# opensensor/thingino-accel

Measured on AMD Instinct MI355X. Metric: images/sec yolov5s_int8 640x640 batch256, higher is better.
Workload: dtype int8

## Files before the change

thingino-accel_amd/csrc/hip/conv_i8.hip:

```cpp
#include "conv_i8_common.hpp"

#ifndef I8M_ABL
#define I8M_ABL 0
#endif
template <int BPX, int BN, int STAGES, int KS = 1, int NW = 4>
__global__ __launch_bounds__(NW * 64) void conv_i8_mfma(const mhip_conv_i8_t p, const long total_pix, const int k64,
                                                         const int8_t *__restrict__ zeros, const unsigned noc,
                                                         const unsigned nblk, const int lg_inc, const unsigned kw_magic,
                                                         const fastdiv_t dhw, const fastdiv_t dow, const int bufmode,
                                                         const unsigned in_bytes) {
    ANAT_BEGIN();
    const bool POW2 = lg_inc >= 0;
    const bool masked = p.kh * p.kw <= 32;
    constexpr int SLICE = (BPX + BN) * BK;
    constexpr int STAGE = KS * SLICE;
    constexpr int NWN = BN == 128 ? 2 : 1;
    constexpr int NWM = NW / NWN;
    constexpr int WPX = BPX / NWM / 16;
    constexpr int WOC = BN / NWN / 16;
    constexpr int XROWS = BPX / NW;
    constexpr int XI = XROWS / 16;
    constexpr int LW = (BN / 16 + NW - 1) / NW;
    constexpr int L = XI + LW;
    static_assert(XI >= 1 && XROWS % 16 == 0, "every wave fetches whole 16-row pieces of the pixel tile");
// ... 1198 lines not shown
static bool chain_shape_ok(const mhip_conv_i8_t *a, const mhip_conv_i8_t *b, const mhip_conv_i8_t *d, int side) {
    if (!both_shape_ok(a, b) || a->out_c != 64 || !d || (side != 1 && side != 2)) return false;
    return d->kh == 1 && d->kw == 1 && d->stride_h == 1 && d->stride_w == 1 && !d->pad_top && !d->pad_left && d->in_c == 64 && d->out_c == 64 &&
           d->oc_pad == 64 && d->row_pad == 64 && d->frames == a->frames && d->in_h == a->out_h && d->in_w == a->out_w && d->out_h == a->out_h &&
           d->out_w == a->out_w && !d->out_pix_stride && !d->out_ch_off && d->lut && d->lut2 && !d->add && !d->out_nchw && d->nseg <= 1 &&
           persist_eligible(d) && d->out != a->out && d->out != b->out;
}
extern "C" int mhip_conv_i8_both_chain_ok(const mhip_conv_i8_t *a, const mhip_conv_i8_t *b, const mhip_conv_i8_t *d, int side) {
    return chain_shape_ok(a, b, d, side) ? 1 : 0;
}
static int both_launch(const mhip_conv_i8_t *a, const mhip_conv_i8_t *b, const conv_chain_t *ch);
extern "C" int mhip_conv_i8_both_chain(const mhip_conv_i8_t *a, const mhip_conv_i8_t *b, const mhip_conv_i8_t *d, int side, int elide) {
    if (!chain_shape_ok(a, b, d, side) || !d->w || !d->out) return -2;
    const mhip_conv_i8_t *src = side == 1 ? a : b;
    const mhip_conv_i8_t *other = side == 1 ? b : a;
    if (!other->out) return -2;
    if (!elide && (!src->out || d->in != src->out || d->in_stride != src->out_stride)) return -2;
    conv_chain_t ch;
    ch.w = d->w; ch.bias = d->bias; ch.lut2 = d->lut2; ch.out = d->out; ch.out_stride = d->out_stride;
    ch.out_bytes = (unsigned)persist_out_bytes(d); ch.cs = d->cs; ch.side = side; ch.elide = elide ? 1 : 0;
    return both_launch(a, b, &ch);
}
extern "C" int mhip_conv_i8_both(const mhip_conv_i8_t *a, const mhip_conv_i8_t *b) {
    if (!a || !b || !a->out || !b->out) return -2;
    return both_launch(a, b, nullptr);
}
static int both_launch(const mhip_conv_i8_t *a, const mhip_conv_i8_t *b, const conv_chain_t *ch) {
    if (!both_shape_ok(a, b) || (tune().variant && !ch) || !mhip_zero_page()) return -2;
    if (a->nseg > 1) {
        for (int i = 0; i < a->nseg; i++)
            if (a->seg_in[i] != b->seg_in[i]) return -2;
    } else if (a->in != b->in) {
        return -2;
    }
    const long total_pix = (long)a->frames * a->out_h * a->out_w;
    const int k64 = (a->kh * a->row_pad + BK - 1) / BK * BK, nks = k64 / BK;
    int lg = 0;
    while ((1 << lg) < a->in_c) lg++;
    int bpx, wres;
    both_form(2 * a->out_c, nks, ch != nullptr, &bpx, &wres);
    if (a->out_c == 128) {
        if (ch) return -2;
        return a->nseg > 1 ? launch_persist_t<128, 256, 2, true, true, false, true>(a, total_pix, k64, lg, 65536u, b, wres)
                           : launch_persist_t<128, 256, 2, true, false, false, true>(a, total_pix, k64, lg, 65536u, b, wres);
    }
    if (ch) {
        if (a->nseg > 1)
            return bpx == 256 ? launch_persist_t<256, 128, 2, true, true, false, true, true>(a, total_pix, k64, lg, 65536u, b, wres, ch)
                              : launch_persist_t<128, 128, 2, true, true, false, true, true>(a, total_pix, k64, lg, 65536u, b, wres, ch);
        return bpx == 256 ? launch_persist_t<256, 128, 2, true, false, false, true, true>(a, total_pix, k64, lg, 65536u, b, wres, ch)
                          : launch_persist_t<128, 128, 2, true, false, false, true, true>(a, total_pix, k64, lg, 65536u, b, wres, ch);
    }
    if (a->nseg > 1)
        return bpx == 256 ? launch_persist_t<256, 128, 2, true, true, false, true>(a, total_pix, k64, lg, 65536u, b, wres)
                          : launch_persist_t<128, 128, 2, true, true, false, true>(a, total_pix, k64, lg, 65536u, b, wres);
    return bpx == 256 ? launch_persist_t<256, 128, 2, true, false, false, true>(a, total_pix, k64, lg, 65536u, b, wres)
                      : launch_persist_t<128, 128, 2, true, false, false, true>(a, total_pix, k64, lg, 65536u, b, wres);
}

extern "C" int mhip_conv_i8_seg_ok(const mhip_conv_i8_t *p) {
    return p && (p->in_c % 16) == 0 && !mhip_conv_i8_small_c(p->in_c, p->kw, p->out_c) && seg_valid(p) && persist_eligible(p);
}

extern "C" int mhip_conv_i8_variants(const mhip_conv_i8_t *p, int *codes, int max) {
    if (!p || (p->in_c % 16) != 0 || mhip_conv_i8_small_c(p->in_c, p->kw, p->out_c)) return 0;
    const int k64 = (p->kh * p->row_pad + BK - 1) / BK * BK, nks = k64 / BK;
    int n = 0;
    if (p->pre_w) {
        const int first = conv_i8_pre_tile_rows(p);
        for (int th : {first, 16, 8, 4})
            if (th && n < max && conv_i8_patch_ok(p, th, nullptr)) {
                const int code = th == 16 ? 10 : (th == 8 ? 9 : 11);
                bool seen = false;
                for (int i = 0; i < n; i++) seen |= codes[i] == code;
                if (!seen) codes[n++] = code;
            }
        return n;
    }
    if (p->post_w) {
        for (int th : {16, 8, 4})
            if (n < max && conv_i8_patch_ok(p, th, nullptr)) codes[n++] = th == 16 ? 10 : (th == 8 ? 9 : 11);
        return n;
    }
    if (p->split_w) {
        for (int th : {16, 8, 4})
            if (n < max && conv_i8_patch_ok(p, th, nullptr)) codes[n++] = th == 16 ? 10 : (th == 8 ? 9 : 11);
        return n;
    }
    if (p->nseg > 1) {
        const int bn = p->oc_pad % 128 == 0 ? 128 : (p->oc_pad % 64 == 0 ? 64 : 32);
        const variant_t dv = default_variant(p, nks);
        const int dflt = dv.persist && dv.wres ? (dv.bpx == 256 ? 15 : 14) : (dv.bpx == 256 ? 4 : 2);
        if (n < max) codes[n++] = dflt;
        if (n < max && dflt != 2) codes[n++] = 2;
        if (n < max && dflt != 4) codes[n++] = 4;
        if (n < max && dflt != 14 && LUTB + 2 * (size_t)128 * BK + (size_t)nks * bn * BK <= 80 * 1024) codes[n++] = 14;
        if (n < max && dflt != 15 && LUTB + 2 * (size_t)256 * BK + (size_t)nks * bn * BK <= 80 * 1024) codes[n++] = 15;
        return n;
    }
    const int dflt = variant_code(default_variant(p, nks));
    if (n < max) codes[n++] = dflt;
    for (int code = 1; code <= NVARIANTS; code++) {
        const variant_t v = variant_of(code);
        if (code == dflt) continue;
        if (v.patch && !conv_i8_patch_ok(p, v.patch, nullptr)) continue;
        if (v.persist && !persist_eligible(p)) continue;
        if (v.ks2 && ((nks & 1) || nks < 4 || p->oc_pad % 64 != 0)) continue;
        if (v.w8 && (p->oc_pad % 128 != 0 || nks < 3)) continue;
        if (v.persist < 0) continue;
        if (v.r128 && !r128_ok(p)) continue;
        if (v.rows && !conv_i8_rows_ok(p)) continue;
        if (v.wres) {
            const int bn = p->oc_pad % 128 == 0 ? 128 : (p->oc_pad % 64 == 0 ? 64 : 32);
            if (LUTB + 2 * (size_t)v.bpx * BK + (size_t)nks * bn * BK > 80 * 1024) continue;
        }
        if (!v.persist && v.stages == 3 && nks <= 2) continue;
        if (n < max) codes[n++] = code;
    }
    return n;
}

template <int BN>
static int launch_generic(const mhip_conv_i8_t *p, long total_pix, int k64) {
    dim3 grid((unsigned)((total_pix + BP - 1) / BP), (unsigned)(p->oc_pad / BN));
    hipLaunchKernelGGL((conv_i8_generic<BN>), grid, dim3(NTHREADS), 0, mhip_stream_native(), *p, total_pix, k64,
                       make_fastdiv((unsigned)(p->out_h * p->out_w)));
    return mhip_check(hipGetLastError(), "conv_i8_generic launch");
}

extern "C" int mhip_conv_i8(const mhip_conv_i8_t *p) {
    if (!p || !p->in || (!p->out && !(p->post_w && p->post_out) && !(p->split_w && p->split_out[0] && p->split_out[1])) || !p->w) return -1;
    if (p->out_pix_stride < 0 || p->out_ch_off < 0 || (p->out_nchw && (p->out_pix_stride || p->out_ch_off)) ||
        (p->out_pix_stride && p->out_pix_stride < p->out_ch_off + p->out_c))
        return -1;
    if (p->frames <= 0 || p->in_h <= 0 || p->in_w <= 0 || p->in_c <= 0 || p->out_h <= 0 || p->out_w <= 0 ||
        p->out_c <= 0 || p->kh <= 0 || p->kw <= 0 || p->stride_h < 0 || p->stride_w < 0)
        return -1;
    int row_pad, oc_pad;
    mhip_conv_i8_pack_geom(p->in_c, p->kw, p->out_c, &row_pad, &oc_pad, nullptr);
    if (row_pad != p->row_pad || oc_pad != p->oc_pad) return -1;
    if (p->add && (!p->safe || p->out_nchw || ((p->out_c | p->out_pix_stride | p->out_ch_off) & 15) || (p->in_c % 16) != 0 ||
                   mhip_conv_i8_small_c(p->in_c, p->kw, p->out_c) || p->nseg > 1))
        return -1;
    const long total_pix = (long)p->frames * p->out_h * p->out_w;
    const int k64 = (p->kh * p->row_pad + BK - 1) / BK * BK;
    if (total_pix <= 0 || total_pix > 0x7fffffffL || (total_pix + BP - 1) / BP * (oc_pad / 32) > 0x7fffffffL) return -1;
    if (p->in_planar) {
        if (p->in_planar > 4 || p->in_c != 4 || p->in_w < 4 || p->stride_h < 1 || p->stride_w < 1 || p->add || p->nseg > 1 ||
            !mhip_conv_i8_small_c(p->in_c, p->kw, p->out_c))
            return -2;
        return conv_i8_try_smallc(p, k64);
    }
    if (mhip_conv_i8_small_c(p->in_c, p->kw, p->out_c)) {
        if (p->stride_h >= 1 && p->stride_w >= 1) {
            int rc = conv_i8_try_rgb(p, k64);
            if (rc == -2) rc = conv_i8_try_smallc(p, k64);
            if (rc != -2) return rc;
        }
        if (p->add || p->nseg > 1) return -1;
        if (oc_pad % 64 == 0) return launch_generic<64>(p, total_pix, k64);
        return launch_generic<32>(p, total_pix, k64);
    }
    if (p->pre_w) {
        if (!mhip_zero_page() || !mhip_conv_i8_pre_ok(p)) return -1;
        int th = conv_i8_pre_tile_rows(p);
        const int code = p->variant ? p->variant : tune().variant;
        if (code >= 9 && code <= 11) {
            const int want = code == 10 ? 16 : (code == 9 ? 8 : 4);
            if (conv_i8_patch_ok(p, want, nullptr)) th = want;
        } else if (tune().small_batch && conv_i8_patch_ok(p, 4, nullptr) &&
                   ((long)p->frames * p->out_h * p->out_w + 255) / 256 * ((p->oc_pad + 127) / 128) < 256) {
            th = 4;
        }
        return conv_i8_launch_patch(p, k64, th);
    }
    if (p->post_w) {
        if (!mhip_zero_page() || (p->in_c % 16) != 0 || !mhip_conv_i8_post_ok(p)) return -1;
        int th = conv_i8_post_tile_rows(p);
        const int code = p->variant ? p->variant : tune().variant;
        if (code >= 9 && code <= 11) {
            const int want = code == 10 ? 16 : (code == 9 ? 8 : 4);
            if (conv_i8_patch_ok(p, want, nullptr)) th = want;
        } else if (tune().small_batch && conv_i8_patch_ok(p, 4, nullptr) &&
                   ((long)p->frames * p->out_h * p->out_w + 255) / 256 * ((p->oc_pad + 127) / 128) < tune().few_wgs) {
            th = 4;
        }
        return conv_i8_launch_patch(p, k64, th);
    }
    if (p->split_w) {
        if (!mhip_zero_page() || (p->in_c % 16) != 0 || !mhip_conv_i8_split_ok(p)) return -1;
        int th = conv_i8_split_tile_rows(p);
        const int code = p->variant ? p->variant : tune().variant;
        if (code >= 9 && code <= 11) {
            const int want = code == 10 ? 16 : (code == 9 ? 8 : 4);
            if (conv_i8_patch_ok(p, want, nullptr)) th = want;
        } else if (tune().small_batch && conv_i8_patch_ok(p, 4, nullptr) &&
                   ((long)p->frames * p->out_h * p->out_w + 255) / 256 * ((p->oc_pad + 127) / 128) < tune().few_wgs) {
            th = 4;
        }
        return conv_i8_launch_patch(p, k64, th);
    }
    if ((p->in_c % 16) == 0) {
        if (!mhip_zero_page()) return -1;
        const int nks = k64 / BK;
        if (p->variant < 0 || p->variant > NVARIANTS) return -1;
        int code = p->variant;
        if (p->nseg > 1) {
            if (!seg_valid(p) || !persist_eligible(p)) return -1;
            if (!code && tune().variant) {
                int codes[NVARIANTS];
                const int n = mhip_conv_i8_variants(p, codes, NVARIANTS);
                for (int i = 0; i < n; i++)
                    if (codes[i] == tune().variant) code = codes[i];
            }
            variant_t v = variant_of(code == 4 || code == 14 || code == 15 ? code : 2);
            if (!code) {
                const variant_t dv = default_variant(p, nks);
                v.bpx = dv.bpx ? dv.bpx : 128;
                v.wres = dv.persist && dv.wres;
            }
            return launch_variant(p, total_pix, k64, v);
        }
        if (!code && tune().variant) {
            int codes[NVARIANTS];
            const int n = mhip_conv_i8_variants(p, codes, NVARIANTS);
            for (int i = 0; i < n; i++)
                if (codes[i] == tune().variant) code = codes[i];
        }
        return launch_variant(p, total_pix, k64, code ? variant_of(code) : default_variant(p, nks));
    }
    if (oc_pad % 64 == 0) return launch_generic<64>(p, total_pix, k64);
    return launch_generic<32>(p, total_pix, k64);
}
```

thingino-accel_amd/csrc/hip/conv_i8_common.hpp:

```cpp
#pragma once
#include <hip/hip_runtime.h>
#include <stdint.h>
#include <stdlib.h>
#include <string.h>
#include <type_traits>

#include "../mhip.h"

extern "C" hipStream_t mhip_stream_native(void);
extern "C" int mhip_check(hipError_t e, const char *what);
extern "C" const void *mhip_zero_page(void);

typedef int v4i __attribute__((ext_vector_type(4)));
typedef int v2i __attribute__((ext_vector_type(2)));

#ifdef ANATOMY
struct anat_rec_t {
    unsigned key, wg, hwid, xcc;
    unsigned long long t[4];
};
static __device__ anat_rec_t *g_anat_buf;
static __device__ unsigned g_anat_cap;
#define ANAT_SETTER(NAME)                                                                                                    \
    extern "C" int NAME(void *buf, unsigned cap) {                                                                          \
// ... 352 lines not shown
                if (rem & 8) { __builtin_memcpy(d, s, 8); o = 8; }
                if (rem & 4) { __builtin_memcpy(d + o, s + o, 4); o += 4; }
                if (rem & 2) { __builtin_memcpy(d + o, s + o, 2); o += 2; }
                if (rem & 1) d[o] = s[o];
            }
        }
    } else {
        for (int id = tid; id < BPX * BN; id += (int)blockDim.x) {
            const int c = id / BPX, row = id - c * BPX;
            const long off = rowoff[row];
            if (off < 0 || c >= ncols) continue;
            p.out[off + (size_t)(oc0 + c) * hw] = tile[row * ROW + c];
        }
    }
}

template <int BPX, int BN, int WPX, int WOC, bool LUT0 = false>
__device__ __forceinline__ void epilogue(const mhip_conv_i8_t &p, v4i (&acc)[WOC][WPX], int8_t *tile, const uint8_t *slut,
                                         const long *rowoff, int oc0, int pxw, int ocw, int hw) {
    const bool direct = !p.out_nchw && ((p.out_c | p.out_pix_stride | p.out_ch_off) & 15) == 0;
#define EPI(L, S, D) epilogue_t<BPX, BN, WPX, WOC, L, S, D, LUT0>(p, acc, tile, slut, rowoff, oc0, pxw, ocw, hw)
    if (direct) {
        if (p.lut) { if (p.safe) EPI(true, true, true); else EPI(true, false, true); }
        else { if (p.safe) EPI(false, true, true); else EPI(false, false, true); }
    } else {
        if (p.lut) { if (p.safe) EPI(true, true, false); else EPI(true, false, false); }
        else { if (p.safe) EPI(false, true, false); else EPI(false, false, false); }
    }
#undef EPI
}

template <int WPX, int WOC>
__device__ __forceinline__ void init_acc(const mhip_conv_i8_t &p, v4i (&acc)[WOC][WPX], int ocbase) {
    const int lane = threadIdx.x & 63;
#pragma unroll
    for (int s = 0; s < WOC; s++) {
        const v4i b = p.bias ? *(const v4i *)(p.bias + ocbase + s * 16 + (lane >> 4) * 4) : (v4i){0, 0, 0, 0};
#pragma unroll
        for (int t = 0; t < WPX; t++) acc[s][t] = b;
    }
}


struct tune_t {
    int init;
    int persist;
    int persist_stages;
    int persist_maxk;
    int persist_slots;
    int stages;
    int bpx;
    int variant;
    int bufmode;
    int small_batch;
    int rgb_direct;
    int wres;
    int few_wgs;
    int rows;
    int patch_ring;
    int patch_lds_kb;
    int both_bpx;
    int both_wide;
};
const tune_t &conv_i8_tune_state();

extern "C" int mhip_conv_i8_small_c(int in_c, int kw, int out_c);

static inline long in_extent_bytes(const mhip_conv_i8_t *p) {
    return (long)(p->frames - 1) * (long)p->in_stride + (long)p->in_h * p->in_w * p->in_c;
}
static inline long persist_out_bytes(const mhip_conv_i8_t *p) {
    const long pstride = p->out_pix_stride ? p->out_pix_stride : p->out_c;
    return (long)(p->frames - 1) * (long)p->out_stride + (long)p->out_h * p->out_w * pstride;
}
static inline bool conv_i8_direct_rows(const mhip_conv_i8_t *p) {
    return !p->out_nchw && ((p->out_c | p->out_pix_stride | p->out_ch_off) & 15) == 0;
}

bool conv_i8_patch_ok(const mhip_conv_i8_t *p, int th, int *ring);
int conv_i8_launch_patch(const mhip_conv_i8_t *p, int k64, int th);
int conv_i8_pre_tile_rows(const mhip_conv_i8_t *p);
int conv_i8_post_tile_rows(const mhip_conv_i8_t *p);
int conv_i8_split_tile_rows(const mhip_conv_i8_t *p);
bool conv_i8_rows_ok(const mhip_conv_i8_t *p);
int conv_i8_launch_rows(const mhip_conv_i8_t *p);
int conv_i8_try_rgb(const mhip_conv_i8_t *p, int k64);
int conv_i8_try_smallc(const mhip_conv_i8_t *p, int k64);
```

thingino-accel_amd/csrc/hip/conv_i8_patch.hip:

```cpp
#include "conv_i8_common.hpp"
#include <stdio.h>

#ifdef PATCH_STAMPS
__device__ unsigned long long patch_stamp_sums[8];
extern "C" int mhip_patch_stamps(unsigned long long *out, int reset) {
    if (out && hipMemcpyFromSymbol(out, HIP_SYMBOL(patch_stamp_sums), sizeof(patch_stamp_sums)) != hipSuccess) return -1;
    if (reset) {
        unsigned long long z[8] = {0};
        if (hipMemcpyToSymbol(HIP_SYMBOL(patch_stamp_sums), z, sizeof(z)) != hipSuccess) return -1;
    }
    return 0;
}
#define STAMP(t)                                                                          \
    do {                                                                                  \
        __builtin_amdgcn_sched_barrier(0);                                                \
        asm volatile("s_memtime %0\n\ts_waitcnt lgkmcnt(0)" : "=s"(t)::"memory");        \
        __builtin_amdgcn_sched_barrier(0);                                                \
    } while (0)
#else
#define STAMP(t) do { } while (0)
#endif
#define PT_TW 16
#define PT_NIMAX 10

template <int LO, int HI>
__device__ __forceinline__ void wait_vmcnt_tree(int n) {
    if constexpr (LO == HI) {
        wait_vmcnt<LO>();
    } else {
        constexpr int MID = (LO + HI + 1) / 2;
        if (n >= MID) wait_vmcnt_tree<MID, HI>(n);
        else wait_vmcnt_tree<LO, MID - 1>(n);
    }
}
template <int HI>
__device__ __forceinline__ void wait_vmcnt_upto(int n) {
    wait_vmcnt_tree<0, HI>(n > HI ? HI : n);
}
__device__ __forceinline__ void barrier_lds() {
    asm volatile("s_waitcnt lgkmcnt(0)\n\ts_barrier" ::: "memory");
}

template <int TH, int BN, bool HAS_LUT, bool PRE = false, bool POST = false, bool SPLIT = false, bool CHAIN = false>
__global__ __launch_bounds__(NTHREADS) void conv_i8_patch(const mhip_conv_i8_t p, const int k64, const int tiles_x,
                                                          const int tiles_y, const unsigned ntiles_all, const int PH,
                                                          const int PW, const int PWP, const int PWH, const int nblk,
                                                          const int8_t *__restrict__ zeros, const fastdiv_t dtx,
                                                          const fastdiv_t dty, const fastdiv_t dpwp, const unsigned out_bytes,
                                                          const int ring, const int xmap, const unsigned in_bytes) {
    ANAT_BEGIN();
    constexpr int WPX = TH / 4;
    constexpr int WOC = BN / 16;
    constexpr int NST = WPX;
    extern __shared__ __attribute__((aligned(16))) int8_t dynlds[];
    uint8_t *slut = (uint8_t *)dynlds;
    lds_base_must_be_zero(dynlds);
    const int nks = k64 / BK;
    constexpr int NPO = 2 * BN;
    static_assert(!SPLIT || (BN == 64 && HAS_LUT && !PRE && !POST), "SPLIT: one 64-channel tile, no other stage");
    static_assert(!CHAIN || SPLIT, "CHAIN: a stage of the SPLIT form");
    constexpr int LB = LUTB + ((PRE || POST) ? 512 : 0) + (SPLIT ? 1024 : 0) + (CHAIN ? 512 : 0);
    int *dutab = (int *)(dynlds + LB);
    int8_t *wl = dynlds + LB + ((nks * 16 + 255) & ~255);
    const int patch_bytes = nblk * 1024;
    int8_t *w1l = wl + nks * BN * BK;
    int8_t *pwl = w1l;
    const int *pbl = (const int *)(pwl + NPO * NPO);
    int8_t *swl = w1l;
    const int *sbl = (const int *)(swl + 64 * BK);
    int8_t *cwl = swl + 64 * BK + 64 * 4;
    const int *cbl = (const int *)(cwl + 32 * BK);
    int8_t *patch0 = w1l + (PRE ? p.in_c * BK : 0) + (POST ? NPO * NPO + NPO * 4 : 0) + (SPLIT ? 64 * BK + 64 * 4 : 0) + (CHAIN ? 32 * BK + 32 * 4 : 0);
    int8_t *tpatch = patch0 + ring * patch_bytes;

    const int tid = threadIdx.x, lane = tid & 63;
    const int wv = __builtin_amdgcn_readfirstlane(tid >> 6);
    const int oc0 = blockIdx.y * BN;
    const int C = p.in_c, lgc = 31 - __builtin_clz((unsigned)C), cpp = C >> 4, lgcpp = lgc - 4;
    const int s = p.stride_w;
    const unsigned M = C >= 128 ? 6u : (C >= 64 ? 2u : 0u);

    v4i bias[WOC];
#pragma unroll
    for (int q = 0; q < WOC; q++) bias[q] = p.bias ? *(const v4i *)(p.bias + oc0 + q * 16 + (lane >> 4) * 4) : (v4i){0, 0, 0, 0};
    constexpr int W1MAX = 4;
    v4i pbias[PRE ? W1MAX : 1];
    if (PRE) {
#pragma unroll
        for (int q = 0; q < W1MAX; q++) pbias[q] = q < (C >> 4) ? *(const v4i *)(p.pre_bias + q * 16 + (lane >> 4) * 4) : (v4i){0, 0, 0, 0};
    }
    if (HAS_LUT) {
        if (p.lut2) { if (tid < 128) ((uint32_t *)slut)[tid] = ((const uint32_t *)p.lut2)[tid]; }
        else if (tid < 64) ((uint32_t *)slut)[tid] = ((const uint32_t *)p.lut)[tid];
    }
    if (PRE && tid >= 128) ((uint32_t *)slut)[tid] = ((const uint32_t *)p.pre_lut2)[tid - 128];
    if (POST) {
        if (tid >= 128) ((uint32_t *)slut)[tid] = ((const uint32_t *)p.post_lut2)[tid - 128];
        if (tid < NPO) ((int *)(pwl + NPO * NPO))[tid] = ((const int *)(p.post_w + NPO * NPO))[tid];
    }
    if (SPLIT) {
        if (tid >= 128) {
            ((uint32_t *)slut)[tid] = ((const uint32_t *)p.split_lut2[0])[tid - 128];
            ((uint32_t *)slut)[tid + 128] = ((const uint32_t *)p.split_lut2[1])[tid - 128];
        }
        if (tid < 64) ((int *)(swl + 64 * BK))[tid] = ((const int *)(p.split_w + 64 * BK))[tid];
    }
    if (CHAIN) {
        if (tid >= 128) ((uint32_t *)slut)[tid + 256] = ((const uint32_t *)p.chain_lut2)[tid - 128];
        if (tid >= 64 && tid < 96) ((int *)(cwl + 32 * BK))[tid - 64] = ((const int *)(p.chain_w + 32 * BK))[tid - 64];
    }
    const int rowbytes = p.kw * C, kbytes = p.kh * rowbytes;
    for (int i = tid; i < nks * 4; i += NTHREADS) {
        const int kb = i * 16;
        int du = 0;
        if (kb < kbytes) {
            const int ky = kb / rowbytes, rem = kb - ky * rowbytes, kx = rem >> lgc, cc = (rem & (C - 1)) >> 4;
            const int dp = ky * PWP + (s == 2 ? (kx >> 1) + (kx & 1) * PWH : kx);
            du = dp * cpp + cc;
        }
        dutab[i] = du;
    }
    __syncthreads();
    {
        const int schunk = (lane & 3) ^ (((lane >> 4) & 1) << 1);
        for (int i = wv; i < nks * (BN / 16); i += 4) {
            const int ks = i / (BN / 16), g = i - ks * (BN / 16);
            glds16(p.w + (size_t)(oc0 + g * 16 + (lane >> 2)) * k64 + ks * BK + schunk * 16, wl + (ks * BN + g * 16) * BK);
        }
        if (PRE)
            for (int g = wv; g < C / 16; g += 4) glds16(p.pre_w + (size_t)(g * 16 + (lane >> 2)) * BK + schunk * 16, w1l + g * 16 * BK);
        if (POST)
            for (int i = wv; i < NPO * NPO / 1024; i += 4) glds16(p.post_w + i * 1024 + lane * 16, pwl + i * 1024);
        if (SPLIT)
            glds16(p.split_w + wv * 1024 + lane * 16, swl + wv * 1024);
        if (CHAIN && wv < 2)
            glds16(p.chain_w + wv * 1024 + lane * 16, cwl + wv * 1024);
    }
    int uoff[PT_NIMAX], upos[PT_NIMAX];
#pragma unroll
    for (int n = 0; n < PT_NIMAX; n++) {
        uoff[n] = 0;
        upos[n] = -1;
        if (n * 4 + wv < nblk) {
            const unsigned phys = (unsigned)((n * 4 + wv) * 64 + lane);
            const unsigned U = phys ^ ((phys >> 3) & M);
            const unsigned pp = U >> lgcpp, cc = U & (unsigned)(cpp - 1);
            const unsigned py = fdiv(pp, dpwp), col = pp - py * (unsigned)PWP;
            const int px = s == 2 ? ((int)col < PWH ? 2 * (int)col : 2 * ((int)col - PWH) + 1) : (int)col;
            if ((int)py < PH && px < PW) {
                uoff[n] = ((int)py * p.in_w + px) * C + (int)cc * 16;
                upos[n] = ((int)py << 16) | px;
            }
        }
    }
    const int npw = nblk > wv ? (nblk - wv + 3) >> 2 : 0;
    const unsigned xcd = blockIdx.x & 7u;
    const unsigned xstart = xmap ? (unsigned)(((unsigned long long)ntiles_all * xcd) >> 3) : 0u;
    const unsigned xend = xmap ? (unsigned)(((unsigned long long)ntiles_all * (xcd + 1u)) >> 3) : 0u;
    const unsigned ntiles = xmap ? (xend - xstart) * 8u + xcd : ntiles_all;
    auto tile_xy = [&](unsigned t, int &tx, int &ty, unsigned &f) {
        const unsigned j = xmap ? xstart + (t >> 3) : t, q = fdiv(j, dtx);
        tx = (int)(j - q * (unsigned)tiles_x);
        f = fdiv(q, dty);
        ty = (int)(q - f * (unsigned)tiles_y);
    };
    const __amdgpu_buffer_rsrc_t xrs = __builtin_amdgcn_make_buffer_rsrc((void *)p.in, 0, (int)in_bytes, 0x00020000);
    auto issue_patch = [&](unsigned t, int8_t *dst) {
#ifdef PATCH_ABL
        return;
#endif
        int tx, ty;
        unsigned f;
        tile_xy(t, tx, ty, f);
        const int iy0 = ty * TH * s - p.pad_top, ix0 = tx * PT_TW * s - p.pad_left;
        if (in_bytes != 0u && iy0 >= 0 && ix0 >= 0 && iy0 + PH <= p.in_h && ix0 + PW <= p.in_w) {
            const int sbase = (int)(f * (unsigned)p.in_stride) + (iy0 * p.in_w + ix0) * C;
#pragma unroll
            for (int n = 0; n < PT_NIMAX; n++)
                if (n * 4 + wv < nblk) blds16(xrs, uoff[n], sbase, dst + (n * 4 + wv) * 1024);
            return;
        }
        const int8_t *base = p.in + (size_t)f * p.in_stride + ((long)iy0 * p.in_w + ix0) * C;
#pragma unroll
        for (int n = 0; n < PT_NIMAX; n++)
            if (n * 4 + wv < nblk) {
                const int py = upos[n] >> 16, px = upos[n] & 0xffff;
                const bool ok = upos[n] >= 0 && (unsigned)(iy0 + py) < (unsigned)p.in_h && (unsigned)(ix0 + px) < (unsigned)p.in_w;
                glds16(ok ? base + uoff[n] : zeros, dst + (n * 4 + wv) * 1024);
            }
    };

    const __amdgpu_buffer_rsrc_t orsrc = __builtin_amdgcn_make_buffer_rsrc(SPLIT ? p.split_out[0] : (POST ? p.post_out : p.out), 0, (int)out_bytes, 0x00020000);
    const unsigned out_bytes1 = SPLIT ? (unsigned)(p.frames - 1) * (unsigned)p.split_out_stride[1] + (unsigned)(p.out_h * p.out_w) * 32u : 0u;
    const __amdgpu_buffer_rsrc_t orsrc1 = __builtin_amdgcn_make_buffer_rsrc(SPLIT ? p.split_out[1] : p.out, 0, (int)out_bytes1, 0x00020000);
    const unsigned out_bytes2 = CHAIN ? (unsigned)(p.frames - 1) * (unsigned)p.chain_out_stride + (unsigned)(p.out_h * p.out_w) * 32u : 0u;
    const __amdgpu_buffer_rsrc_t orsrc2 = __builtin_amdgcn_make_buffer_rsrc(CHAIN ? p.chain_out : p.out, 0, (int)out_bytes2, 0x00020000);
    const bool cside1 = CHAIN && p.chain_side == 2;
    const bool has_add = !SPLIT && p.add != nullptr;
    constexpr int RROW = WOC == 4 ? 1024 : 512;
    constexpr int NRI = WOC == 4 ? WPX : 2 * WPX;
    int8_t *rstage = patch0 + (ring + (PRE ? 1 : 0)) * patch_bytes + wv * (WPX * RROW);
    const int frow = lane & 15, fchunk = lane >> 4;
    const int chan = (lane >> 4) * (4 * WOC);
    const int NR = has_add || POST ? NRI : 0;
    const int ntail = POST ? (has_add ? NRI : 0) + WPX * (NPO / 64) : (SPLIT ? (CHAIN ? 3 : 2) * WPX : NST);
    const int ppstride = p.post_out_pix_stride ? p.post_out_pix_stride : NPO;
    auto issue_rows = [&](const int8_t *base, size_t fstride, int tx, int ty, unsigned f) {
#pragma unroll
        for (int u = 0; u < WPX; u++) {
            const int oy = ty * TH + wv * WPX + u, ox = tx * PT_TW + frow;
            const int8_t *src = oy < p.out_h && ox < p.out_w ? base + (size_t)f * fstride + ((size_t)(oy * p.out_w + ox) * BN + (size_t)chan) : zeros;
            if (WOC == 4) {
                glds16(src, rstage + u * RROW);
            } else {
                __builtin_amdgcn_global_load_lds((const __attribute__((address_space(1))) void *)src,
                                                 (__attribute__((address_space(3))) void *)(rstage + u * RROW), 4, 0, 0);
                __builtin_amdgcn_global_load_lds((const __attribute__((address_space(1))) void *)(src + 4),
                                                 (__attribute__((address_space(3))) void *)(rstage + u * RROW + 256), 4, 0, 0);
            }
        }
    };
    const int pstride = p.out_pix_stride ? p.out_pix_stride : p.out_c;
    const int lo = p.relu ? 0 : -128;
    const uint8_t *lut128 = slut + 128;
    int ubase[WPX];
#pragma unroll
    for (int u = 0; u < WPX; u++) ubase[u] = ((wv * WPX + u) * s * PWP + frow) * cpp;

    const unsigned G = gridDim.x;
    const int D = ring - 1;
    unsigned t = blockIdx.x;
    int yg0 = 0, yg1 = 0, yg2 = 0;
    {
        int issued = 0;
        for (int d = 0; d < D; d++)
            if (t + (unsigned)d * G < ntiles) {
                issue_patch(t + (unsigned)d * G, patch0 + d * patch_bytes);
                issued++;
            }
        yg0 = issued > 1 ? (issued - 1) * npw : 0;
        yg1 = issued > 2 ? (issued - 2) * npw : 0;
        yg2 = 0;
    }
#ifdef PATCH_STAMPS
    unsigned long long st0 = 0, st1 = 0, st2 = 0, st3 = 0, st4 = 0, sum_wait = 0, sum_issue = 0, sum_k = 0, sum_epi = 0, sum_tiles = 0;
#endif
    int cur = 0;
    int pn_last = 0;
    bool first = true;
    ANAT_NOW(1);
    for (; t < ntiles; t += G) {
        STAMP(st0);
        int tx, ty;
        unsigned f;
        tile_xy(t, tx, ty, f);
        int voffs[WPX];
        uint32_t xw[WPX][WOC];
#pragma unroll
        for (int u = 0; u < WPX; u++) {
            const int oy = ty * TH + wv * WPX + u, ox = tx * PT_TW + frow;
            const unsigned off = f * (unsigned)p.out_stride + (unsigned)(oy * p.out_w + ox) * (unsigned)pstride +
                                 (unsigned)(p.out_ch_off + oc0 + chan);
            const bool ok = oy < p.out_h && ox < p.out_w && oc0 + chan < p.out_c;
            voffs[u] = ok ? (int)off : -1;
#pragma unroll
            for (int q = 0; q < WOC; q++) xw[u][q] = 0;
        }
        if (POST) {
#pragma unroll
            for (int u = 0; u < WPX; u++) {
                const int oy = ty * TH + wv * WPX + u, ox = tx * PT_TW + frow;
                const unsigned off = f * (unsigned)p.post_out_stride + (unsigned)(oy * p.out_w + ox) * (unsigned)ppstride +
                                     (unsigned)(p.post_out_ch_off + (lane >> 4) * (NPO / 4));
                voffs[u] = oy < p.out_h && ox < p.out_w ? (int)off : -1;
            }
            if (has_add) issue_rows(p.add, p.out_stride, tx, ty, f);
            else issue_rows(p.post_in, p.post_in_stride, tx, ty, f);
        } else if (SPLIT) {
#pragma unroll
            for (int u = 0; u < WPX; u++) {
                const int oy = ty * TH + wv * WPX + u, ox = tx * PT_TW + frow;
                voffs[u] = oy < p.out_h && ox < p.out_w ? (oy * p.out_w + ox) * 32 + (lane >> 4) * 8 : -1;
            }
        } else if (has_add) {
#pragma unroll
            for (int u = 0; u < WPX; u++) {
                const int8_t *src = voffs[u] >= 0 ? p.add + (unsigned)voffs[u] : zeros;
                if (WOC == 4) {
// ... 59 lines not shown
                    }
                    uint32_t pk4[4];
                    requant_pack_pre<16>(a1, p.pre_cs, pk4);
#pragma unroll
                    for (int e = 0; e < 4; e++) pk1[e] = inimg ? pk4[e] : 0u;
                    const unsigned Uw = (unsigned)(pp * cpp + (lane >> 4));
                    if (live) *(v4i *)(tpatch + ((Uw ^ ((Uw >> 3) & M)) << 4)) = (v4i){(int)pk1[0], (int)pk1[1], (int)pk1[2], (int)pk1[3]};
                } else {
                    int a1[8];
#pragma unroll
                    for (int q = 0; q < 2; q++) {
                        const v4i wa = *(const v4i *)(w1l + lds_off(q * 16 + frow, fchunk));
                        const v4i r = __builtin_amdgcn_mfma_i32_16x16x64_i8(wa, xb1, pbias[PRE ? q : 0], 0, 0, 0);
#pragma unroll
                        for (int e = 0; e < 4; e++) a1[q * 4 + e] = r[e];
                    }
                    uint32_t pk2[2];
                    requant_pack_pre<8>(a1, p.pre_cs, pk2);
                    const int g4 = lane >> 4;
                    const unsigned Uw = (unsigned)(pp * cpp + (g4 >> 1));
                    if (live)
                        *(uint2 *)(tpatch + ((Uw ^ ((Uw >> 3) & M)) << 4) + (g4 & 1) * 8) = make_uint2(inimg ? pk2[0] : 0u, inimg ? pk2[1] : 0u);
                }
            }
            barrier_lds();
            patch = tpatch;
        }
        v4i acc[WOC][WPX];
        v4i xa[WPX], wa[WOC], xb[WPX], wb[WOC];
        auto load_frags = [&](int ks, int du, v4i (&xf)[WPX], v4i (&wf)[WOC]) {
#pragma unroll
            for (int u = 0; u < WPX; u++) {
                const unsigned U = (unsigned)(ubase[u] + du);
                xf[u] = *(const v4i *)(patch + ((U ^ ((U >> 3) & M)) << 4));
            }
            const int8_t *ws = wl + ks * BN * BK;
#pragma unroll
            for (int q = 0; q < WOC; q++) wf[q] = *(const v4i *)(ws + lds_off(q * 16 + frow, fchunk));
        };
        auto mfma_step = [&](const v4i (&xf)[WPX], const v4i (&wf)[WOC]) {
#pragma unroll
            for (int q = 0; q < WOC; q++)
#pragma unroll
                for (int u = 0; u < WPX; u++) acc[q][u] = __builtin_amdgcn_mfma_i32_16x16x64_i8(wf[q], xf[u], acc[q][u], 0, 0, 0);
        };
        const int last = nks - 1;
        auto clampk = [&](int k) { return k < last ? k : last; };
        load_frags(0, dutab[fchunk], xa, wa);
        load_frags(clampk(1), dutab[clampk(1) * 4 + fchunk], xb, wb);
        int du_n = dutab[clampk(2) * 4 + fchunk];
#pragma unroll
        for (int q = 0; q < WOC; q++)
#pragma unroll
            for (int u = 0; u < WPX; u++) acc[q][u] = __builtin_amdgcn_mfma_i32_16x16x64_i8(wa[q], xa[u], bias[q], 0, 0, 0);
        int ks = 1;
        for (; ks + 1 < nks; ks += 2) {
            load_frags(ks + 1, du_n, xa, wa);
            du_n = dutab[clampk(ks + 2) * 4 + fchunk];
            __builtin_amdgcn_sched_barrier(0);
            mfma_step(xb, wb);
            __builtin_amdgcn_sched_barrier(0);
            load_frags(clampk(ks + 2), du_n, xb, wb);
            du_n = dutab[clampk(ks + 3) * 4 + fchunk];
            __builtin_amdgcn_sched_barrier(0);
            mfma_step(xa, wa);
            __builtin_amdgcn_sched_barrier(0);
        }
        if (ks < nks) mfma_step(xb, wb);
        STAMP(st3);
        if (D > 0) cur = cur + 1 == ring ? 0 : cur + 1;
        if (has_add) {
            if (D > 0) wait_vmcnt_upto<15>(pn_last);
#pragma unroll
            for (int u = 0; u < WPX; u++) {
                if (WOC == 4) {
                    const v4i r = *(const v4i *)(rstage + u * RROW + lane * 16);
                    xw[u][0] = (uint32_t)r[0]; xw[u][1] = (uint32_t)r[1]; xw[u][WOC > 2 ? 2 : 0] = (uint32_t)r[2]; xw[u][WOC > 3 ? 3 : 0] = (uint32_t)r[3];
                } else {
                    xw[u][0] = *(const uint32_t *)(rstage + u * RROW + lane * 4);
                    xw[u][WOC > 1 ? 1 : 0] = *(const uint32_t *)(rstage + u * RROW + 256 + lane * 4);
                }
            }
        }
        uint32_t pku[POST || SPLIT ? WPX : 1][WOC];
        if (POST && has_add) {
#pragma unroll
            for (int u = 0; u < WPX; u++) {
                if constexpr (WOC == 4) asm volatile("s_waitcnt lgkmcnt(0)" : "+v"(xw[u][0]), "+v"(xw[u][1]), "+v"(xw[u][2]), "+v"(xw[u][3])::"memory");
                else asm volatile("s_waitcnt lgkmcnt(0)" : "+v"(xw[u][0]), "+v"(xw[u][1])::"memory");
            }
            issue_rows(p.post_in, p.post_in_stride, tx, ty, f);
        }
#pragma unroll
        for (int u = 0; u < WPX; u++) {
            uint32_t pk[WOC];
            int a[WOC * 4];
#pragma unroll
            for (int q = 0; q < WOC; q++)
#pragma unroll
                for (int r = 0; r < 4; r++) a[q * 4 + r] = acc[q][u][r];
            const bool fast = HAS_LUT && p.lut2 != nullptr;
            if (has_add) {
                const add_args_t ga = {p.add_s_conv, p.add_s_other, p.add_inv};
                if (fast) requant_pack<WOC * 4, HAS_LUT, true, true, true, true>(a, p.cs, lo, lut128, pk, xw[u], &ga);
                else requant_pack<WOC * 4, HAS_LUT, true, true, true>(a, p.cs, lo, lut128, pk, xw[u], &ga);
            } else {
                if (fast) requant_pack<WOC * 4, HAS_LUT, true, true, false, true>(a, p.cs, lo, lut128, pk);
                else requant_pack<WOC * 4, HAS_LUT, true, true>(a, p.cs, lo, lut128, pk);
            }
            if (POST) {
#pragma unroll
                for (int q = 0; q < WOC; q++) pku[POST ? u : 0][q] = pk[q];
                continue;
            }
            if (SPLIT) {
#pragma unroll
                for (int q = 0; q < WOC; q++) pku[SPLIT ? u : 0][q] = pk[q];
                continue;
            }
            const int voff = voffs[u];
            if (WOC == 4)
                __builtin_amdgcn_raw_buffer_store_b128((v4i){(int)pk[0], (int)pk[1], (int)pk[2], (int)pk[3]}, orsrc, voff, 0, 0);
            else if (WOC == 2)
                __builtin_amdgcn_raw_buffer_store_b64((v2i){(int)pk[0], (int)pk[WOC > 1 ? 1 : 0]}, orsrc, voff, 0, 0);
        }
        if (SPLIT) {
            v4i sw4[4], sb4[4];
#pragma unroll
            for (int r = 0; r < 4; r++) {
                sw4[r] = *(const v4i *)(swl + lds_off(r * 16 + frow, fchunk));
                sb4[r] = *(const v4i *)(sbl + r * 16 + fchunk * 4);
            }
            v4i sc[WPX][4];
#pragma unroll
            for (int u = 0; u < WPX; u++) {
                const v4i b0 = {(int)pku[SPLIT ? u : 0][0], (int)pku[SPLIT ? u : 0][1], (int)pku[SPLIT ? u : 0][WOC > 2 ? 2 : 0], (int)pku[SPLIT ? u : 0][WOC > 3 ? 3 : 0]};
#pragma unroll
                for (int r = 0; r < 4; r++) sc[u][r] = __builtin_amdgcn_mfma_i32_16x16x64_i8(sw4[r], b0, sb4[r], 0, 0, 0);
            }
            const unsigned fo0 = f * (unsigned)p.split_out_stride[0], fo1 = f * (unsigned)p.split_out_stride[1];
            uint32_t ck[CHAIN ? WPX : 1][2];
#pragma unroll
            for (int u = 0; u < WPX; u++) {
                int a2[16];
#pragma unroll
                for (int r = 0; r < 4; r++)
#pragma unroll
                    for (int e = 0; e < 4; e++) a2[r * 4 + e] = sc[u][r][e];
                uint32_t pk4[4];
                requant_pack_two(a2, p.split_cs[0], p.split_cs[1], pk4);
                const int voff0 = voffs[u] >= 0 ? voffs[u] + (int)fo0 : -1, voff1 = voffs[u] >= 0 ? voffs[u] + (int)fo1 : -1;
                __builtin_amdgcn_raw_buffer_store_b64((v2i){(int)pk4[0], (int)pk4[1]}, orsrc, voff0, 0, 0);
                __builtin_amdgcn_raw_buffer_store_b64((v2i){(int)pk4[2], (int)pk4[3]}, orsrc1, voff1, 0, 0);
                if (CHAIN) {
                    ck[CHAIN ? u : 0][0] = cside1 ? pk4[2] : pk4[0];
                    ck[CHAIN ? u : 0][1] = cside1 ? pk4[3] : pk4[1];
                }
            }
            if (CHAIN) {
                v4i cw4[2], cb4[2];
#pragma unroll
                for (int r = 0; r < 2; r++) {
                    cw4[r] = *(const v4i *)(cwl + lds_off(r * 16 + frow, fchunk));
                    cb4[r] = *(const v4i *)(cbl + r * 16 + fchunk * 4);
                }
                v4i cc[WPX][2];
#pragma unroll
                for (int u = 0; u < WPX; u++) {
                    const v4i b0 = {(int)ck[CHAIN ? u : 0][0], (int)ck[CHAIN ? u : 0][1], 0, 0};
#pragma unroll
                    for (int r = 0; r < 2; r++) cc[u][r] = __builtin_amdgcn_mfma_i32_16x16x64_i8(cw4[r], b0, cb4[r], 0, 0, 0);
                }
                const unsigned fo2 = f * (unsigned)p.chain_out_stride;
#pragma unroll
                for (int u = 0; u < WPX; u++) {
                    int a1[8];
#pragma unroll
                    for (int r = 0; r < 2; r++)
#pragma unroll
                        for (int e = 0; e < 4; e++) a1[r * 4 + e] = cc[u][r][e];
                    uint32_t pk2[2];
                    requant_pack_chain(a1, p.chain_cs, pk2);
                    const int voff2 = voffs[u] >= 0 ? voffs[u] + (int)fo2 : -1;
                    __builtin_amdgcn_raw_buffer_store_b64((v2i){(int)pk2[0], (int)pk2[1]}, orsrc2, voff2, 0, 0);
                }
            }
        }
        if (POST) {
            if (has_add) wait_vmcnt<0>();
            else if (D > 0) wait_vmcnt_upto<15>(pn_last);
#pragma unroll
            for (int u = 0; u < WPX; u++) {
                v4i b0, b1 = {0, 0, 0, 0};
                if (WOC == 4) {
                    b0 = (v4i){(int)pku[POST ? u : 0][0], (int)pku[POST ? u : 0][1], (int)pku[POST ? u : 0][WOC > 2 ? 2 : 0], (int)pku[POST ? u : 0][WOC > 3 ? 3 : 0]};
                    b1 = *(const v4i *)(rstage + u * RROW + lane * 16);
                } else {
                    b0 = (v4i){(int)pku[POST ? u : 0][0], (int)pku[POST ? u : 0][WOC > 1 ? 1 : 0], *(const int *)(rstage + u * RROW + lane * 4),
                               *(const int *)(rstage + u * RROW + 256 + lane * 4)};
                }
#pragma unroll
                for (int h = 0; h < NPO / 64; h++) {
                    int a[16];
#pragma unroll
                    for (int s4 = 0; s4 < 4; s4++) {
                        const int row = (h * 4 + s4) * 16;
                        v4i c = *(const v4i *)(pbl + row + fchunk * 4);
// ... 1 lines not shown
                        if (WOC == 4) c = __builtin_amdgcn_mfma_i32_16x16x64_i8(*(const v4i *)(pwl + NPO * BK + lds_off(row + frow, fchunk)), b1, c, 0, 0, 0);
#pragma unroll
                        for (int e = 0; e < 4; e++) a[s4 * 4 + e] = c[e];
                    }
                    uint32_t pk4[4];
                    requant_pack_pre<16>(a, p.post_cs, pk4);
                    const int voff = voffs[u] >= 0 ? voffs[u] + h * 16 : -1;
                    __builtin_amdgcn_raw_buffer_store_b128((v4i){(int)pk4[0], (int)pk4[1], (int)pk4[2], (int)pk4[3]}, orsrc, voff, 0, 0);
                }
            }
        }
#ifdef PATCH_STAMPS
        STAMP(st4);
        if (D == 0) st1 = st2;
        sum_wait += st1 - st0; sum_issue += st2 - st1; sum_k += st3 - st2; sum_epi += st4 - st3; sum_tiles += 1;
#endif
    }
    ANAT_NOW(2);
    ANAT_END(p);
#ifdef PATCH_STAMPS
    if (lane == 0) {
        atomicAdd(&patch_stamp_sums[0], sum_wait); atomicAdd(&patch_stamp_sums[1], sum_issue); atomicAdd(&patch_stamp_sums[2], sum_k);
        atomicAdd(&patch_stamp_sums[3], sum_epi); atomicAdd(&patch_stamp_sums[4], sum_tiles);
    }
#endif
}

ANAT_SETTER(mhip_anatomy_set_patch)
struct patch_geom_t {
    int bn, tiles_x, tiles_y, PH, PW, PWP, PWH, nblk, nks, ring;
    size_t lds;
};
static inline const tune_t &tune() { return conv_i8_tune_state(); }
static size_t patch_lds_budget(int bn) {
    const int kb = tune().patch_lds_kb;
    if (kb >= 16 && kb <= 160 && kb != 80) return (size_t)kb * 1024;
    return (size_t)(bn == 32 ? 53 : 80) * 1024;
}
static bool patch_geom(const mhip_conv_i8_t *p, int th, patch_geom_t *g) {
    const bool direct = conv_i8_direct_rows(p);
    const int C = p->in_c, s = p->stride_w;
    static const bool no_c16 = getenv("MARS_HIP_PATCH_NO_C16") != nullptr;
    if (!direct || !p->safe || (C != 16 && C != 32 && C != 64 && C != 128) || (C == 16 && (no_c16 || p->pre_w)) || (s != 1 && s != 2) || p->stride_h != s ||
        p->kh > 7 || p->kw > 7 || p->kh * p->kw < 2 || p->row_pad != p->kw * C || persist_out_bytes(p) > 0x7fffffffL)
        return false;
    const int k64 = (p->kh * p->row_pad + BK - 1) / BK * BK;
    g->nks = k64 / BK;
    g->bn = p->oc_pad % 64 == 0 ? 64 : 32;
    g->tiles_x = (p->out_w + PT_TW - 1) / PT_TW;
    g->tiles_y = (p->out_h + th - 1) / th;
    if ((double)p->out_h * p->out_w < (C == 128 ? 0.80 : 0.85) * (double)g->tiles_x * PT_TW * g->tiles_y * th) return false;
    g->PH = (th - 1) * s + p->kh;
    g->PW = (PT_TW - 1) * s + p->kw;
    g->PWH = s == 2 ? (g->PW + 1) / 2 : 0;
    g->PWP = s == 2 ? 2 * g->PWH : g->PW;
    const long units = (long)g->PH * g->PWP * (C / 16);
    g->nblk = (int)((units + 63) / 64);
    if (g->nblk > 4 * PT_NIMAX) return false;
    const bool pre = p->pre_w != nullptr;
    if (pre && (s != 1 || (C != 32 && C != 64) || !p->pre_bias || !p->pre_lut2 || !p->lut2)) return false;
    const bool post = p->post_w != nullptr;
    if (post) {
        const long ppstride = p->post_out_pix_stride ? p->post_out_pix_stride : 2 * g->bn;
        if (pre || s != 1 || p->out_c != g->bn || p->oc_pad != g->bn || p->out_pix_stride || p->out_ch_off || !p->lut2 || !p->post_lut2 || !p->post_in ||
            !p->post_out || ((p->post_out_pix_stride | p->post_out_ch_off) & 15) || p->post_out_pix_stride < 0 || p->post_out_ch_off < 0 ||
            ppstride < p->post_out_ch_off + 2 * g->bn ||
            (long)(p->frames - 1) * (long)p->post_out_stride + (long)p->out_h * p->out_w * ppstride > 0x7fffffffL)
            return false;
    }
    const bool split = p->split_w != nullptr;
    if (split) {
        if (pre || post || p->add || g->bn != 64 || p->out_c != 64 || p->oc_pad != 64 || p->out_pix_stride || p->out_ch_off || !p->lut2 || !p->split_lut2[0] ||
            !p->split_lut2[1] || !p->split_out[0] || !p->split_out[1])
            return false;
        for (int i = 0; i < 2; i++)
            if ((long)(p->frames - 1) * (long)p->split_out_stride[i] + (long)p->out_h * p->out_w * 32 > 0x7fffffffL) return false;
    }
    const bool chain = p->chain_side != 0;
    if (chain) {
        if (!split || (p->chain_side != 1 && p->chain_side != 2) || !p->chain_w || !p->chain_lut2 || !p->chain_out || p->chain_out == p->split_out[0] ||
            p->chain_out == p->split_out[1] || (long)(p->frames - 1) * (long)p->chain_out_stride + (long)p->out_h * p->out_w * 32 > 0x7fffffffL)
            return false;
    }
    const size_t pb = (size_t)g->nblk * 1024;
    const size_t radd = p->add || post ? (size_t)4 * (th / 4) * (g->bn == 64 ? 1024 : 512) : 0;
    const size_t fixed = LUTB + (pre ? 512 + (size_t)C * BK + pb : 0) + (post ? 512 + (size_t)4 * g->bn * g->bn + (size_t)8 * g->bn : 0) +
                         (split ? 1024 + (size_t)64 * BK + 64 * 4 : 0) + (chain ? 512 + (size_t)32 * BK + 32 * 4 : 0) +
                         (((size_t)g->nks * 16 + 255) & ~(size_t)255) + (size_t)g->nks * g->bn * BK + radd;
    const size_t budget = patch_lds_budget(g->bn);
    if (fixed + pb > budget) return false;
    const int fit = (int)((budget - fixed) / pb);
    const int cap = tune().patch_ring > 0 ? (tune().patch_ring > 4 ? 4 : tune().patch_ring) : 2;
    int ring = fit < cap ? fit : cap;
    g->ring = ring;
    g->lds = fixed + (size_t)ring * pb;
    if ((long)g->tiles_x * g->tiles_y * p->frames > 0x7fffffffL) return false;
    return true;
}

static inline long post_out_bytes(const mhip_conv_i8_t *p) {
    const long ppstride = p->post_out_pix_stride ? p->post_out_pix_stride : 2 * p->out_c;
    return (long)(p->frames - 1) * (long)p->post_out_stride + (long)p->out_h * p->out_w * ppstride;
}
static inline long split_out_bytes(const mhip_conv_i8_t *p, int side) {
    return (long)(p->frames - 1) * (long)p->split_out_stride[side] + (long)p->out_h * p->out_w * 32;
}
template <int TH, int BN, bool HAS_LUT, bool PRE = false, bool POST = false, bool SPLIT = false, bool CHAIN = false>
static int launch_patch_t(const mhip_conv_i8_t *p, int k64, const patch_geom_t &g) {
    auto kern = conv_i8_patch<TH, BN, HAS_LUT, PRE, POST, SPLIT, CHAIN>;
    static int cus = 0;
    static size_t slots_lds[8];
    static int slots_n[8], nslots = 0;
    if (!cus) {
        int dev = 0;
        hipDeviceProp_t prop;
        if (hipFuncSetAttribute((const void *)kern, hipFuncAttributeMaxDynamicSharedMemorySize, 160 * 1024) != hipSuccess ||
            hipGetDevice(&dev) != hipSuccess || hipGetDeviceProperties(&prop, dev) != hipSuccess)
            return mhip_check(hipErrorUnknown, "conv_i8_patch occupancy query");
        cus = prop.multiProcessorCount;
    }
    int slots = 0;
    for (int i = 0; i < nslots; i++)
        if (slots_lds[i] == g.lds) slots = slots_n[i];
    if (!slots) {
        int occ = 0;
        if (hipOccupancyMaxActiveBlocksPerMultiprocessor(&occ, kern, NTHREADS, g.lds) != hipSuccess)
            return mhip_check(hipErrorUnknown, "conv_i8_patch occupancy query");
        slots = (occ > 0 ? occ : 1) * cus;
        if (nslots < 8) { slots_lds[nslots] = g.lds; slots_n[nslots++] = slots; }
    }
    const unsigned ntiles = (unsigned)((long)g.tiles_x * g.tiles_y * p->frames);
    const unsigned noc = (unsigned)(p->oc_pad / BN);
    unsigned gx = (unsigned)(tune().persist_slots > 0 ? tune().persist_slots : slots) / noc;
    if (gx < 1) gx = 1;
    if (gx > ntiles) gx = ntiles;
    const int xmap = gx >= 8 && ntiles < 0x0fffffffu;
    if (xmap) gx &= ~7u;
    {
        static const char *dbg = getenv("MARS_HIP_PATCH_DEBUG");
        static size_t last_lds = 0;
        static int last_ring = 0;
        if (dbg && (last_lds != g.lds || last_ring != g.ring)) {
            fprintf(stderr, "Mars: conv_i8_patch<%d,%d> ring %d, patch %d KB, LDS %zu B, %d workgroups per CU, grid %u x %u\n", TH, BN, g.ring,
                    g.nblk, g.lds, slots / cus, gx, noc);
            last_lds = g.lds;
            last_ring = g.ring;
        }
    }
    hipLaunchKernelGGL(kern, dim3(gx, noc), dim3(NTHREADS), g.lds, mhip_stream_native(), *p, k64,
                       g.tiles_x, g.tiles_y, ntiles, g.PH, g.PW, g.PWP, g.PWH, g.nblk, (const int8_t *)mhip_zero_page(),
                       make_fastdiv((unsigned)g.tiles_x), make_fastdiv((unsigned)g.tiles_y), make_fastdiv((unsigned)g.PWP),
                       (unsigned)(SPLIT ? split_out_bytes(p, 0) : (POST ? post_out_bytes(p) : persist_out_bytes(p))), g.ring, xmap,
                       in_extent_bytes(p) <= 0x7fffffffL ? (unsigned)in_extent_bytes(p) : 0u);
    return mhip_check(hipGetLastError(), "conv_i8_patch launch");
}

bool conv_i8_patch_ok(const mhip_conv_i8_t *p, int th, int *ring) {
    patch_geom_t g;
    if (!patch_geom(p, th, &g)) return false;
    if (ring) *ring = g.ring;
    return true;
}

int conv_i8_launch_patch(const mhip_conv_i8_t *p, int k64, int th) {
    patch_geom_t g;
    if (!patch_geom(p, th, &g)) return -1;
#define PATCH(T, B)                                                                       \
    (p->post_w ? launch_patch_t<T, B, true, false, true>(p, k64, g)                       \
     : p->pre_w ? launch_patch_t<T, B, true, true>(p, k64, g)                             \
                : (p->lut ? launch_patch_t<T, B, true>(p, k64, g) : launch_patch_t<T, B, false>(p, k64, g)))
    if (p->split_w && p->chain_side) {
        if (th == 16) return launch_patch_t<16, 64, true, false, false, true, true>(p, k64, g);
        if (th == 8) return launch_patch_t<8, 64, true, false, false, true, true>(p, k64, g);
        return launch_patch_t<4, 64, true, false, false, true, true>(p, k64, g);
    }
    if (p->split_w) {
        if (th == 16) return launch_patch_t<16, 64, true, false, false, true>(p, k64, g);
        if (th == 8) return launch_patch_t<8, 64, true, false, false, true>(p, k64, g);
        return launch_patch_t<4, 64, true, false, false, true>(p, k64, g);
    }
    if (th == 16) return g.bn == 64 ? PATCH(16, 64) : PATCH(16, 32);
    if (th == 8) return g.bn == 64 ? PATCH(8, 64) : PATCH(8, 32);
    return g.bn == 64 ? PATCH(4, 64) : PATCH(4, 32);
#undef PATCH
}

int conv_i8_pre_tile_rows(const mhip_conv_i8_t *p) {
    patch_geom_t g;
    for (int th : {16, 8, 4})
        if (patch_geom(p, th, &g) && (th == 4 || g.ring >= 2)) return th;
    return 0;
}
extern "C" int mhip_conv_i8_pre_ok(const mhip_conv_i8_t *p) {
    if (!p || !p->pre_w || p->nseg > 1 || p->out_nchw) return 0;
    return conv_i8_pre_tile_rows(p) != 0;
}

int conv_i8_post_tile_rows(const mhip_conv_i8_t *p) {
    patch_geom_t g;
    for (int th : {16, 8, 4})
        if (patch_geom(p, th, &g)) return th;
    return 0;
}
extern "C" int mhip_conv_i8_post_ok(const mhip_conv_i8_t *p) {
    if (!p || !p->post_w || p->pre_w || p->nseg > 1 || p->out_nchw) return 0;
    return conv_i8_post_tile_rows(p) != 0;
}
extern "C" int mhip_conv_i8_post_k(int c, int k) {
    if (c == 64) return k;
    return k < 32 ? (k >> 3) * 16 + (k & 7) : ((k - 32) >> 3) * 16 + 8 + (k & 7);
}
extern "C" int mhip_conv_i8_post_row(int c, int oc) {
    const int per = c / 2, g = oc / per, rem = oc - g * per;
    return (rem >> 2) * 16 + g * 4 + (rem & 3);
}
extern "C" size_t mhip_conv_i8_post_pack(int c, const int8_t *packed, const int32_t *bias, int8_t *out) {
    if (c != 32 && c != 64) return 0;
    const int n = 2 * c;
    const size_t bytes = (size_t)n * n + (size_t)n * 4;
    if (!packed || !out) return bytes;
    memset(out, 0, bytes);
    for (int oc = 0; oc < n; oc++) {
        const int R = mhip_conv_i8_post_row(c, oc), src = mhip_conv_i8_oc_row(oc, n);
        for (int k = 0; k < n; k++) {
            const int pos = mhip_conv_i8_post_k(c, k), ks = pos >> 6, chunk = (pos & 63) >> 4;
            out[(size_t)(ks * n + R) * BK + (((chunk ^ ((R >> 1) & 2))) << 4) + (pos & 15)] = packed[(size_t)src * n + k];
        }
        ((int32_t *)(out + (size_t)n * n))[R] = bias ? bias[src] : 0;
    }
    return bytes;
}

int conv_i8_split_tile_rows(const mhip_conv_i8_t *p) {
    patch_geom_t g;
    for (int th : {16, 8, 4})
        if (patch_geom(p, th, &g)) return th;
    return 0;
}
extern "C" int mhip_conv_i8_split_ok(const mhip_conv_i8_t *p) {
    if (!p || !p->split_w || p->pre_w || p->post_w || p->add || p->nseg > 1 || p->out_nchw) return 0;
    return conv_i8_split_tile_rows(p) != 0;
}
extern "C" int mhip_conv_i8_split_row(int side, int oc) {
    const int g = oc >> 3, rem = oc & 7;
    return side * 32 + (rem >> 2) * 16 + g * 4 + (rem & 3);
}
extern "C" size_t mhip_conv_i8_split_pack(const int8_t *packed0, const int32_t *bias0, const int8_t *packed1, const int32_t *bias1, int8_t *out) {
    const size_t bytes = (size_t)64 * BK + (size_t)64 * 4;
    if (!packed0 || !packed1 || !out) return bytes;
    memset(out, 0, bytes);
    for (int side = 0; side < 2; side++) {
        const int8_t *packed = side ? packed1 : packed0;
        const int32_t *bias = side ? bias1 : bias0;
        for (int oc = 0; oc < 32; oc++) {
            const int R = mhip_conv_i8_split_row(side, oc), src = mhip_conv_i8_oc_row(oc, 32);
            for (int k = 0; k < 64; k++) out[(size_t)R * BK + ((((k >> 4) ^ ((R >> 1) & 2))) << 4) + (k & 15)] = packed[(size_t)src * 64 + k];
            ((int32_t *)(out + (size_t)64 * BK))[R] = bias ? bias[src] : 0;
        }
    }
    return bytes;
}

extern "C" int mhip_conv_i8_chain_k(int c) { return (c >> 3) * 16 + (c & 7); }
extern "C" size_t mhip_conv_i8_chain_pack(const int8_t *packed, const int32_t *bias, int8_t *out) {
    const size_t bytes = (size_t)32 * BK + (size_t)32 * 4;
    if (!packed || !out) return bytes;
    memset(out, 0, bytes);
    for (int oc = 0; oc < 32; oc++) {
        const int R = mhip_conv_i8_split_row(0, oc), src = mhip_conv_i8_oc_row(oc, 32);
        for (int c = 0; c < 32; c++) {
            const int k = mhip_conv_i8_chain_k(c);
            out[(size_t)R * BK + ((((k >> 4) ^ ((R >> 1) & 2))) << 4) + (k & 15)] = packed[(size_t)src * 64 + c];
        }
        ((int32_t *)(out + (size_t)32 * BK))[R] = bias ? bias[src] : 0;
    }
    return bytes;
}
```

thingino-accel_amd/csrc/host/mars_internal.h:

```cpp
#ifndef MARS_INTERNAL_H
#define MARS_INTERNAL_H

#include <math.h>
#include <stddef.h>
#include <stdint.h>

#include "../mhip.h"
#include "mars_hip.h"
#include "mars_runtime.h"

enum {
    OP_CONV_I8 = 0,
    OP_CONV_F32,
    OP_RELU_BYTES,
    OP_LUT_I8,
    OP_BINARY_I8,
    OP_SIGMOID_F32,
    OP_BINARY_F32,
    OP_RELU_F32,
    OP_BN,
    OP_MAXPOOL,
    OP_CONCAT_SLICE,
    OP_UPSAMPLE,
    OP_UPSAMPLE_Q, OP_MAXPOOL_Q,
    OP_CONCAT_Q,
    OP_CONV_F32_VHEAD,
    OP_FAIL,
};

#define NO_OFF ((size_t)-1)
#define MARS_MAX_IO 4
#define MARS_MAX_MODEL_TUNE 16

typedef struct {
    size_t bytes;
    size_t extent;
    size_t stride;
    uint8_t *dev;
    int is_weight;
    int needed;
    int io_in, io_out;
    uint8_t *host;
    uint8_t *dense_dev;
    int pix_c, pix_stride;
    int rec_c, rec_hw;
    int nhwc_c, nhwc_hw;
    size_t zero_from;
    int partial;
    int nhwc_pitch;
    int tail_read;
} mtensor_t;

typedef struct {
    int kind, layer, err;
    int t_in[4], n_in, t_out;
    int in_h, in_w, in_c, out_h, out_w, out_c, kh, kw, sh, sw, pt, pl;
    int nchw, relu, is_mul, is_f32, leaky, safe;
    size_t in_byte_off, out_byte_off;
    int k_limit;
    int vc_n, vc_t[3], vc_run, vc_shift;
    int rows_only;
    int out_nchw;
    int silu_f32;
    int f32_exact;
    int variant;
    int add_t; float add_s_conv, add_s_other, add_inv;
    int nseg, seg_t[4], seg_c[4], seg_up;
    int chain_n, chain_out[3];
    int pair_next;
    int pair_both;
    int both_chain;
    int both_elide;
    int row_pad, oc_pad, c_pad;
    int ch_off, scale_h, scale_w, bn_n;
    int out_pix_stride, out_ch_off;
    int store_c;
    float cs, f0, f1, f2;
    size_t n;
    size_t w_off, b_off, lut_off, s_off;
    int pre;
    size_t pre_w_off, pre_b_off, pre_lut2_off;
    float pre_cs;
    int post_next;
    size_t post_w_off;
    int split_next;
    size_t split_w_off;
    int split_chain;
    size_t chain_w_off;
    size_t w2_off;
    int w2_rows;
    int w2_planes;
    size_t w3_off;
    int w3_stem;
    int in_rec, out_rec;
    size_t lut2_off;
    size_t w_blob_off[2];
    double macs, bytes;
    int prof_kind;
    float last_ms;
    void *ev0, *ev1;
    int prof_rec;
    void *ev_start;
} mars_op_t;

typedef struct { void *dev; size_t bytes; int frames; void *ev[2]; } mars_block_t;
typedef struct { void *dst; size_t off, bytes; } mars_block_part_t;
typedef struct { void *dev; int cap, frames; } mars_det_side_t;
typedef struct { int buf; const int8_t *base; size_t stride; int c, h, w, pix_step, ch_step; } mars_side_tensor_t;
typedef struct { float key[4][2]; int n; } mars_lut_cache_t;

typedef struct {
    int fusion;
    unsigned no_fuse_lut : 1, no_nhwc_internal : 1, no_vconcat_q : 1, no_pair_f32 : 1, no_rec : 1, no_zero_tail : 1, no_vconcat_f32 : 1,
        no_rowpad : 1, no_post : 1, no_split : 1, no_chain : 1, no_both : 1, no_both_chain : 1;
    size_t rec_limit;
    size_t vconcat_limit;
    size_t bottleneck_limit;
} plan_switches_t;

typedef struct mars_model_ext {
    mars_model_t pub;
    plan_switches_t sw;
    int batch, profiling, deferred;
    int plan_err;
    int no_vconcat;
    int no_download;
    int no_bottleneck;
    int no_post;
    int no_split;
    int no_chain;
    int no_both;
    int no_both_chain;
    int rec_frames;
    int rec_skipped;
    size_t rec_max_frames;
    mtensor_t *mt;
    mars_op_t *ops;
    int n_ops, cap_ops;
    uint8_t *arena_host;
    size_t arena_size, arena_cap;
    uint8_t *arena_dev;
    size_t blob_mirror_bytes;
    uint8_t *act_dev;
    size_t act_bytes;
    uint8_t *scratch_dev;
    size_t scratch_per_frame;
    int scratch_t, scratch_cpad, scratch_f0, scratch_n;
    void *det_dev;
    int *det_counts_dev;
    float *det_lut_dev;
    int det_cap;
    mars_lut_cache_t det_lut;
    int det_lut_mono[4];
    float *heads_lut_dev;
    mars_lut_cache_t heads_lut;
    float *dfl_lut_dev;
    mars_lut_cache_t dfl_lut;
    void *ev_graph_done, *ev_tail_done;
    int tail_pending;
    int frame0, run_frames;
    void *ev_fork, *ev_join[3];
    void *ev_chunk[2][8];
    void *graph_exec;
    unsigned graph_gen;
    int ran_plain;
    void *pipe;
    struct { char key[28]; int value, saved; } tune[MARS_MAX_MODEL_TUNE];
    int n_tune, tune_depth;
    int plan_f32_mode;
    unsigned char *layer_noop;
    void *roi_dev;
    int roi_cap_slots, roi_cap_frames;
    int roi_slots;
    struct mars_model_ext *roi_from;
    void *roi_fit_dev;
    int roi_fit_slots;
    mars_block_t cls;
    size_t cls_sums_off, cls_top_off;
    int cls_c, cls_top_k;
    void *ev_label_done;
    int label_pending;
    mars_det_side_t label;
    mars_block_t match;
    size_t match_top_off, match_row_off;
    int match_top_k;
    mars_det_side_t ident;
    mars_det_side_t track;
    mars_block_t track_app;
    mars_block_t seg;
    size_t seg_rec_off, seg_word_off;
    int seg_max, seg_ph, seg_pw;
    mars_block_t segn;
    size_t segn_rec_off, segn_word_off;
    int segn_max, segn_oh, segn_ow;
    int segn_key[10];
    mars_block_t pose;
    size_t pose_rec_off, pose_kpt_off;
    int pose_max, pose_k;
    mars_lut_cache_t pose_lut;
    mars_block_t obb;
    size_t obb_cnt_off, obb_out_off, obb_csn_off;
    mars_lut_cache_t obb_lut;
    int det_mapped;
    mars_block_t tile_roi;
    mars_block_t tile;
    size_t tile_off[4];
    mars_block_t redact;
    size_t redact_stats_off;
    void *ev_redact_done;
    mars_block_t overlay;
    size_t overlay_stats_off;
    void *overlay_img;
    size_t overlay_img_bytes;
    mars_det_side_t motion;
    struct mars_model_ext *live_next;
} mars_model_ext_t;

enum {
    FORM_PLAIN = 0,
    FORM_PAIR,
    FORM_BOTH,
    FORM_BOTH_CHAIN,
    FORM_POST,
    FORM_SPLIT,
    FORM_SPLIT_CHAIN,
    FORM_PAIR_F32,
    FORM_BAD,
    FORM_COUNT
};
static inline int form_span(int form) {
    static const int span[FORM_COUNT] = {[FORM_PLAIN] = 1, [FORM_PAIR] = 2, [FORM_BOTH] = 2, [FORM_BOTH_CHAIN] = 3, [FORM_POST] = 2, [FORM_SPLIT] = 3,
                                         [FORM_SPLIT_CHAIN] = 4, [FORM_PAIR_F32] = 2, [FORM_BAD] = 1};
    return form >= 0 && form < FORM_COUNT ? span[form] : 0;
}
static inline int op_form(const mars_model_ext_t *m, int i, int g[4]) {
    const mars_op_t *o = &m->ops[i];
    int form = FORM_PLAIN;
    if (o->split_next) form = o->split_chain ? FORM_SPLIT_CHAIN : FORM_SPLIT;
    else if (o->post_next) form = FORM_POST;
    else if (o->pair_next) form = o->kind == OP_CONV_F32 ? FORM_PAIR_F32 : !o->pair_both ? FORM_PAIR : o->both_chain ? FORM_BOTH_CHAIN : FORM_BOTH;
    int span = form_span(form);
    if (i + span > m->n_ops) { form = FORM_BAD; span = m->n_ops - i; }
    for (int k = 0; k < 4; k++) g[k] = k < span ? i + k : -1;
    return form;
}
static inline int op_span(const mars_model_ext_t *m, int i) {
    int g[4], n = 0;
    op_form(m, i, g);
    while (n < 4 && g[n] >= 0) n++;
    return n;
}
static inline int op_head(const mars_model_ext_t *m, int i) {
    int h = 0;
    for (int s; h + (s = op_span(m, h)) <= i; h += s) {}
    return h;
}
static inline int op_is_mate(const mars_model_ext_t *m, int i) { return op_head(m, i) != i; }
static inline int op_plain(const mars_model_ext_t *m, int i) {
    int g[4];
    return op_form(m, i, g) == FORM_PLAIN;
}
static inline uint8_t *tdev(const mars_model_ext_t *m, int ti) {
    if (ti < 0 || !m->mt[ti].dev) return NULL;
    return m->mt[ti].dev + (m->mt[ti].is_weight ? 0 : (size_t)m->frame0 * m->mt[ti].stride);
}
static inline size_t tstride(const mars_model_ext_t *m, int ti) { return ti >= 0 ? m->mt[ti].stride : 0; }


#define MARS_INTERNAL __attribute__((visibility("hidden")))
#define ALIGN_UP(x, a) (((x) + (size_t)(a) - 1) & ~((size_t)(a) - 1))
#define NO_TENSOR 0xFFFFFFFFu
#define MAX_DIM_PRODUCT ((size_t)1 << 40)
#define ARENA_MAX ((size_t)1 << 40)
#define MAX_CHANNELS 65536
MARS_INTERNAL int mars_verbose(void);
#define VLOG(...) do { if (mars_verbose()) fprintf(stderr, "Mars: " __VA_ARGS__); } while (0)
MARS_INTERNAL void drop_graph(mars_model_ext_t *m);
MARS_INTERNAL mars_model_ext_t *mars_live_models(void);
MARS_INTERNAL void plan_switches_read(plan_switches_t *sw, int at_load);
MARS_INTERNAL mars_error_t build_plan(mars_model_ext_t *m);
MARS_INTERNAL mars_error_t upload_params(mars_model_ext_t *m);
MARS_INTERNAL mars_error_t alloc_batch(mars_model_ext_t *m, int n);
MARS_INTERNAL size_t elem_size(uint32_t dtype);
MARS_INTERNAL size_t shape_numel(const mars_tensor_t *d);
MARS_INTERNAL size_t reference_buffer_size(const mars_model_ext_t *m);
MARS_INTERNAL size_t arena_reserve(mars_model_ext_t *m, size_t bytes);
MARS_INTERNAL void blob_read(const mars_model_ext_t *m, size_t off, size_t n, void *dst);
MARS_INTERNAL int op_reads(const mars_op_t *o, int t);
MARS_INTERNAL int op_writes(const mars_op_t *o, int t);
MARS_INTERNAL size_t planned_stride(const mtensor_t *t);
MARS_INTERNAL int conv_i8_pre_fits(const mars_op_t *op, int frames, size_t in_stride, size_t out_stride);
MARS_INTERNAL void conv_i8_group_records(const mars_model_ext_t *m, int form, const mars_op_t *g[4], int side, int frames, int live, mhip_conv_i8_t *p);
MARS_INTERNAL int conv_i8_group_fits(const mars_model_ext_t *m, int form, const mars_op_t *g[4], int side, int frames);
MARS_INTERNAL void fuse_both_chain(mars_model_ext_t *m);
MARS_INTERNAL void plan_layer(mars_model_ext_t *m, int li);
MARS_INTERNAL void fold_silu(mars_model_ext_t *m, int f32);
MARS_INTERNAL void fuse_lut(mars_model_ext_t *m);
MARS_INTERNAL void nhwc_internal(mars_model_ext_t *m);
MARS_INTERNAL void fold_add(mars_model_ext_t *m, int f32);
MARS_INTERNAL void virtual_concat(mars_model_ext_t *m);
MARS_INTERNAL void elide_concat(mars_model_ext_t *m);
MARS_INTERNAL void trim_concat(mars_model_ext_t *m);
MARS_INTERNAL void fuse_pool_chains(mars_model_ext_t *m);
MARS_INTERNAL void pair_convs(mars_model_ext_t *m);
MARS_INTERNAL void fuse_bottleneck(mars_model_ext_t *m);
MARS_INTERNAL void fuse_post(mars_model_ext_t *m);
MARS_INTERNAL void fuse_split(mars_model_ext_t *m);
MARS_INTERNAL void fuse_split_chain(mars_model_ext_t *m);
MARS_INTERNAL void pad_output_rows(mars_model_ext_t *m);
MARS_INTERNAL void virtual_concat_q(mars_model_ext_t *m);
MARS_INTERNAL void f32_policy(mars_model_ext_t *m);
MARS_INTERNAL void zero_tail_f32(mars_model_ext_t *m);
MARS_INTERNAL void pair_convs_f32(mars_model_ext_t *m);
MARS_INTERNAL void rec_pairs(mars_model_ext_t *m);
MARS_INTERNAL void virtual_concat_f32(mars_model_ext_t *m);
MARS_INTERNAL void plan_check(mars_model_ext_t *m);
MARS_INTERNAL int mars_preproc_prepare(int w, int h, int tw, int th);
MARS_INTERNAL int mars_preproc_prepare_nv12(int w, int h, int tw, int th, int frames);

MARS_INTERNAL void mars_roi_release(mars_model_ext_t *m);

static inline int mars_scale_ok(float s) { return s > 0 && isfinite(s); }
static inline mars_error_t mars_stage_guard(const mars_model_ext_t *m) {
    if (!m->act_dev || !mhip_ready()) return MARS_ERR_NNA_INIT_FAILED;
    return m->pipe ? MARS_ERR_INVALID_TENSOR : MARS_OK;
}
static inline int mars_has_dets(const mars_model_ext_t *m) { return m->det_dev && m->det_counts_dev && m->det_cap >= m->batch; }
typedef struct { int tid, nhwc, tw, th; int8_t *dev; size_t stride; } mars_pixel_input_t;
MARS_INTERNAL mars_error_t mars_pixel_input(const mars_model_ext_t *m, int input_index, int geometry_only, mars_pixel_input_t *out);
MARS_INTERNAL mars_error_t mars_aux_behind_current(void **ev);
MARS_INTERNAL size_t mars_block_layout(const size_t *sz, int n, size_t *off);
MARS_INTERNAL mars_error_t mars_block_reserve(mars_block_t *b, size_t total, int with_events, int *fresh);
MARS_INTERNAL void mars_block_release(mars_block_t *b);
MARS_INTERNAL float mars_block_ms(const mars_block_t *b);
MARS_INTERNAL mars_error_t mars_block_fetch(const mars_block_t *b, const mars_block_part_t *parts, int n, int *tail_pending);
MARS_INTERNAL mars_error_t mars_side_reserve(mars_det_side_t *s, int frames, size_t rec);
MARS_INTERNAL void mars_side_release(mars_det_side_t *s);
MARS_INTERNAL mars_error_t mars_side_fetch(const mars_det_side_t *s, void *dst, size_t rec);
MARS_INTERNAL mars_error_t mars_scatter_on_aux(mars_model_ext_t *det, mars_model_ext_t *m, const mars_block_t *src, size_t top_off, int top_k,
                                               mars_det_side_t *side);
MARS_INTERNAL mars_error_t mars_side_tensor(const mars_model_ext_t *m, int T, int want_c, int want_h, int want_w, mars_side_tensor_t *out);
MARS_INTERNAL int mars_lut_stale(const mars_lut_cache_t *c, int n, const float key[4][2]);
MARS_INTERNAL mars_error_t mars_lut_refresh(mars_lut_cache_t *c, void *dst, int n, const float key[4][2], const float *tab, size_t floats_per_head);
MARS_INTERNAL void mars_stages_release(mars_model_ext_t *m);

MARS_INTERNAL int mars_tensor_chw(const mars_tensor_t *d, int *c, int *h, int *w);
MARS_INTERNAL int mars_locate_i8(const mars_model_ext_t *m, int T, int ch, int hh, int ww, int any_writer, int *buf, int *off, int *pix_step, int *ch_step);
MARS_INTERNAL mars_error_t mars_own_det_buffers(mars_model_ext_t *m);
MARS_INTERNAL mars_error_t mars_tail_on_aux(mars_model_ext_t *m, int (*launch)(struct mars_model_ext *, const void *, void *, int *), const void *cfg);

mars_error_t mars_detect_prepare(mars_model_ext_t *m, const int *output_indices, int n_outputs);
int mars_detect_launch(mars_model_ext_t *m, const int *output_indices, int n_outputs, float nms_thresh, void *dets_dev,
                       int *counts_dev);

typedef struct {
    int n, ti[4], stride[4], nc[4], h[4], w[4], pix_step[4], ch_step[4];
    float anchors[4][3][2];
    float conf, nms;
    int map, px, py;
    float rx, ry;
    int internal;
} mars_heads_cfg_t;
MARS_INTERNAL int mars_find_heads(const mars_model_ext_t *m, int *tensor_ids, int *strides, int *num_classes, int cap);
MARS_INTERNAL mars_error_t mars_heads_resolve(mars_model_ext_t *m, const mars_yolo_heads_t *h, mars_heads_cfg_t *c);
MARS_INTERNAL mars_error_t mars_heads_prepare(mars_model_ext_t *m, const mars_heads_cfg_t *c);
MARS_INTERNAL int mars_heads_launch(mars_model_ext_t *m, const mars_heads_cfg_t *c, void *dets_dev, int *counts_dev);

typedef struct {
    int n, reg_max, stride[4], nc[4], h[4], w[4];
    int box_t[4], cls_t[4], box_buf[4], cls_buf[4], box_off[4], cls_off[4];
    int box_pix_step[4], box_ch_step[4], cls_pix_step[4], cls_ch_step[4];
    float box_scale[4], cls_scale[4];
    float conf, nms;
    int map, px, py;
    float rx, ry;
    int nw, nh;
    int internal;
    int *cand_pred, *kept_pred;
    void *premap;
} mars_dfl_cfg_t;
MARS_INTERNAL int mars_find_dfl_heads(const mars_model_ext_t *m, int *box_ids, int *cls_ids, int *strides, int *num_classes, int *reg_max, int cap);
MARS_INTERNAL mars_error_t mars_dfl_resolve(mars_model_ext_t *m, const mars_yolo_dfl_heads_t *h, mars_dfl_cfg_t *c);
MARS_INTERNAL mars_error_t mars_dfl_prepare(mars_model_ext_t *m, const mars_dfl_cfg_t *c);
MARS_INTERNAL int mars_dfl_launch(mars_model_ext_t *m, const mars_dfl_cfg_t *c, void *dets_dev, int *counts_dev);

int32_t mars_trunc_x86(float x);
void mars_pack_conv_i8(const int8_t *w, size_t avail, int nchw, int out_c, int in_c, int kh, int kw,
                       int c_pad, int row_pad, int oc_pad, int8_t *dst);

#endif
```

thingino-accel_amd/csrc/host/mars_model.c:

```c
#include <math.h>
#include <stdio.h>
#include <stdlib.h>
#include <string.h>
#include <sys/types.h>
#include <time.h>

#include "mars_internal.h"
#include "nna.h"


int mars_verbose(void) {
    static int v = -1;
    if (v < 0) v = getenv("MARS_VERBOSE") ? 1 : 0;
    return v;
}

void plan_switches_read(plan_switches_t *sw, int at_load) {
    const char *e;
    if (at_load) sw->fusion = (e = getenv("MARS_HIP_FUSION")) ? atoi(e) : 1;
    sw->no_fuse_lut = getenv("MARS_HIP_NO_FUSE_LUT") != NULL;
    sw->no_nhwc_internal = getenv("MARS_HIP_NO_NHWC_INTERNAL") != NULL;
    sw->no_vconcat_q = getenv("MARS_HIP_NO_VCONCAT_Q") != NULL;
    sw->no_pair_f32 = getenv("MARS_HIP_NO_PAIR_F32") != NULL;
    sw->no_rec = getenv("MARS_HIP_NO_REC") != NULL;
    sw->no_zero_tail = getenv("MARS_HIP_NO_ZERO_TAIL") != NULL;
    sw->no_vconcat_f32 = getenv("MARS_HIP_NO_VCONCAT_F32") != NULL;
    sw->no_rowpad = getenv("MARS_HIP_NO_ROWPAD") != NULL;
    sw->no_post = getenv("MARS_HIP_NO_POST") != NULL;
    sw->no_split = getenv("MARS_HIP_NO_SPLIT") != NULL;
    sw->no_chain = getenv("MARS_HIP_NO_CHAIN") != NULL;
    sw->no_both = getenv("MARS_HIP_NO_BOTH") != NULL;
    sw->no_both_chain = getenv("MARS_HIP_NO_BOTH_CHAIN") != NULL;
    sw->rec_limit = (e = getenv("MARS_HIP_REC_LIMIT")) ? (size_t)strtoull(e, NULL, 0) : (size_t)0xfffffff0u;
    sw->vconcat_limit = (e = getenv("MARS_HIP_VCONCAT_LIMIT")) ? (size_t)strtoull(e, NULL, 0) : (size_t)0x7fffffffu;
    sw->bottleneck_limit = (e = getenv("MARS_HIP_BOTTLENECK_LIMIT")) ? (size_t)strtoull(e, NULL, 0) : 0;
}

void drop_graph(mars_model_ext_t *m) {
    if (m->graph_exec) {
        mhip_sync();
        mhip_graph_destroy(m->graph_exec);
    }
    m->graph_exec = NULL;
    m->ran_plain = 0;
}

static const char *const k_err[] = {
    "OK", "Invalid magic number", "Version mismatch", "Memory allocation failed",
    "Invalid file format", "NNA initialization failed", "Layer execution failed",
    "Invalid tensor", "Invalid layer",
};

const char *mars_get_error_string(mars_error_t err) {
    int i = -(int)err;
    if (i >= 0 && i < (int)(sizeof(k_err) / sizeof(k_err[0]))) return k_err[i];
    return "Unknown error";
}

static void free_device_state(mars_model_ext_t *m) {
    drop_graph(m);
    if (m->act_dev) mhip_free(m->act_dev);
    if (m->scratch_dev) mhip_free(m->scratch_dev);
    m->act_dev = m->scratch_dev = NULL;
    for (uint32_t i = 0; m->mt && i < m->pub.header.num_tensors; i++) {
        if (m->mt[i].host) mhip_host_free(m->mt[i].host);
        m->mt[i].host = NULL;
        if (m->mt[i].dense_dev) mhip_free(m->mt[i].dense_dev);
        m->mt[i].dense_dev = NULL;
        if (!m->mt[i].is_weight) m->mt[i].dev = NULL;
    }
    if (m->det_dev) mhip_free(m->det_dev);
    if (m->det_counts_dev) mhip_free(m->det_counts_dev);
    m->det_dev = NULL;
    m->det_counts_dev = NULL;
    m->det_cap = 0;
    m->tail_pending = 0;
    mars_stages_release(m);
}

static void free_ops(mars_model_ext_t *m) {
    drop_graph(m);
    for (int i = 0; i < m->n_ops; i++) {
        if (m->ops[i].ev0) mhip_event_destroy(m->ops[i].ev0);
        if (m->ops[i].ev1) mhip_event_destroy(m->ops[i].ev1);
    }
    free(m->ops);
    m->ops = NULL;
    m->n_ops = m->cap_ops = 0;
}

static mars_model_ext_t *g_live_models = NULL;
mars_model_ext_t *mars_live_models(void) { return g_live_models; }

void mars_free(mars_model_t *model) {
    if (!model) return;
    mars_model_ext_t *m = (mars_model_ext_t *)model;
    for (mars_model_ext_t **pp = &g_live_models; *pp; pp = &(*pp)->live_next)
        if (*pp == m) { *pp = m->live_next; break; }
    for (mars_model_ext_t *x = g_live_models; x; x = x->live_next)
        if (x->roi_from == m) x->roi_from = NULL;
    if (m->pipe) mars_hip_pipe_close(model);
    if (mhip_ready()) mhip_sync();
    free_device_state(m);
    free_ops(m);
    if (m->arena_dev) mhip_free(m->arena_dev);
    if (m->det_lut_dev) mhip_free(m->det_lut_dev);
    if (m->heads_lut_dev) mhip_free(m->heads_lut_dev);
    if (m->dfl_lut_dev) mhip_free(m->dfl_lut_dev);
    if (m->ev_graph_done) mhip_event_destroy(m->ev_graph_done);
    if (m->ev_tail_done) mhip_event_destroy(m->ev_tail_done);
    if (m->ev_label_done) mhip_event_destroy(m->ev_label_done);
    if (m->ev_fork) mhip_event_destroy(m->ev_fork);
    for (int k = 0; k < 3; k++)
        if (m->ev_join[k]) mhip_event_destroy(m->ev_join[k]);
    for (int k = 0; k < 2; k++)
        for (int c = 0; c < 8; c++)
            if (m->ev_chunk[k][c]) mhip_event_destroy(m->ev_chunk[k][c]);
    free(m->arena_host);
    free(m->layer_noop);
    free(m->mt);
    free(m->pub.weights);
    free(m->pub.layers);
    free(m->pub.tensors);
    free(m);
}

mars_error_t build_plan(mars_model_ext_t *m) {
    const uint32_t nt = m->pub.header.num_tensors, nl = m->pub.header.num_layers;
    plan_switches_read(&m->sw, 0);
    free_ops(m);
    m->arena_size = 0;
    if (m->arena_host) memset(m->arena_host, 0, m->arena_cap);
    m->scratch_per_frame = 0;
    m->plan_err = MARS_OK;
    m->plan_f32_mode = mhip_conv_f32_mode(-1);
    m->blob_mirror_bytes = m->pub.weights_size;
    for (uint32_t i = 0; i < nt; i++) {
        m->mt[i].extent = m->mt[i].bytes;
        m->mt[i].pix_c = m->mt[i].pix_stride = 0;
        m->mt[i].needed = (m->mt[i].io_in || m->mt[i].io_out) ? 1 : 0;
    }
    for (uint32_t i = 0; i < nl && m->plan_err == MARS_OK; i++) {
        const int n0 = m->n_ops;
        plan_layer(m, (int)i);
        m->layer_noop[i] = m->n_ops == n0;
    }
    if (m->plan_err != MARS_OK) return (mars_error_t)m->plan_err;
    if (m->sw.fusion >= 1) {
        fold_silu(m, 0);
        fuse_lut(m);
        fold_silu(m, 1);
        nhwc_internal(m);
        fold_add(m, 0);
        fold_add(m, 1);
        if (!m->no_vconcat) virtual_concat(m);
        elide_concat(m);
        trim_concat(m);
        fuse_pool_chains(m);
        pair_convs(m);
        if (m->sw.fusion >= 2 && !m->no_bottleneck) fuse_bottleneck(m);
        fuse_post(m);
        fuse_split(m);
        fuse_split_chain(m);
        pad_output_rows(m);
        virtual_concat_q(m);
        fuse_both_chain(m);
    } else {
        nhwc_internal(m);
    }
    f32_policy(m);
    zero_tail_f32(m);
    if (m->sw.fusion >= 1) pair_convs_f32(m);
    rec_pairs(m);
    virtual_concat_f32(m);
    if (m->plan_err == MARS_OK) plan_check(m);
    return (mars_error_t)m->plan_err;
}

mars_error_t upload_params(mars_model_ext_t *m) {
    size_t mirror_off = arena_reserve(m, m->blob_mirror_bytes + 64);
    if (mirror_off == NO_OFF) return MARS_ERR_ALLOC_FAILED;
    if (!m->deferred) blob_read(m, 0, m->blob_mirror_bytes, m->arena_host + mirror_off);
    if (m->arena_dev) mhip_free(m->arena_dev);
    m->arena_dev = (uint8_t *)mhip_malloc(m->arena_size);
    if (!m->arena_dev) return MARS_ERR_ALLOC_FAILED;
    if (mhip_h2d_async(m->arena_dev, m->arena_host, m->arena_size) || mhip_sync()) return MARS_ERR_NNA_INIT_FAILED;
    for (uint32_t i = 0; i < m->pub.header.num_tensors; i++) {
        if (!m->mt[i].is_weight) continue;
        m->mt[i].dev = m->arena_dev + mirror_off + (size_t)m->pub.tensors[i].desc.data_offset;
        m->mt[i].stride = 0;
        m->pub.tensors[i].paddr = m->mt[i].dev;
    }
    m->pub.ddr_paddr = m->arena_dev;
    m->pub.ddr_size = m->arena_size;
    return MARS_OK;
}

static mars_error_t replan(mars_model_ext_t *m) {
    const mars_error_t e = build_plan(m);
    return e == MARS_OK ? upload_params(m) : e;
}

enum { ASK_VCONCAT, ASK_PRE, ASK_GROUP };
typedef struct { size_t flag; int ask, form, chained; } take_back_t;
#define FLAG(f) offsetof(mars_model_ext_t, f)
static const take_back_t TAKE_BACK[] = {
    {FLAG(no_vconcat), ASK_VCONCAT, 0, 0},
    {FLAG(no_bottleneck), ASK_PRE, 0, 0},
    {FLAG(no_post), ASK_GROUP, FORM_POST, FORM_POST},
    {FLAG(no_chain), ASK_GROUP, FORM_SPLIT_CHAIN, FORM_SPLIT_CHAIN},
    {FLAG(no_split), ASK_GROUP, FORM_SPLIT, FORM_SPLIT_CHAIN},
    {FLAG(no_both_chain), ASK_GROUP, FORM_BOTH_CHAIN, FORM_BOTH_CHAIN},
    {FLAG(no_both), ASK_GROUP, FORM_BOTH, FORM_BOTH_CHAIN},
};
#undef FLAG

mars_error_t alloc_batch(mars_model_ext_t *m, int n) {
    const uint32_t nt = m->pub.header.num_tensors;
    if (m->pipe) mars_hip_pipe_close(&m->pub);
    if (mhip_sync()) return MARS_ERR_LAYER_FAILED;
    plan_switches_read(&m->sw, 0);
    const size_t vlim = m->sw.vconcat_limit, blim = m->sw.bottleneck_limit;
    const int rec_replan = (size_t)n > m->rec_max_frames || (m->rec_skipped && n < m->rec_frames);
    m->rec_frames = n;
    if (m->no_vconcat || m->no_bottleneck || m->no_post || m->no_split || m->no_chain || m->no_both || m->no_both_chain || rec_replan) {
        m->no_vconcat = m->no_bottleneck = m->no_post = m->no_split = m->no_chain = m->no_both = m->no_both_chain = 0;
        const mars_error_t e = replan(m);
        if (e != MARS_OK) return e;
    }
    for (size_t r = 0; r < sizeof TAKE_BACK / sizeof *TAKE_BACK; r++) {
        const take_back_t *tb = &TAKE_BACK[r];
        int *off = (int *)((char *)m + tb->flag);
        if (*off || (tb->ask == ASK_PRE && m->sw.fusion < 2)) continue;
        for (int i = 0; i < m->n_ops; i++) {
            const mars_op_t *op = &m->ops[i], *mem[4] = {op, NULL, NULL, NULL};
            int g[4], fits = 1;
            if (op->kind != OP_CONV_I8) continue;
            if (tb->ask == ASK_VCONCAT) {
                fits = op->nseg < 2 || op->t_out < 0 || planned_stride(&m->mt[op->t_out]) * (size_t)n <= vlim;
            } else if (tb->ask == ASK_PRE) {
                const size_t in_stride = op->t_in[0] >= 0 ? planned_stride(&m->mt[op->t_in[0]]) : 0;
                fits = !op->pre || op->t_out < 0 || (conv_i8_pre_fits(op, n, in_stride, planned_stride(&m->mt[op->t_out])) && !(blim && (size_t)n > blim));
            } else {
                const int form = op_form(m, i, g);
                if (form != tb->form && form != tb->chained) continue;
                for (int q = 1; q < form_span(tb->form); q++) mem[q] = &m->ops[g[q]];
                fits = conv_i8_group_fits(m, tb->form, mem, tb->form == FORM_SPLIT_CHAIN ? op->split_chain : op->both_chain, n);
            }
            if (fits) continue;
            *off = 1;
            const mars_error_t e = replan(m);
            if (e != MARS_OK) return e;
            break;
        }
    }
    free_device_state(m);
    size_t per_frame = 0;
    for (uint32_t i = 0; i < nt; i++) {
        mtensor_t *t = &m->mt[i];
        if (t->is_weight || !t->needed) continue;
        t->stride = planned_stride(t);
        per_frame += t->stride;
    }
    m->act_bytes = per_frame * (size_t)n;
    m->act_dev = (uint8_t *)mhip_malloc(m->act_bytes + 512);
    if (!m->act_dev) return MARS_ERR_ALLOC_FAILED;
    if (mhip_memset_async(m->act_dev, 0, m->act_bytes + 256)) return MARS_ERR_ALLOC_FAILED;
    size_t off = 256;
    for (uint32_t i = 0; i < nt; i++) {
        mtensor_t *t = &m->mt[i];
        mars_runtime_tensor_t *rt = &m->pub.tensors[i];
        if (t->is_weight) continue;
        rt->vaddr = NULL; rt->paddr = NULL; rt->alloc_size = 0;
        if (!t->needed) continue;
        t->dev = m->act_dev + off;
        off += t->stride * (size_t)n;
        rt->paddr = t->dev;
        rt->alloc_size = t->stride * (size_t)n;
        if (t->io_in || t->io_out) {
            const size_t hb = t->bytes * (size_t)n, ref = reference_buffer_size(m);
            size_t cap = hb > ref ? hb : ref;
            if (ref > ((size_t)8 << 20)) cap = hb;
            t->host = (uint8_t *)mhip_host_alloc(cap ? cap : 64);
            if (!t->host) return MARS_ERR_ALLOC_FAILED;
            memset(t->host, 0, cap);
            rt->vaddr = t->host;
            rt->alloc_size = n == 1 && cap >= ref ? ref : hb;
        }
        if (t->pix_stride) {
            t->dense_dev = (uint8_t *)mhip_malloc(t->bytes * (size_t)n);
            if (!t->dense_dev) return MARS_ERR_ALLOC_FAILED;
        }
    }
    if (m->scratch_per_frame) {
        m->scratch_dev = (uint8_t *)mhip_malloc(ALIGN_UP(m->scratch_per_frame, 256) * (size_t)n + 256);
        if (!m->scratch_dev) return MARS_ERR_ALLOC_FAILED;
    }
    m->batch = n;
    m->frame0 = 0;
    m->run_frames = n;
    return mhip_sync() ? MARS_ERR_ALLOC_FAILED : MARS_OK;
}

static mars_error_t load_host(const void *data, size_t size, unsigned flags, mars_model_ext_t **out_m) {
    if (!data || !out_m || size < sizeof(mars_header_t)) return MARS_ERR_INVALID_FILE;
    const uint8_t *p = (const uint8_t *)data;
    mars_header_t h;
    memcpy(&h, p, sizeof(h));
    if (h.magic != MARS_MAGIC) {
// ... 20 lines not shown
    m->layer_noop = (unsigned char *)calloc(h.num_layers ? h.num_layers : 1, 1);
    if (!m->pub.tensors || !m->pub.layers || !m->mt || !m->layer_noop) { mars_free(&m->pub); return MARS_ERR_ALLOC_FAILED; }
    const uint8_t *q = p + sizeof(h);
    for (uint32_t i = 0; i < h.num_tensors; i++, q += sizeof(mars_tensor_t)) memcpy(&m->pub.tensors[i].desc, q, sizeof(mars_tensor_t));
    for (uint32_t i = 0; i < h.num_layers; i++, q += sizeof(mars_layer_t)) memcpy(&m->pub.layers[i].desc, q, sizeof(mars_layer_t));

    m->pub.weights_size = (size_t)h.weights_size;
    if (h.weights_size) {
        m->pub.weights = calloc(1, (size_t)h.weights_size);
        if (!m->pub.weights) { mars_free(&m->pub); return MARS_ERR_ALLOC_FAILED; }
        if (!deferred) memcpy(m->pub.weights, p + h.weights_offset, (size_t)h.weights_size);
    }
    m->pub.ddr_base = m->pub.weights;
    for (uint32_t i = 0; i < h.num_tensors; i++) {
        mars_runtime_tensor_t *rt = &m->pub.tensors[i];
        if (rt->desc.ndims > MARS_MAX_DIMS) { mars_free(&m->pub); return MARS_ERR_INVALID_FILE; }
        m->mt[i].bytes = shape_numel(&rt->desc) * elem_size(rt->desc.dtype);
        if (rt->desc.data_size > 0) {
            if (rt->desc.data_offset > h.weights_size) { mars_free(&m->pub); return MARS_ERR_INVALID_FILE; }
            m->mt[i].is_weight = 1;
            rt->vaddr = (uint8_t *)m->pub.weights + rt->desc.data_offset;
            rt->alloc_size = (size_t)rt->desc.data_size;
        }
    }
    for (uint32_t i = 0; i < h.num_inputs; i++) {
        uint32_t id = h.input_tensor_ids[i];
        if (id < h.num_tensors && !m->mt[id].is_weight) m->mt[id].io_in = (int)i + 1;
    }
    for (uint32_t i = 0; i < h.num_outputs; i++) {
        uint32_t id = h.output_tensor_ids[i];
        if (id < h.num_tensors && !m->mt[id].is_weight) m->mt[id].io_out = (int)i + 1;
    }

    mars_error_t err = build_plan(m);
    if (err != MARS_OK) { mars_free(&m->pub); return err; }
    VLOG("%u layers -> %d launches, parameter arena %zu bytes\n", h.num_layers, m->n_ops, m->arena_size);
    *out_m = m;
    return MARS_OK;
}

mars_error_t mars_hip_load_memory_ex(const void *data, size_t size, unsigned flags, mars_model_t **out_model) {
    if (!out_model) return MARS_ERR_INVALID_FILE;
    mars_model_ext_t *m = NULL;
    mars_error_t err = load_host(data, size, flags, &m);
    if (err != MARS_OK) return err;
    if (!nna_is_ready() || !mhip_ready()) {
        fprintf(stderr, "Mars: no initialised MI355X device (call nna_init first); refusing to load\n");
        mars_free(&m->pub);
        return MARS_ERR_NNA_INIT_FAILED;
    }
    err = upload_params(m);
    if (err == MARS_OK) err = alloc_batch(m, 1);
    if (err != MARS_OK) { mars_free(&m->pub); return err; }
    m->live_next = g_live_models;
    g_live_models = m;
    *out_model = &m->pub;
    return MARS_OK;
}

static int describe_op_full(const mars_op_t *o, char *line, size_t cap, int k) {
#define ADD(...) k += snprintf(line + k, cap - (size_t)k, __VA_ARGS__)
    ADD(" | err %d in %dx%dx%d out %dx%dx%d k %dx%d s %dx%d p %d,%d", o->err, o->in_h, o->in_w, o->in_c, o->out_h, o->out_w, o->out_c, o->kh, o->kw, o->sh, o->sw, o->pt, o->pl);
    ADD(" nchw %d out_nchw %d relu %d is_mul %d is_f32 %d leaky %d safe %d silu %d f32_exact %d variant %d", o->nchw, o->out_nchw, o->relu, o->is_mul, o->is_f32, o->leaky,
        o->safe, o->silu_f32, o->f32_exact, o->variant);
    ADD(" row_pad %d oc_pad %d c_pad %d store_c %d ch_off %d out_ch_off %d out_pix_stride %d in_byte_off %zu out_byte_off %zu scale %dx%d bn_n %d n %zu", o->row_pad,
        o->oc_pad, o->c_pad, o->store_c, o->ch_off, o->out_ch_off, o->out_pix_stride, o->in_byte_off, o->out_byte_off, o->scale_h, o->scale_w, o->bn_n, o->n);
    ADD(" k_limit %d rows_only %d pair_next %d in_rec %d out_rec %d vc %d,%d,%d:", o->k_limit, o->rows_only, o->pair_next, o->in_rec, o->out_rec, o->vc_n, o->vc_run, o->vc_shift);
    for (int q = 0; q < o->vc_n && q < 3; q++) ADD(" %d", o->vc_t[q]);
    ADD(" add %d %a %a %a seg %d up %d:", o->add_t, (double)o->add_s_conv, (double)o->add_s_other, (double)o->add_inv, o->nseg, o->seg_up);
    for (int q = 0; q < o->nseg && q < 4; q++) ADD(" %d/%d", o->seg_t[q], o->seg_c[q]);
    ADD(" chain %d:", o->chain_n);
    for (int q = 0; q < o->chain_n && q < 3; q++) ADD(" %d", o->chain_out[q]);
    ADD(" cs %a f %a %a %a", (double)o->cs, (double)o->f0, (double)o->f1, (double)o->f2);
    ADD(" w_off %zd b_off %zd lut_off %zd lut2_off %zd s_off %zd w2_off %zd rows %d planes %d w3_off %zd stem %d blob %zd %zd", (ssize_t)o->w_off, (ssize_t)o->b_off,
        (ssize_t)o->lut_off, (ssize_t)o->lut2_off, (ssize_t)o->s_off, (ssize_t)o->w2_off, o->w2_rows, o->w2_planes, (ssize_t)o->w3_off, o->w3_stem, (ssize_t)o->w_blob_off[0],
        (ssize_t)o->w_blob_off[1]);
    ADD(" post_next %d", o->post_next);
    if (o->post_next) ADD(" %zd", (ssize_t)o->post_w_off);
    ADD(" split_next %d", o->split_next);
    if (o->split_next) ADD(" %zd", (ssize_t)o->split_w_off);
    ADD(" split_chain %d", o->split_chain);
    if (o->split_chain) ADD(" %zd", (ssize_t)o->chain_w_off);
    ADD(" pair_both %d both_chain %d both_elide %d", o->pair_both, o->both_chain, o->both_elide);
    ADD(" pre %d", o->pre);
    if (o->pre) ADD(" %zd %zd %zd %a", (ssize_t)o->pre_w_off, (ssize_t)o->pre_b_off, (ssize_t)o->pre_lut2_off, (double)o->pre_cs);
    ADD(" macs %a bytes %a prof_kind %d", o->macs, o->bytes, o->prof_kind);
#undef ADD
    return k;
}

size_t mars_hip_describe_plan(const void *data, size_t size, unsigned flags, char *out, size_t cap) {
    static const char *const kinds[] = {"conv_i8", "conv_f32", "relu_bytes", "lut_i8", "binary_i8", "sigmoid_f32", "binary_f32", "relu_f32", "bn",
                                        "maxpool", "concat_slice", "upsample", "upsample_q", "maxpool_q", "concat_q", "conv_f32_vhead", "fail"};
    mars_model_ext_t *m = NULL;
    const int full = (flags & MARS_HIP_DESCRIBE_FULL) != 0;
    if (load_host(data, size, flags & ~MARS_HIP_DESCRIBE_FULL, &m) != MARS_OK) return 0;
    size_t n = 0;
    char line[4096];
#define EMIT() do { const size_t l = strlen(line); if (out && n < cap) memcpy(out + n, line, n + l <= cap ? l : cap - n); n += l; } while (0)
    for (int i = 0; i < m->n_ops; i++) {
        const mars_op_t *o = &m->ops[i];
        int k = snprintf(line, sizeof line, "op %d layer %d %s in", i, o->layer, o->kind >= 0 && o->kind <= OP_FAIL ? kinds[o->kind] : "?");
        for (int q = 0; q < o->n_in && q < 4; q++) k += snprintf(line + k, sizeof line - (size_t)k, " %d", o->t_in[q]);
        k += snprintf(line + k, sizeof line - (size_t)k, " out %d", o->t_out);
#define FLAG(cond, ...) if (cond) k += snprintf(line + k, sizeof line - (size_t)k, __VA_ARGS__)
        FLAG(o->kind == OP_CONV_I8 || o->kind == OP_CONV_F32 || o->kind == OP_CONV_F32_VHEAD, " k%dx%d s%d c%d->%d", o->kh, o->kw, o->sw, o->in_c, o->out_c);
        FLAG(o->nchw, " relayout"); FLAG(o->out_nchw, " planar_store"); FLAG(o->lut_off != NO_OFF, " lut"); FLAG(o->add_t, " add=%d", o->add_t - 1);
        FLAG(o->nseg, " seg=%d", o->nseg); FLAG(o->pair_next && !(o->pair_both && o->nseg), " pair_next");  FLAG(o->pair_both, " pair_both"); FLAG(o->both_chain, " both_chain=%d", o->both_chain); FLAG(o->both_elide, " both_elide"); FLAG(o->post_next, " post_next"); FLAG(o->split_next, " split_next"); FLAG(o->pre, " pre"); FLAG(o->silu_f32, " silu");
        FLAG(o->k_limit, " k_limit=%d", o->k_limit); FLAG(o->in_rec, " in_rec=%d", o->in_rec); FLAG(o->out_rec, " out_rec");
        FLAG(o->vc_shift, " view=-%d", o->vc_shift); FLAG(o->vc_n, " vcat=%dx%d", o->vc_n, o->vc_run);
        FLAG(o->rows_only, " rows_only=%d", o->rows_only); FLAG(o->out_byte_off, " out_off=%zu", o->out_byte_off); FLAG(o->chain_n, " chain=%d", o->chain_n);
        FLAG(o->out_pix_stride, " pix_stride=%d", o->out_pix_stride); FLAG(o->kind == OP_FAIL, " err=%d", o->err);
#undef FLAG
        if (full) k = describe_op_full(o, line, sizeof line, k);
        snprintf(line + k, sizeof line - (size_t)k, "\n");
        EMIT();
    }
    for (uint32_t t = 0; t < m->pub.header.num_tensors; t++) {
        const mtensor_t *mt = &m->mt[t];
        const int listed = mt->nhwc_c || mt->partial || mt->zero_from || mt->rec_c || mt->pix_stride;
        if (!listed && !(full && mt->needed)) continue;
        int k = listed ? snprintf(line, sizeof line, "tensor %u nhwc_c %d pitch %d partial %d zero_from %zu rec_c %d pix_stride %d", t, mt->nhwc_c, mt->nhwc_pitch,
                                  mt->partial, mt->zero_from, mt->rec_c, mt->pix_stride)
                       : snprintf(line, sizeof line, "+tensor %u", t);
        if (full)
            k += snprintf(line + k, sizeof line - (size_t)k, " | bytes %zu extent %zu needed %d tail_read %d weight %d io %d,%d pix_c %d rec_hw %d nhwc_hw %d", mt->bytes,
                          mt->extent, mt->needed, mt->tail_read, mt->is_weight, mt->io_in, mt->io_out, mt->pix_c, mt->rec_hw, mt->nhwc_hw);
        snprintf(line + k, sizeof line - (size_t)k, "\n");
        EMIT();
    }
    if (full) {
        const plan_switches_t *w = &m->sw;
        snprintf(line, sizeof line, "+plan n_ops %d arena_size %zu scratch_per_frame %zu blob_mirror_bytes %zu rec_max_frames %zu rec_skipped %d f32_mode %d | fusion %d"
                 " no_fuse_lut %d no_nhwc_internal %d no_vconcat_q %d no_pair_f32 %d no_rec %d no_zero_tail %d no_vconcat_f32 %d no_rowpad %d no_post %d no_split %d no_chain %d no_both %d no_both_chain %d rec_limit %zu"
                 " vconcat_limit %zu bottleneck_limit %zu\n", m->n_ops, m->arena_size, m->scratch_per_frame, m->blob_mirror_bytes, m->rec_max_frames, m->rec_skipped,
                 m->plan_f32_mode, w->fusion, w->no_fuse_lut, w->no_nhwc_internal, w->no_vconcat_q, w->no_pair_f32, w->no_rec, w->no_zero_tail, w->no_vconcat_f32,
                 w->no_rowpad, w->no_post, w->no_split, w->no_chain, w->no_both, w->no_both_chain, w->rec_limit, w->vconcat_limit, w->bottleneck_limit);
        EMIT();
    }
#undef EMIT
    if (out && cap) out[n < cap ? n : cap - 1] = 0;
    mars_free(&m->pub);
    return n;
}

int mars_yolo_find_heads(const void *data, size_t size, int *tensor_ids, int *strides, int *num_classes, int cap) {
    mars_model_ext_t *m = NULL;
    if (load_host(data, size, 0, &m) != MARS_OK) return -1;
    const int n = mars_find_heads(m, tensor_ids, strides, num_classes, cap);
    mars_free(&m->pub);
    return n;
}

int mars_yolo_find_dfl_heads(const void *data, size_t size, int *box_ids, int *cls_ids, int *strides, int *num_classes, int *reg_max, int cap) {
    mars_model_ext_t *m = NULL;
    if (load_host(data, size, 0, &m) != MARS_OK) return -1;
    const int n = mars_find_dfl_heads(m, box_ids, cls_ids, strides, num_classes, reg_max, cap);
    mars_free(&m->pub);
    return n;
}

mars_error_t mars_load_memory(const void *data, size_t size, mars_model_t **model) {
    return mars_hip_load_memory_ex(data, size, 0, model);
}

mars_error_t mars_load_file(const char *path, mars_model_t **model) {
    if (!path || !model) return MARS_ERR_INVALID_FILE;
    FILE *fp = fopen(path, "rb");
    if (!fp) {
        fprintf(stderr, "Mars: Cannot open %s\n", path);
        return MARS_ERR_INVALID_FILE;
    }
    fseek(fp, 0, SEEK_END);
    long size = ftell(fp);
    fseek(fp, 0, SEEK_SET);
    if (size <= 0) { fclose(fp); return MARS_ERR_INVALID_FILE; }
    void *buf = malloc((size_t)size);
    if (!buf) { fclose(fp); return MARS_ERR_ALLOC_FAILED; }
    if (fread(buf, 1, (size_t)size, fp) != (size_t)size) { free(buf); fclose(fp); return MARS_ERR_INVALID_FILE; }
    fclose(fp);
    mars_error_t err = mars_load_memory(buf, (size_t)size, model);
    free(buf);
    return err;
}

mars_runtime_tensor_t *mars_get_input(mars_model_t *model, int index) {
    if (!model || index < 0 || (uint32_t)index >= model->header.num_inputs) return NULL;
    uint32_t tid = model->header.input_tensor_ids[index];
    if (tid >= model->header.num_tensors) return NULL;
    return &model->tensors[tid];
}

mars_runtime_tensor_t *mars_get_output(mars_model_t *model, int index) {
    if (!model || index < 0 || (uint32_t)index >= model->header.num_outputs) return NULL;
    uint32_t tid = model->header.output_tensor_ids[index];
    if (tid >= model->header.num_tensors) return NULL;
    return &model->tensors[tid];
}

int mars_get_num_inputs(mars_model_t *model) { return model ? (int)model->header.num_inputs : 0; }
int mars_get_num_outputs(mars_model_t *model) { return model ? (int)model->header.num_outputs : 0; }

void mars_print_summary(mars_model_t *model) {
    if (!model) return;
    mars_model_ext_t *m = (mars_model_ext_t *)model;
    printf("\nMars model summary (MI355X)\n");
    printf("Layers: %u\n", model->header.num_layers);
    printf("Tensors: %u\n", model->header.num_tensors);
    printf("Inputs: %u\n", model->header.num_inputs);
    printf("Outputs: %u\n", model->header.num_outputs);
    printf("Weights: %zu bytes\n", model->weights_size);
    printf("Launches per run: %d, batch %d, activations %zu bytes, parameters %zu bytes\n\n", m->n_ops, m->batch,
           m->act_bytes, m->arena_size);
}
```

thingino-accel_amd/csrc/host/mars_plan.c:

```c
#include <math.h>
#include <stdio.h>
#include <stdlib.h>
#include <string.h>
#include <time.h>

#include "mars_internal.h"
#include "nna.h"

int32_t mars_trunc_x86(float x) {
    if (x >= -2147483648.0f && x < 2147483648.0f) return (int32_t)x;
    return INT32_MIN;
}
static int sat8(int32_t v) { return v > 127 ? 127 : (v < -128 ? -128 : v); }
static int q_half_up(float v) { return sat8(mars_trunc_x86(v + 0.5f)); }

size_t elem_size(uint32_t dtype) {
    switch (dtype) {
        case MARS_DTYPE_FLOAT32: case MARS_DTYPE_INT32: return 4;
        case MARS_DTYPE_INT16: return 2;
        default: return 1;
    }
}

size_t shape_numel(const mars_tensor_t *d) {
// ... 565 lines not shown
static void lut2_from_lut(mars_model_ext_t *m, mars_op_t *c, const int8_t *tab) {
    if (!mhip_conv_i8_lut2_ok(c->cs)) return;
    int8_t tab2[512];
    for (int k = -256; k < 256; k++) {
        int r = k >= 0 ? (k + 1) >> 1 : -((1 - k) >> 1);
        const int lo = c->relu ? 0 : -128;
        r = r < lo ? lo : (r > 127 ? 127 : r);
        tab2[k + 256] = tab[r + 128];
    }
    c->lut2_off = arena_reserve(m, 512);
    if (c->lut2_off != NO_OFF) memcpy(m->arena_host + c->lut2_off, tab2, 512);
}

static void conv_i8_geometry(const mars_op_t *op, int frames, mhip_conv_i8_t *p) {
    memset(p, 0, sizeof(*p));
    p->frames = frames;
    p->in_c = op->in_c; p->in_h = op->in_h; p->in_w = op->in_w;
    p->out_h = op->out_h; p->out_w = op->out_w; p->out_c = op->store_c ? op->store_c : op->out_c;
    p->kh = op->kh; p->kw = op->kw; p->stride_h = op->sh; p->stride_w = op->sw; p->pad_top = op->pt; p->pad_left = op->pl;
    p->row_pad = op->row_pad; p->oc_pad = op->oc_pad; p->safe = op->safe;
    p->out_pix_stride = op->out_pix_stride; p->out_ch_off = op->out_ch_off;
}
int conv_i8_pre_fits(const mars_op_t *op, int frames, size_t in_stride, size_t out_stride) {
    mhip_conv_i8_t p;
    conv_i8_geometry(op, frames, &p);
    p.in_stride = in_stride; p.out_stride = out_stride;
    p.pre_w = (const int8_t *)op; p.pre_bias = (const int32_t *)op; p.pre_lut2 = (const uint8_t *)op; p.lut2 = (const uint8_t *)op;
    p.lut = (const uint8_t *)op;
    return mhip_conv_i8_pre_ok(&p);
}

typedef struct { const mars_model_ext_t *m; int frames, live; } rec_ctx_t;
static uint8_t *rec_addr(const rec_ctx_t *c, int ti) {
    if (c->live) return tdev(c->m, ti);
    return ti >= 0 ? (uint8_t *)c->m->mt + ti : NULL;
}
static size_t rec_stride(const rec_ctx_t *c, int ti) { return c->live ? tstride(c->m, ti) : ti >= 0 ? planned_stride(&c->m->mt[ti]) : 0; }
static const uint8_t *rec_param(const rec_ctx_t *c, size_t off, int image) {
    if (!c->live) return image || off != NO_OFF ? (const uint8_t *)c->m->mt : NULL;
    return off != NO_OFF ? c->m->arena_dev + off : NULL;
}
static void conv_i8_record(const rec_ctx_t *c, const mars_op_t *op, int unwritten, mhip_conv_i8_t *p) {
    conv_i8_geometry(op, c->frames, p);
    p->in = (const int8_t *)rec_addr(c, op->t_in[0]); p->in_stride = rec_stride(c, op->t_in[0]);
    p->out = (int8_t *)rec_addr(c, op->t_out); p->out_stride = rec_stride(c, op->t_out);
    if (c->live && p->in) p->in += op->in_byte_off;
    if (c->live && p->out) p->out += op->out_byte_off;
    p->w = (const int8_t *)rec_param(c, op->w_off, 0);
    p->bias = (const int32_t *)rec_param(c, op->b_off, 0);
    p->lut = rec_param(c, op->lut_off, 0);
    p->lut2 = op->lut_off != NO_OFF ? rec_param(c, op->lut2_off, 0) : NULL;
    p->w_rgb = !op->w2_rows ? (const int8_t *)rec_param(c, op->w2_off, 0) : NULL;
    p->w_rows = op->w2_rows ? (const int8_t *)rec_param(c, op->w2_off, 0) : NULL;
    if (op->pre) {
        p->pre_w = (const int8_t *)rec_param(c, op->pre_w_off, 0);
        p->pre_bias = (const int32_t *)rec_param(c, op->pre_b_off, 0);
        p->pre_lut2 = rec_param(c, op->pre_lut2_off, 0);
        p->pre_cs = op->pre_cs;
    }
    p->cs = op->cs; p->relu = op->relu; p->out_nchw = op->out_nchw;
    p->variant = op->variant;
    if (unwritten && op->t_out >= 0) p->out_stride = planned_stride(&c->m->mt[op->t_out]);
    if (op->add_t && (!c->live || rec_stride(c, op->add_t - 1) == p->out_stride)) {
        p->add = (const int8_t *)rec_addr(c, op->add_t - 1);
        p->add_s_conv = op->add_s_conv; p->add_s_other = op->add_s_other; p->add_inv = op->add_inv;
    }
    p->nseg = op->nseg;
    p->seg_up = op->seg_up;
    int c0 = 0;
    for (int k = 0; k < 4; k++) {
        p->seg_c0[k] = 0x7fffffff;
        if (k < op->nseg) {
            p->seg_in[k] = (const int8_t *)rec_addr(c, op->seg_t[k]);
            p->seg_stride[k] = rec_stride(c, op->seg_t[k]);
            p->seg_c[k] = op->seg_c[k];
            p->seg_c0[k] = c0;
            c0 += op->seg_c[k];
        }
    }
    if (op->nseg > 1) p->in = p->seg_in[0];
}
void conv_i8_group_records(const mars_model_ext_t *m, int form, const mars_op_t *g[4], int side, int frames, int live, mhip_conv_i8_t *p) {
    const rec_ctx_t c = {m, frames, live};
    const int patch = form == FORM_POST || form == FORM_SPLIT || form == FORM_SPLIT_CHAIN;
    conv_i8_record(&c, g[0], patch, &p[0]);
    if (!patch) {
        for (int k = 1; k < form_span(form); k++) conv_i8_record(&c, g[k], 0, &p[k]);
        return;
    }
    if (form == FORM_POST) {
        const mars_op_t *cv3 = g[1];
        p->post_w = (const int8_t *)rec_param(&c, g[0]->post_w_off, 1);
        p->post_lut2 = rec_param(&c, cv3->lut2_off, 0);
        p->post_cs = cv3->cs;
        p->post_in = (const int8_t *)rec_addr(&c, cv3->seg_t[1]); p->post_in_stride = rec_stride(&c, cv3->seg_t[1]);
        p->post_out = (int8_t *)rec_addr(&c, cv3->t_out); p->post_out_stride = rec_stride(&c, cv3->t_out);
        if (live && p->post_out) p->post_out += cv3->out_byte_off;
        p->post_out_pix_stride = cv3->out_pix_stride; p->post_out_ch_off = cv3->out_ch_off;
        return;
    }
    p->split_w = (const int8_t *)rec_param(&c, g[0]->split_w_off, 1);
    for (int k = 0; k < 2; k++) {
        p->split_lut2[k] = rec_param(&c, g[1 + k]->lut2_off, 0);
        p->split_cs[k] = g[1 + k]->cs;
        p->split_out[k] = (int8_t *)rec_addr(&c, g[1 + k]->t_out); p->split_out_stride[k] = rec_stride(&c, g[1 + k]->t_out);
    }
    if (form == FORM_SPLIT_CHAIN) {
        p->chain_side = side;
        p->chain_w = (const int8_t *)rec_param(&c, g[0]->chain_w_off, 1);
        p->chain_lut2 = rec_param(&c, g[3]->lut2_off, 0);
        p->chain_cs = g[3]->cs;
        p->chain_out = (int8_t *)rec_addr(&c, g[3]->t_out); p->chain_out_stride = rec_stride(&c, g[3]->t_out);
    }
}
int conv_i8_group_fits(const mars_model_ext_t *m, int form, const mars_op_t *g[4], int side, int frames) {
    mhip_conv_i8_t p[3];
    const int tile = form == FORM_BOTH || form == FORM_BOTH_CHAIN;
    for (int k = 0; k < form_span(form); k++)
        if (g[k]->t_out < 0 || (tile && g[k]->nchw)) return 0;
    if ((!tile && g[0]->t_in[0] < 0) || ((form == FORM_BOTH_CHAIN || form == FORM_SPLIT_CHAIN) && side != 1 && side != 2)) return 0;
    conv_i8_group_records(m, form, g, side, frames, 0, p);
    switch (form) {
        case FORM_POST: return mhip_conv_i8_post_ok(&p[0]);
        case FORM_SPLIT: case FORM_SPLIT_CHAIN: return mhip_conv_i8_split_ok(&p[0]);
        case FORM_BOTH: return mhip_conv_i8_both_ok(&p[0], &p[1]);
        case FORM_BOTH_CHAIN: return mhip_conv_i8_both_chain_ok(&p[0], &p[1], &p[2], side);
        default: return 0;
    }
}

static int match_silu(const mars_model_ext_t *m, int i, int f32, const int *readers, const int *writers, int q[3], int *fwd) {
    const mars_op_t *c = &m->ops[i], *s = c + 1, *mu = c + 2;
    if (c->kind != (f32 ? OP_CONV_F32 : OP_CONV_I8) || s->kind != (f32 ? OP_SIGMOID_F32 : OP_LUT_I8) || mu->kind != (f32 ? OP_BINARY_F32 : OP_BINARY_I8) || !mu->is_mul)
        return 0;
    if (!f32 && m->pub.layers[s->layer].desc.type != MARS_LAYER_SIGMOID) return 0;
    const int q1 = q[0] = c->t_out, q2 = q[1] = s->t_out, q3 = q[2] = mu->t_out;
    if (s->t_in[0] != q1 || q1 == q2 || q2 == q3 || q1 == q3) return 0;
    *fwd = mu->t_in[0] == q1 && mu->t_in[1] == q2;
    if (!*fwd && !(mu->t_in[0] == q2 && mu->t_in[1] == q1)) return 0;
    if (f32 ? q3 == c->t_in[0] || m->mt[q3].is_weight : op_reads(c, q3)) return 0;
    if (readers[q1] != 2 || readers[q2] != 1 || writers[q1] != 1 || writers[q2] != 1 || writers[q3] != 1) return 0;
    if (m->mt[q1].io_out || m->mt[q2].io_out || m->mt[q1].io_in || m->mt[q2].io_in) return 0;
    const size_t n1 = (size_t)c->out_h * c->out_w * c->out_c;
    return s->n == n1 && mu->n == n1;
}

void fold_silu(mars_model_ext_t *m, int f32) {
    int *readers, *writers;
    if (!use_counts(m, &readers, &writers)) return;
    for (int i = 0; i + 2 < m->n_ops; i++) {
        mars_op_t *c = &m->ops[i];
        int q[3], fwd;
        if (!match_silu(m, i, f32, readers, writers, q, &fwd)) continue;
        const size_t n1 = (size_t)c->out_h * c->out_w * c->out_c;
        if (f32) {
            c->silu_f32 = 1;
        } else {
            const mars_tensor_t *d1 = &m->pub.tensors[q[0]].desc, *d2 = &m->pub.tensors[q[1]].desc, *d3 = &m->pub.tensors[q[2]].desc;
            int8_t tab[256];
            for (int v = -128; v < 128; v++) {
                int sg = sigmoid_q(v, d1->scale, d2->scale);
                tab[v + 128] = (int8_t)(fwd ? binary_q(1, v, sg, d1->scale, d2->scale, d3->scale)
                                            : binary_q(1, sg, v, d2->scale, d1->scale, d3->scale));
            }
            c->lut_off = lut_i8(m, tab);
            lut2_from_lut(m, c, tab);
        }
        c->t_out = q[2];
        touch(m, q[2], n1 * (f32 ? 4 : 1));
        m->mt[q[0]].needed = 0;
        m->mt[q[1]].needed = 0;
        memmove(&m->ops[i + 1], &m->ops[i + 3], (size_t)(m->n_ops - i - 3) * sizeof(mars_op_t));
        m->n_ops -= 2;
    }
    free(readers);
}

void fuse_lut(mars_model_ext_t *m) {
    if (m->sw.no_fuse_lut) return;
    int *readers, *writers;
    if (!use_counts(m, &readers, &writers)) return;
    for (int i = 0; i + 1 < m->n_ops; i++) {
        mars_op_t *c = &m->ops[i], *s = &m->ops[i + 1];
        if (c->kind != OP_CONV_I8 || s->kind != OP_LUT_I8 || c->lut_off != NO_OFF || s->lut_off == NO_OFF) continue;
        const int q1 = c->t_out, q2 = s->t_out;
        if (q1 < 0 || q2 < 0 || s->t_in[0] != q1 || q1 == q2) continue;
        if (op_reads(c, q2)) continue;
        if (readers[q1] != 1 || writers[q1] != 1 || writers[q2] != 1 || m->mt[q1].io_out || m->mt[q1].io_in || m->mt[q1].is_weight || m->mt[q2].is_weight) continue;
        const size_t n1 = (size_t)c->out_h * c->out_w * c->out_c;
        if (s->n != n1 || m->mt[q2].bytes < n1) continue;
        if (m->pub.tensors[q1].desc.dtype != MARS_DTYPE_INT8 || m->pub.tensors[q2].desc.dtype != MARS_DTYPE_INT8) continue;
        c->lut_off = s->lut_off;
        lut2_from_lut(m, c, (const int8_t *)(m->arena_host + s->lut_off));
        c->t_out = q2;
        touch(m, q2, n1);
        m->mt[q1].needed = 0;
        memmove(&m->ops[i + 1], &m->ops[i + 2], (size_t)(m->n_ops - i - 2) * sizeof(mars_op_t));
        m->n_ops -= 1;
    }
    free(readers);
}

void elide_concat(mars_model_ext_t *m) {
    int *readers, *writers;
    if (!use_counts(m, &readers, &writers)) return;
    for (int i = 0; i < m->n_ops; i++) {
// ... 359 lines not shown
    for (int i = 0; i + 1 < m->n_ops; i++) {
        mars_op_t *a = &m->ops[i], *b = &m->ops[i + 1];
        if (a->kind != OP_CONV_I8 || b->kind != OP_CONV_I8 || a->pre || b->pre || !op_plain(m, i) || !op_plain(m, i + 1) || op_is_mate(m, i)) continue;
        const int c = a->out_c, T = a->t_out, O = b->t_out;
        if ((c != 32 && c != 64) || a->oc_pad != c || a->kh * a->kw < 2 || a->sh != 1 || a->sw != 1 || !a->safe || a->nchw || a->out_nchw || a->nseg ||
            a->out_pix_stride || a->out_ch_off || a->store_c || a->chain_n || a->in_byte_off || a->out_byte_off || a->lut_off == NO_OFF ||
            a->lut2_off == NO_OFF || a->n_in >= 4)
            continue;
        if (b->kh != 1 || b->kw != 1 || b->sh != 1 || b->sw != 1 || b->pt || b->pl || !b->safe || b->nchw || b->out_nchw || b->add_t || b->chain_n ||
            b->store_c || b->in_byte_off || b->lut_off == NO_OFF || b->lut2_off == NO_OFF || b->nseg != 2 || b->seg_up || b->seg_t[0] != T ||
            b->seg_c[0] != c || b->seg_c[1] != c || b->in_c != 2 * c || b->out_c != 2 * c || b->oc_pad != 2 * c || b->row_pad != 2 * c ||
            b->in_h != a->out_h || b->in_w != a->out_w || b->out_h != a->out_h || b->out_w != a->out_w)
            continue;
        const int Y = b->seg_t[1];
        if (T < 0 || O < 0 || Y < 0 || Y == T || O == T || O == Y || readers[T] != 1 || writers[T] != 1 || m->mt[T].io_in || m->mt[T].io_out ||
            m->mt[T].is_weight || m->mt[T].tail_read || m->mt[Y].is_weight || m->mt[Y].pix_stride ||
            m->mt[Y].bytes != (size_t)a->out_h * a->out_w * c || op_reads(a, O) || op_reads(a, Y))
            continue;
        const mars_op_t *g[4] = {a, b};
        if (!conv_i8_group_fits(m, FORM_POST, g, 0, 1)) continue;
        const size_t bytes = mhip_conv_i8_post_pack(c, NULL, NULL, NULL);
        const size_t off = arena_reserve(m, bytes);
        if (off == NO_OFF) break;
        mhip_conv_i8_post_pack(c, (const int8_t *)(m->arena_host + b->w_off), b->b_off != NO_OFF ? (const int32_t *)(m->arena_host + b->b_off) : NULL,
                               (int8_t *)(m->arena_host + off));
        a->post_next = 1;
        a->post_w_off = off;
        a->t_in[a->n_in++] = Y;
        m->mt[T].needed = 0;
        readers[T] = 0;
        readers[Y]++;
        i++;
    }
    free(readers);
}

static int free_1x1_ok(const mars_op_t *d, const mars_op_t *a, int in_c, int out_c) {
    return d->kind == OP_CONV_I8 && d->kh == 1 && d->kw == 1 && d->sh == 1 && d->sw == 1 && !d->pt && !d->pl && d->safe && !d->nchw && !d->out_nchw && !d->add_t &&
           !d->chain_n && !d->store_c && !d->in_byte_off && !d->out_byte_off && !d->out_pix_stride && !d->out_ch_off && d->lut_off != NO_OFF &&
           d->lut2_off != NO_OFF && !d->nseg && !d->pre && d->n_in == 1 && d->in_c == in_c && d->out_c == out_c && d->oc_pad == out_c && d->row_pad == in_c &&
           d->in_h == a->out_h && d->in_w == a->out_w && d->out_h == a->out_h && d->out_w == a->out_w;
}
void fuse_split(mars_model_ext_t *m) {
    if (m->sw.no_split || m->no_split) return;
    int *readers, *writers;
    if (!use_counts(m, &readers, &writers)) return;
    for (int i = 0; i + 2 < m->n_ops; i++) {
        mars_op_t *a = &m->ops[i], *b = &m->ops[i + 1], *c = &m->ops[i + 2];
        int gi[4];
        if (a->kind != OP_CONV_I8 || a->pre || !op_plain(m, i) || op_form(m, i + 1, gi) != FORM_PAIR || !op_plain(m, i + 2) || op_is_mate(m, i)) continue;
        const int T = a->t_out;
        if (a->out_c != 64 || a->oc_pad != 64 || a->kh * a->kw < 2 || (a->sh != 1 && a->sh != 2) || a->sw != a->sh || !a->safe || a->nchw || a->out_nchw ||
            a->nseg || a->out_pix_stride || a->out_ch_off || a->store_c || a->chain_n || a->in_byte_off || a->out_byte_off || a->add_t ||
            a->lut_off == NO_OFF || a->lut2_off == NO_OFF || a->n_in != 1)
            continue;
        if (T < 0 || !free_1x1_ok(b, a, 64, 32) || !free_1x1_ok(c, a, 64, 32) || b->t_in[0] != T || c->t_in[0] != T) continue;
        const int O0 = b->t_out, O1 = c->t_out;
        if (O0 < 0 || O1 < 0 || O0 == O1 || O0 == T || O1 == T || readers[T] != 2 || writers[T] != 1 || m->mt[T].io_in || m->mt[T].io_out ||
            m->mt[T].is_weight || m->mt[T].tail_read || m->mt[O0].pix_stride || m->mt[O1].pix_stride || op_reads(a, O0) || op_reads(a, O1))
            continue;
        const mars_op_t *g[4] = {a, b, c};
        if (!conv_i8_group_fits(m, FORM_SPLIT, g, 0, 1)) continue;
        const size_t bytes = mhip_conv_i8_split_pack(NULL, NULL, NULL, NULL, NULL);
        const size_t off = arena_reserve(m, bytes);
        if (off == NO_OFF) break;
        mhip_conv_i8_split_pack((const int8_t *)(m->arena_host + b->w_off), b->b_off != NO_OFF ? (const int32_t *)(m->arena_host + b->b_off) : NULL,
                                (const int8_t *)(m->arena_host + c->w_off), c->b_off != NO_OFF ? (const int32_t *)(m->arena_host + c->b_off) : NULL,
                                (int8_t *)(m->arena_host + off));
        a->split_next = 1;
        a->split_w_off = off;
        m->mt[T].needed = 0;
        i += 2;
    }
    free(readers);
}

static void move_up(mars_model_ext_t *m, int to, int from) {
    const mars_op_t moved = m->ops[from];
    memmove(&m->ops[to + 1], &m->ops[to], sizeof(mars_op_t) * (size_t)(from - to));
    m->ops[to] = moved;
}

static int find_chained_1x1(const mars_model_ext_t *m, int i, int form, int c, const int *writers, int *side_out) {
    const int n = form_span(form) - 1, O0 = m->ops[i + n - 2].t_out, O1 = m->ops[i + n - 1].t_out;
    const mars_op_t *a = &m->ops[i], *g[4] = {a, a + 1, a + 2, NULL};
    for (int j = i + n; j < m->n_ops && j <= i + 48; j++) {
        const mars_op_t *d = &m->ops[j];
        if (!free_1x1_ok(d, a, c, c) || !op_plain(m, j) || op_is_mate(m, j)) continue;
        const int side = d->t_in[0] == O0 ? 1 : (d->t_in[0] == O1 ? 2 : 0), O = d->t_out;
        if (!side || O < 0 || O == O0 || O == O1 || O == a->t_out || writers[O] != 1 || m->mt[O].io_in || m->mt[O].is_weight || m->mt[O].pix_stride || op_reads(d, O))
            continue;
        int reads = 0;
        for (int k = 0; k < n; k++) reads |= op_reads(&a[k], O);
        if (reads || touched_between(m, i + n, j, O, USE_READ | USE_WRITE) || touched_between(m, i + n, j, d->t_in[0], USE_WRITE)) continue;
        g[n] = d;
        if (!conv_i8_group_fits(m, form, g, side, 1)) continue;
        *side_out = side;
        return j;
    }
    return -1;
}

void fuse_split_chain(mars_model_ext_t *m) {
    if (m->sw.no_chain || m->no_chain || m->sw.no_split || m->no_split) return;
    int *readers, *writers, g[4];
    if (!use_counts(m, &readers, &writers)) return;
    for (int i = 0; i + 3 < m->n_ops; i += op_span(m, i)) {
        mars_op_t *a = &m->ops[i];
        if (a->kind != OP_CONV_I8 || op_form(m, i, g) != FORM_SPLIT) continue;
        int side;
        const int j = find_chained_1x1(m, i, FORM_SPLIT_CHAIN, 32, writers, &side);
        if (j < 0) continue;
        const size_t bytes = mhip_conv_i8_chain_pack(NULL, NULL, NULL);
        const size_t off = arena_reserve(m, bytes);
        if (off == NO_OFF) break;
        move_up(m, i + 3, j);
        const mars_op_t *d = &m->ops[i + 3];
        mhip_conv_i8_chain_pack((const int8_t *)(m->arena_host + d->w_off), d->b_off != NO_OFF ? (const int32_t *)(m->arena_host + d->b_off) : NULL,
                                (int8_t *)(m->arena_host + off));
        a->split_chain = side;
        a->chain_w_off = off;
    }
    free(readers);
}

void fuse_both_chain(mars_model_ext_t *m) {
    if (m->sw.no_both_chain || m->no_both_chain || m->sw.no_both || m->no_both) return;
    int *readers, *writers, g[4];
    if (!use_counts(m, &readers, &writers)) return;
    for (int i = 0; i + 2 < m->n_ops; i += op_span(m, i)) {
        mars_op_t *a = &m->ops[i];
        if (a->kind != OP_CONV_I8 || op_form(m, i, g) != FORM_BOTH || a->in_byte_off || a[1].in_byte_off || a->out_byte_off || a[1].out_byte_off) continue;
        int side;
        const int j = find_chained_1x1(m, i, FORM_BOTH_CHAIN, 64, writers, &side);
        if (j < 0) continue;
        move_up(m, i + 2, j);
        a->both_chain = side;
        const int S = a[side - 1].t_out;
        if (readers[S] == 1 && writers[S] == 1 && !m->mt[S].io_in && !m->mt[S].io_out && !m->mt[S].is_weight && !m->mt[S].tail_read) {
            a->both_elide = 1;
            m->mt[S].needed = 0;
        }
    }
    free(readers);
}

void pad_output_rows(mars_model_ext_t *m) {
    for (uint32_t i = 0; i < m->pub.header.num_tensors; i++) m->mt[i].pix_c = m->mt[i].pix_stride = 0;
    if (m->sw.no_rowpad) return;
    for (int i = 0; i < m->n_ops; i++) {
        mars_op_t *o = &m->ops[i];
        if (o->kind != OP_CONV_I8 || o->out_nchw || o->out_pix_stride || o->out_ch_off || o->add_t || o->t_out < 0 ||
            (o->out_c & 15) == 0 || (o->in_c & 15) != 0)
            continue;
        mtensor_t *t = &m->mt[o->t_out];
        const int P = (o->out_c + 15) & ~15;
        const size_t px = (size_t)o->out_h * o->out_w;
        if (!t->io_out || t->io_in || P > o->oc_pad || t->bytes != px * (size_t)o->out_c || (px * P) % 256 != 0) continue;
        if (touched_by_other(m, o->t_out, i, i)) continue;
        o->out_pix_stride = P;
        o->store_c = P;
        t->pix_c = o->out_c;
        t->pix_stride = P;
        if (px * P > t->extent) t->extent = px * P;
    }
}

void virtual_concat(mars_model_ext_t *m) {
    const int nt = (int)m->pub.header.num_tensors;
    for (int T = 0; T < nt; T++) {
        const mtensor_t *mt = &m->mt[T];
        if (mt->is_weight || mt->io_in || mt->io_out) continue;
        int sl[4], ns = 0, bad = 0, first_reader = -1, last_reader = -1, last_slice = -1;
        for (int i = 0; i < m->n_ops && !bad; i++) {
            const mars_op_t *o = &m->ops[i];
            if (o->t_out == T) {
                if (o->kind != OP_CONCAT_SLICE || ns >= 4) bad = 1;
                else { sl[ns++] = i; last_slice = i; }
            }
            for (int k = 0; k < o->n_in; k++)
                if (o->t_in[k] == T) {
                    if (o->kind != OP_CONV_I8 || k != 0 || o->n_in != 1 || o->nchw || o->kh != 1 || o->kw != 1 || o->sh != 1 ||
                        o->sw != 1 || o->pt || o->pl || !o->safe || o->nseg || (o->out_c & 15) || o->in_h != o->out_h ||
                        o->in_w != o->out_w || (o->in_c & (o->in_c - 1)) != 0 || o->add_t)
                        bad = 1;
                    if (first_reader < 0) first_reader = i;
                    last_reader = i;
                }
        }
        if (bad || ns < 2 || first_reader < 0 || last_slice > first_reader) continue;
        for (int a = 0; a < ns; a++)
            for (int b = a + 1; b < ns; b++)
                if (m->ops[sl[b]].ch_off < m->ops[sl[a]].ch_off) { int t = sl[a]; sl[a] = sl[b]; sl[b] = t; }
        int c = 0;
        const mars_op_t *s0 = &m->ops[sl[0]];
        for (int a = 0; a < ns && !bad; a++) {
            const mars_op_t *o = &m->ops[sl[a]];
            if (o->ch_off != c || (o->in_c & 31) || o->out_h != s0->out_h || o->out_w != s0->out_w || o->out_c != s0->out_c ||
                o->t_in[0] == T || o->t_in[0] < 0)
                bad = 1;
            c += o->in_c;
            if (!bad && touched_between(m, sl[a] + 1, last_reader + 1, o->t_in[0], USE_WRITE)) bad = 1;
        }
        if (bad || c != s0->out_c) continue;
// ... 347 lines not shown
        }
        memmove(&m->ops[rl + 1 + heads], &m->ops[rl + 1], sizeof(mars_op_t) * (size_t)(m->n_ops - rl - 1));
        m->n_ops += heads;
        for (int q = 0; q < heads; q++) {
            mars_op_t *x = &m->ops[r1 + q], *h = &m->ops[rl + 1 + q];
            const double hw = (double)x->in_h * x->in_w;
            x->t_in[0] = TL;
            x->vc_shift = (int)sB;
            x->k_limit = (int)km;
            x->macs = hw * x->out_c * (double)km;
            x->bytes = (hw * (double)km + hw * x->out_c) * 4.0;
            *h = *x;
            h->kind = OP_CONV_F32_VHEAD;
            h->pair_next = 0; h->vc_shift = 0;
            h->k_limit = (int)km + 1;
            h->vc_n = N - 1; h->vc_run = Wb / 4;
            h->n_in = N;
            for (int k = 0; k < N - 1; k++) { h->vc_t[k] = firsts[k]; h->t_in[1 + k] = firsts[k]; }
            h->macs = (double)(sB / 4) * x->out_c * (double)(km + 1);
            h->bytes = ((double)(sB / 4) * (double)(km + 1) + (double)(sB / 4) * x->out_c) * 4.0;
            h->variant = 0;
            h->w3_off = wt_off[q]; h->w3_stem = 0;
            h->w2_off = NO_OFF; h->w2_planes = 0;
        }
        memmove(&m->ops[first_op], &m->ops[e + 1], sizeof(mars_op_t) * (size_t)(m->n_ops - e - 1));
        m->n_ops -= N;
        m->mt[T].needed = 0;
        m->mt[T].partial = 1;
        m->mt[T].zero_from = 0;
        i = first_op - 1;
    }
}

void f32_policy(mars_model_ext_t *m) {
    const int nt = (int)m->pub.header.num_tensors;
    unsigned char *hot = (unsigned char *)calloc((size_t)nt + 1, 1);
    if (!hot) {
        for (int i = 0; i < m->n_ops; i++) m->ops[i].f32_exact = 1;
        return;
    }
    for (int i = m->n_ops - 1; i >= 0; i--) {
        mars_op_t *o = &m->ops[i];
        int reach = 0;
        if (o->kind == OP_MAXPOOL && o->t_in[0] >= 0 && m->pub.tensors[o->t_in[0]].desc.dtype == MARS_DTYPE_FLOAT32) reach = 1;
        if (o->kind == OP_RELU_BYTES && o->t_out >= 0) {
            hot[o->t_out] = 1;
            continue;
        }
        if (o->t_out >= 0 && hot[o->t_out]) reach = 1;
        for (int k = 0; k < o->chain_n; k++)
            if (o->chain_out[k] >= 0 && hot[o->chain_out[k]]) reach = 1;
        if (!reach) continue;
        for (int k = 0; k < o->n_in; k++)
            if (o->t_in[k] >= 0) hot[o->t_in[k]] = 1;
        if (o->kind == OP_CONV_F32) o->f32_exact = 1;
    }
    free(hot);
}

void plan_check(mars_model_ext_t *m) {
    for (int i = 0; i < m->n_ops; i++) {
        const mars_op_t *o = &m->ops[i];
        const char *why = NULL;
        const mars_op_t *M[4];
        int g[4], gg[4];
        op_form(m, i, g);
        for (int k = 0; k < 4; k++) M[k] = g[k] >= 0 ? &m->ops[g[k]] : NULL;
        if (o->kind == -1) why = "a dead op is left";
        else if (o->n_in < 0 || o->n_in > 4 || o->nseg < 0 || o->nseg > 4 || o->chain_n < 0 || o->chain_n > 3 || o->vc_n < 0 || o->vc_n > 3) why = "an operand count is out of range";
        else if (o->add_t && !op_reads(o, o->add_t - 1)) why = "add_t is not among t_in";
        else if (o->chain_n && o->t_out != o->chain_out[o->chain_n - 1]) why = "t_out is not the chain's last stage";
        else if (o->pair_next && (!M[1] || M[1]->kind != o->kind)) why = "pair_next without a mate of its kind";
        else if (o->pair_both && (!o->pair_next || o->kind != OP_CONV_I8 || (o->out_c != 64 && o->out_c != 128) || M[1]->out_c != o->out_c)) why = "pair_both without a pair of 64- or 128-channel sides";
        else if (o->kind == OP_CONV_I8 && o->pair_next && o->nseg && !o->pair_both) why = "a side-by-side pair over a virtual concat";
        else if (o->post_next && (o->kind != OP_CONV_I8 || !M[1] || M[1]->kind != OP_CONV_I8 || M[1]->nseg != 2 || M[1]->seg_t[0] != o->t_out || !op_reads(o, M[1]->seg_t[1])))
            why = "post_next without its 1x1 behind it, or y2 is not among t_in";
        else if (o->split_next && (o->kind != OP_CONV_I8 || !M[2] || M[1]->kind != OP_CONV_I8 || M[2]->kind != OP_CONV_I8 || op_form(m, g[1], gg) != FORM_PAIR || !op_plain(m, g[2]) ||
                                   M[1]->n_in != 1 || M[2]->n_in != 1 || M[1]->t_in[0] != o->t_out || M[2]->t_in[0] != o->t_out || o->post_next || o->pair_next || o->pre || o->add_t))
            why = "split_next without its pair of 1x1s behind it";
        else if (o->split_chain && (!o->split_next || !M[3] || !free_1x1_ok(M[3], o, 32, 32) || !op_plain(m, g[3]) || (o->split_chain != 1 && o->split_chain != 2) ||
                                    M[3]->t_in[0] != M[o->split_chain]->t_out || M[3]->t_out < 0 || M[3]->t_out == M[1]->t_out || M[3]->t_out == M[2]->t_out ||
                                    M[3]->t_out == o->t_out || m->mt[M[3]->t_out].pix_stride || o->chain_w_off == NO_OFF))
            why = "split_chain without its 1x1 behind the pair";
        else if (o->both_chain && (!o->pair_both || !M[2] || !free_1x1_ok(M[2], o, 64, 64) || !op_plain(m, g[2]) || (o->both_chain != 1 && o->both_chain != 2) ||
                                   M[2]->t_in[0] != M[o->both_chain - 1]->t_out || M[2]->t_out < 0 || M[2]->t_out == o->t_out || M[2]->t_out == M[1]->t_out))
            why = "both_chain without its 1x1 behind the pair";
        else if (o->both_elide && (!o->both_chain || m->mt[M[o->both_chain - 1]->t_out].needed || m->mt[M[o->both_chain - 1]->t_out].io_out))
            why = "both_elide on a side that is kept";
        for (int k = 0; !why && k < o->nseg; k++)
            if (!op_reads(o, o->seg_t[k])) why = "a seg_t is not among t_in";
        for (int k = 0; !why && k < o->vc_n; k++)
            if (!op_reads(o, o->vc_t[k])) why = "a vc_t is not among t_in";
        if (!why) continue;
        VLOG("plan_check: op %d (layer %d, kind %d): %s\n", i, o->layer, o->kind, why);
        m->plan_err = MARS_ERR_LAYER_FAILED;
        return;
    }
}
```

thingino-accel_amd/csrc/host/mars_run.c:

```c
#include <math.h>
#include <stdio.h>
#include <stdlib.h>
#include <string.h>
#include <time.h>

#include "mars_internal.h"
#include "nna.h"

static int g_graph_max_batch = 8;
static unsigned g_tune_gen = 1;
static int g_dual_min_batch = 64;
static int g_dual_ways = 2;
static void conv_i8_params(const mars_model_ext_t *m, const mars_op_t *op, mhip_conv_i8_t *p) {
    const mars_op_t *g[4] = {op};
    conv_i8_group_records(m, FORM_PLAIN, g, 0, m->run_frames, 1, p);
}

static void conv_f32_params(mars_model_ext_t *m, mars_op_t *op, mhip_conv_f32_t *p) {
    const int B = m->run_frames;
    uint8_t *A = m->arena_dev;
    memset(p, 0, sizeof(*p));
    p->in = (const float *)tdev(m, op->t_in[0]); p->in_stride = tstride(m, op->t_in[0]);
    p->out = (float *)tdev(m, op->t_out); p->out_stride = tstride(m, op->t_out);
    p->w = (const float *)(A + op->w_off);
// ... 175 lines not shown
mars_error_t mars_hip_run_device_async(mars_model_t *model) {
    if (!model) return MARS_ERR_INVALID_FILE;
    tune_push((mars_model_ext_t *)model);
    mars_error_t e = run_device_async(model);
    tune_pop((mars_model_ext_t *)model);
    return e;
}

static mars_error_t run_device_async(mars_model_t *model) {
    mars_model_ext_t *m = (mars_model_ext_t *)model;
    if (!m->act_dev || !m->arena_dev) return MARS_ERR_NNA_INIT_FAILED;
    int graphable = g_graph_max_batch > 0 && m->batch <= g_graph_max_batch && !m->profiling && !m->pipe;
    for (int i = 0; i < m->n_ops && graphable; i++)
        if (m->ops[i].kind == OP_FAIL) graphable = 0;
    if (!graphable) return enqueue_plan(model);
    if (m->graph_exec && m->graph_gen != g_tune_gen) {
        drop_graph(m);
        m->ran_plain = 0;
    }
    if (!m->graph_exec) {
        if (!m->ran_plain) {
            mars_error_t e = enqueue_plan(model);
            if (e == MARS_OK) m->ran_plain = 1;
            return e;
        }
        if (m->tail_pending) {
            mhip_select_stream(0);
            if (mhip_stream_wait(0, m->ev_tail_done)) return MARS_ERR_LAYER_FAILED;
            m->tail_pending = 0;
        }
        if (mhip_graph_begin() == 0) {
            mars_error_t e = enqueue_plan(model);
            m->graph_exec = mhip_graph_end(e == MARS_OK);
            m->graph_gen = g_tune_gen;
            if (e != MARS_OK) { m->graph_exec = NULL; return e; }
        }
        VLOG("plan of %d launches at batch %d %s\n", m->n_ops, m->batch, m->graph_exec ? "captured into a HIP graph" : "could not be captured");
        if (!m->graph_exec) {
            g_graph_max_batch = 0;
            return enqueue_plan(model);
        }
    }
    if (m->tail_pending) {
        mhip_select_stream(0);
        if (mhip_stream_wait(0, m->ev_tail_done)) return MARS_ERR_LAYER_FAILED;
        m->tail_pending = 0;
    }
    if (mhip_graph_launch(m->graph_exec)) return MARS_ERR_LAYER_FAILED;
    for (uint32_t i = 0; i < model->header.num_layers; i++) model->layers[i].is_executed = true;
    return MARS_OK;
}

static mars_error_t enqueue_range(mars_model_ext_t *m, int sid, int wait_tail) {
    void *prof_last = NULL;
    mhip_select_stream(sid);
    m->scratch_t = -1;
    for (int i = 0; i < m->n_ops; i++) {
        mars_op_t *op = &m->ops[i];
        if (op->kind == OP_FAIL) {
            fprintf(stderr, "Mars: Layer %d execution failed\n", op->layer);
            return (mars_error_t)op->err;
        }
        int g[4];
        const int form = op_form(m, i, g), span = op_span(m, i);
        const mars_op_t *mem[4] = {op, NULL, NULL, NULL};
        for (int q = 1; q < span; q++) mem[q] = &m->ops[g[q]];
        for (int q = 0; q < span && wait_tail; q++) {
            const int t = mem[q]->t_out;
            if (t < 0 || !(m->mt[t].io_out || m->mt[t].tail_read)) continue;
            mhip_stream_wait(sid, m->ev_tail_done);
            wait_tail = 0;
        }
        if (m->profiling) {
            if (!op->ev1) op->ev1 = mhip_event_create();
            if (!prof_last) {
                if (!op->ev0) op->ev0 = mhip_event_create();
                mhip_event_record(op->ev0);
                prof_last = op->ev0;
            }
            op->ev_start = prof_last;
        }
        int rc;
        switch (form) {
            case FORM_POST: case FORM_SPLIT: case FORM_SPLIT_CHAIN: {
                mhip_conv_i8_t p;
                conv_i8_group_records(m, form, mem, op->split_chain, m->run_frames, 1, &p);
                rc = mhip_conv_i8(&p);
                break;
            }
            case FORM_PAIR_F32: {
                mhip_conv_f32_t pa, pb;
                conv_f32_params(m, op, &pa);
                conv_f32_params(m, &m->ops[g[1]], &pb);
                rc = mhip_conv_f32_pair(&pa, &pb);
                break;
            }
            case FORM_PAIR: case FORM_BOTH: case FORM_BOTH_CHAIN: {
                mhip_conv_i8_t p[3];
                conv_i8_group_records(m, form, mem, op->both_chain, m->run_frames, 1, p);
                rc = form == FORM_PAIR ? mhip_conv_i8_pair(&p[0], &p[1]) : form == FORM_BOTH ? mhip_conv_i8_both(&p[0], &p[1])
                                       : mhip_conv_i8_both_chain(&p[0], &p[1], &p[2], op->both_chain, op->both_elide);
                if (form == FORM_BOTH_CHAIN && rc == -2) rc = -1;
                break;
            }
            case FORM_BAD: rc = -1; break;
            default: rc = launch_op(m, op);
        }
        if (rc == -2 && (form == FORM_PAIR || form == FORM_BOTH || form == FORM_PAIR_F32)) {
            rc = launch_op(m, op);
            if (!rc) rc = launch_op(m, &m->ops[g[1]]);
        }
        i += span - 1;
        for (int q = 0; q < span; q++)
            if (op_writes(mem[q], m->scratch_t)) m->scratch_t = -1;
        if (m->profiling) {
            const int nx = i + 1;
            const int end = m->profiling != 2 || nx >= m->n_ops || m->ops[nx].prof_kind != op->prof_kind;
            op->prof_rec = end;
            if (end) {
                mhip_event_record(op->ev1);
                prof_last = op->ev1;
            }
        }
        if (rc != 0) {
            fprintf(stderr, "Mars: Layer %d launch failed: %s\n", op->layer, mhip_last_error());
            return MARS_ERR_LAYER_FAILED;
        }
    }
    return MARS_OK;
}

static mars_error_t enqueue_plan(mars_model_t *model) {
    mars_model_ext_t *m = (mars_model_ext_t *)model;
    for (uint32_t i = 0; i < model->header.num_layers; i++) model->layers[i].is_executed = false;
    const int B = m->batch;
    int dual = g_dual_min_batch > 0 && B >= g_dual_min_batch && B >= 2 && !m->profiling &&
               !(g_graph_max_batch > 0 && B <= g_graph_max_batch);
    if (dual) {
        if (!m->ev_fork) m->ev_fork = mhip_event_create_sync();
        for (int k = 0; k < 3; k++) {
            if (!m->ev_join[k]) m->ev_join[k] = mhip_event_create_sync();
            if (!m->ev_join[k]) dual = 0;
        }
        if (!m->ev_fork) dual = 0;
    }
    mars_error_t e;
    if (!dual) {
        m->frame0 = 0; m->run_frames = B;
        e = enqueue_range(m, 0, m->tail_pending);
    } else {
        const int ways = g_dual_ways < B ? g_dual_ways : B;
        mhip_select_stream(0);
        int rc = mhip_event_record(m->ev_fork);
        for (int k = 1; k < ways && !rc; k++) rc = mhip_stream_wait(3 + k, m->ev_fork);
        if (rc) return MARS_ERR_LAYER_FAILED;
        e = MARS_OK;
        int f0 = 0;
        for (int k = 0; k < ways && e == MARS_OK; k++) {
            const int n = (B - f0 + (ways - k) - 1) / (ways - k);
            m->frame0 = f0; m->run_frames = n;
            e = enqueue_range(m, k ? 3 + k : 0, m->tail_pending);
            f0 += n;
        }
        for (int k = 1; k < ways; k++) {
            mhip_select_stream(3 + k);
            rc = mhip_event_record(m->ev_join[k - 1]);
            if (!rc) rc = mhip_stream_wait(0, m->ev_join[k - 1]);
// ... 488 lines not shown
```

thingino-accel_amd/csrc/mhip.h:

```cpp
#ifndef MHIP_H
#define MHIP_H

#include <stddef.h>
#include <stdint.h>

#ifdef __cplusplus
extern "C" {
#endif

int mhip_init(int device_hint);
void mhip_shutdown(void);
int mhip_ready(void);
int mhip_device_info(int *cu_count, int *lds_bytes, int *gfx_version, size_t *hbm_bytes);
void *mhip_stream(void);
int mhip_sync(void);
void mhip_select_aux(int on);
void mhip_select_stream(int which);
int mhip_stream_wait(int which, void *ev);
int mhip_event_sync(void *ev);
void *mhip_malloc(size_t bytes);
void mhip_free(void *p);
void *mhip_host_alloc(size_t bytes);
void mhip_host_free(void *p);
int mhip_memset_async(void *dst, int value, size_t bytes);
int mhip_h2d_async(void *dst, const void *src, size_t bytes);
int mhip_d2h_async(void *dst, const void *src, size_t bytes);
int mhip_d2d_async(void *dst, const void *src, size_t bytes);
int mhip_h2d_2d_async(void *dst, size_t dpitch, const void *src, size_t spitch, size_t row_bytes, size_t rows);
int mhip_d2h_2d_async(void *dst, size_t dpitch, const void *src, size_t spitch, size_t row_bytes, size_t rows);
void *mhip_event_create(void);
void *mhip_event_create_sync(void);
void mhip_event_destroy(void *ev);
int mhip_event_record(void *ev);
float mhip_event_elapsed_ms(void *start, void *stop);
const char *mhip_last_error(void);
int mhip_graph_begin(void);
void *mhip_graph_end(int ok);
int mhip_graph_launch(void *exec);
void mhip_graph_destroy(void *exec);

typedef struct {
    const int8_t *in;  size_t in_stride;
    int8_t *out;       size_t out_stride;
    const int8_t *w;
    const int32_t *bias;
    const uint8_t *lut;
    const uint8_t *lut2;
    const int8_t *pre_w;
    const int32_t *pre_bias;
    const uint8_t *pre_lut2;
    float pre_cs;
    const int8_t *w_rgb;
    const int8_t *w_rows;
    int frames;
    int in_h, in_w, in_c;
    int out_h, out_w, out_c;
    int kh, kw, stride_h, stride_w, pad_top, pad_left;
    int row_pad;
    int oc_pad;
    float cs;
    int relu;
    int out_nchw;
    int in_planar;
    int safe;
    int out_pix_stride;
    int out_ch_off;
    int variant;
    const int8_t *add;
    float add_s_conv, add_s_other, add_inv;
    int nseg;
    const int8_t *seg_in[4];
    size_t seg_stride[4];
    int seg_c[4], seg_c0[4];
    int seg_up;
    const int8_t *post_w;
    const uint8_t *post_lut2;
    float post_cs;
    const int8_t *post_in;  size_t post_in_stride;
    int8_t *post_out;       size_t post_out_stride;
    int post_out_pix_stride, post_out_ch_off;
    const int8_t *split_w;
    const uint8_t *split_lut2[2];
    float split_cs[2];
    int8_t *split_out[2];   size_t split_out_stride[2];
    int chain_side;
    const int8_t *chain_w;
    const uint8_t *chain_lut2;
    float chain_cs;
    int8_t *chain_out;      size_t chain_out_stride;
} mhip_conv_i8_t;
int mhip_conv_i8_split_ok(const mhip_conv_i8_t *p);
size_t mhip_conv_i8_split_pack(const int8_t *packed0, const int32_t *bias0, const int8_t *packed1, const int32_t *bias1, int8_t *out);
int mhip_conv_i8_split_row(int side, int oc);
size_t mhip_conv_i8_chain_pack(const int8_t *packed, const int32_t *bias, int8_t *out);
int mhip_conv_i8_chain_k(int c);
int mhip_conv_i8_post_ok(const mhip_conv_i8_t *p);
size_t mhip_conv_i8_post_pack(int c, const int8_t *packed, const int32_t *bias, int8_t *out);
int mhip_conv_i8_post_k(int c, int k);
int mhip_conv_i8_post_row(int c, int oc);
int mhip_conv_i8_oc_row(int oc, int oc_pad);
int mhip_conv_i8_pre_ok(const mhip_conv_i8_t *p);
size_t mhip_conv_i8_rgb_pack(int in_c, int kh, int kw, int stride_h, int stride_w, int pad_left, int oc_pad, int k64,
                             const int8_t *packed, int8_t *out);
size_t mhip_conv_i8_rows_pack(int in_c, int kh, int kw, int stride_h, int stride_w, int oc_pad, int k64, int out_w,
                              const int8_t *packed, int8_t *out);
unsigned long mhip_conv_i8_rows_launches(void);
int mhip_conv_i8_is_safe(float cs);
int mhip_conv_i8_lut2_ok(float cs);
int mhip_conv_i8_tune(const char *key, int value);
int mhip_conv_i8_tune_get(const char *key, int *value);
int mhip_conv_i8_variants(const mhip_conv_i8_t *p, int *codes, int max);
int mhip_conv_i8_seg_ok(const mhip_conv_i8_t *p);
int mhip_conv_i8_pair(const mhip_conv_i8_t *a, const mhip_conv_i8_t *b);
int mhip_conv_i8_both_ok(const mhip_conv_i8_t *a, const mhip_conv_i8_t *b);
int mhip_conv_i8_both(const mhip_conv_i8_t *a, const mhip_conv_i8_t *b);
int mhip_conv_i8_both_chain_ok(const mhip_conv_i8_t *a, const mhip_conv_i8_t *b, const mhip_conv_i8_t *d, int side);
int mhip_conv_i8_both_chain(const mhip_conv_i8_t *a, const mhip_conv_i8_t *b, const mhip_conv_i8_t *d, int side, int elide);
int mhip_conv_i8_small_c(int in_c, int kw, int out_c);
void mhip_conv_i8_pack_geom(int in_c, int kw, int out_c, int *row_pad, int *oc_pad, int *c_eff);
int mhip_conv_i8(const mhip_conv_i8_t *p);

typedef struct {
    const float *in;  size_t in_stride;
    float *out;       size_t out_stride;
    const float *w;   const float *bias;
    const void *w_split;
    const void *w_patch;
    int frames;
    int in_h, in_w, in_c, out_h, out_w, out_c;
    int kh, kw, stride_h, stride_w, pad_top, pad_left;
    int silu;
    const float *add; size_t add_stride;
    int use_mfma;
    int k_limit;
    int k_limit_required;
    int in_rec, out_rec;
} mhip_conv_f32_t;
int mhip_conv_f32(const mhip_conv_f32_t *p);
size_t mhip_conv_f32_vcat_pack(int out_c, int in_c, int planes, const float *w, float *out);
int mhip_conv_f32_vcat_head(const mhip_conv_f32_t *p, const float *w_t, const float *const *first, const size_t *first_strides, int n_first, int run_floats);
int mhip_conv_f32_pair(const mhip_conv_f32_t *a, const mhip_conv_f32_t *b);
unsigned long mhip_conv_f32_pair_launches(void);
size_t mhip_conv_f32_split_pack(int out_c, int in_c, int kh, int kw, int stride_w, int planes, const float *w, void *out);
unsigned long mhip_conv_f32_split_launches(void);
int mhip_conv_f32_split_takes(int out_c, int in_c, int kh, int kw, int stride_h, int stride_w, int pad_left, int in_w, int out_w);
size_t mhip_conv_f32_patch_pack(int out_c, int in_c, int kh, int kw, int stride, int pad, int in_h, int in_w, int out_h, int out_w,
                                const float *w, void *out);
size_t mhip_conv_f32_patch_pack2(int out_c, int in_c, int kh, int kw, int stride, int pad, int in_h, int in_w, int out_h, int out_w,
                                 int rec, const float *w, void *out);
int mhip_conv_f32_patch_geom2(int out_c, int in_c, int kh, int kw, int stride, int pad, int in_h, int in_w, int out_h, int out_w,
                              int rec, int *outv, int cap);
unsigned long mhip_conv_f32_prec_launches(void);
unsigned long mhip_conv_f32_recin_launches(void);
int mhip_conv_f32_patch_rec_form(int out_c, int in_c, int kh, int kw, int stride, int pad, int in_h, int in_w, int out_h, int out_w);
int mhip_conv_f32_patch_geom(int out_c, int in_c, int kh, int kw, int stride, int pad, int in_h, int in_w, int out_h, int out_w,
                             int *outv, int cap);
unsigned long mhip_conv_f32_patch_launches(void);
size_t mhip_conv_f32_stem_pack(int out_c, int in_c, int kh, int kw, int stride, int pad, int in_h, int in_w, int out_h, int out_w,
                               const float *w, void *out);
unsigned long mhip_conv_f32_stem_launches(void);
int mhip_conv_f32_mode(int set);

int mhip_lut_i8(const int8_t *in, size_t in_stride, int8_t *out, size_t out_stride, int frames,
                size_t n, const uint8_t *lut_dev);
int mhip_relu_bytes(int8_t *buf, size_t stride, int frames, size_t n);
int mhip_binary_i8(int is_mul, const int8_t *a, size_t a_stride, const int8_t *b, size_t b_stride,
                   int8_t *out, size_t out_stride, int frames, size_t n, float sa, float sb, float inv_so,
                   int out_run, int out_pix_stride, int out_ch_off);
int mhip_sigmoid_f32(const float *in, size_t in_stride, float *out, size_t out_stride, int frames, size_t n);
int mhip_binary_f32(int op , const float *a, size_t a_stride, const float *b,
                    size_t b_stride, float *out, size_t out_stride, int frames, size_t n);
int mhip_relu_f32(const float *in, size_t in_stride, float *out, size_t out_stride, int frames,
                  size_t n, float alpha);
// ... 419 lines not shown
```

Baseline: 60920.

## Fuse following 1x1 conv into patch conv epilogue as NEXT form

```diff
diff --git a/thingino-accel_amd/csrc/hip/conv_i8.hip b/thingino-accel_amd/csrc/hip/conv_i8.hip
--- a/thingino-accel_amd/csrc/hip/conv_i8.hip
+++ b/thingino-accel_amd/csrc/hip/conv_i8.hip
@@ -1304,7 +1304,7 @@
             if (n < max && conv_i8_patch_ok(p, th, nullptr)) codes[n++] = th == 16 ? 10 : (th == 8 ? 9 : 11);
         return n;
     }
-    if (p->split_w) {
+    if (p->split_w || p->next_w) {
         for (int th : {16, 8, 4})
             if (n < max && conv_i8_patch_ok(p, th, nullptr)) codes[n++] = th == 16 ? 10 : (th == 8 ? 9 : 11);
         return n;
@@ -1422,6 +1422,19 @@
         }
         return conv_i8_launch_patch(p, k64, th);
     }
+    if (p->next_w) {
+        if (!mhip_zero_page() || (p->in_c % 16) != 0 || !mhip_conv_i8_next_ok(p)) return -1;
+        int th = conv_i8_next_tile_rows(p);
+        const int code = p->variant ? p->variant : tune().variant;
+        if (code >= 9 && code <= 11) {
+            const int want = code == 10 ? 16 : (code == 9 ? 8 : 4);
+            if (conv_i8_patch_ok(p, want, nullptr)) th = want;
+        } else if (tune().small_batch && conv_i8_patch_ok(p, 4, nullptr) &&
+                   ((long)p->frames * p->out_h * p->out_w + 255) / 256 * ((p->oc_pad + 127) / 128) < tune().few_wgs) {
+            th = 4;
+        }
+        return conv_i8_launch_patch(p, k64, th);
+    }
     if ((p->in_c % 16) == 0) {
         if (!mhip_zero_page()) return -1;
         const int nks = k64 / BK;
diff --git a/thingino-accel_amd/csrc/hip/conv_i8_common.hpp b/thingino-accel_amd/csrc/hip/conv_i8_common.hpp
--- a/thingino-accel_amd/csrc/hip/conv_i8_common.hpp
+++ b/thingino-accel_amd/csrc/hip/conv_i8_common.hpp
@@ -458,6 +458,7 @@
 int conv_i8_pre_tile_rows(const mhip_conv_i8_t *p);
 int conv_i8_post_tile_rows(const mhip_conv_i8_t *p);
 int conv_i8_split_tile_rows(const mhip_conv_i8_t *p);
+int conv_i8_next_tile_rows(const mhip_conv_i8_t *p);
 bool conv_i8_rows_ok(const mhip_conv_i8_t *p);
 int conv_i8_launch_rows(const mhip_conv_i8_t *p);
 int conv_i8_try_rgb(const mhip_conv_i8_t *p, int k64);
diff --git a/thingino-accel_amd/csrc/hip/conv_i8_patch.hip b/thingino-accel_amd/csrc/hip/conv_i8_patch.hip
--- a/thingino-accel_amd/csrc/hip/conv_i8_patch.hip
+++ b/thingino-accel_amd/csrc/hip/conv_i8_patch.hip
@@ -41,7 +41,7 @@
     asm volatile("s_waitcnt lgkmcnt(0)\n\ts_barrier" ::: "memory");
 }
 
-template <int TH, int BN, bool HAS_LUT, bool PRE = false, bool POST = false, bool SPLIT = false, bool CHAIN = false>
+template <int TH, int BN, bool HAS_LUT, bool PRE = false, bool POST = false, bool SPLIT = false, bool CHAIN = false, bool NEXT = false>
 __global__ __launch_bounds__(NTHREADS) void conv_i8_patch(const mhip_conv_i8_t p, const int k64, const int tiles_x,
                                                           const int tiles_y, const unsigned ntiles_all, const int PH,
                                                           const int PW, const int PWP, const int PWH, const int nblk,
@@ -59,7 +59,8 @@
     constexpr int NPO = 2 * BN;
     static_assert(!SPLIT || (BN == 64 && HAS_LUT && !PRE && !POST), "SPLIT: one 64-channel tile, no other stage");
     static_assert(!CHAIN || SPLIT, "CHAIN: a stage of the SPLIT form");
-    constexpr int LB = LUTB + ((PRE || POST) ? 512 : 0) + (SPLIT ? 1024 : 0) + (CHAIN ? 512 : 0);
+    static_assert(!NEXT || (HAS_LUT && !PRE && !POST && !SPLIT), "NEXT: no other stage");
+    constexpr int LB = LUTB + ((PRE || POST || NEXT) ? 512 : 0) + (SPLIT ? 1024 : 0) + (CHAIN ? 512 : 0);
     int *dutab = (int *)(dynlds + LB);
     int8_t *wl = dynlds + LB + ((nks * 16 + 255) & ~255);
     const int patch_bytes = nblk * 1024;
@@ -70,7 +71,9 @@
     const int *sbl = (const int *)(swl + 64 * BK);
     int8_t *cwl = swl + 64 * BK + 64 * 4;
     const int *cbl = (const int *)(cwl + 32 * BK);
-    int8_t *patch0 = w1l + (PRE ? p.in_c * BK : 0) + (POST ? NPO * NPO + NPO * 4 : 0) + (SPLIT ? 64 * BK + 64 * 4 : 0) + (CHAIN ? 32 * BK + 32 * 4 : 0);
+    int8_t *nwl = w1l;
+    const int *nbl = (const int *)(nwl + BN * BK);
+    int8_t *patch0 = w1l + (PRE ? p.in_c * BK : 0) + (POST ? NPO * NPO + NPO * 4 : 0) + (NEXT ? BN * BK + BN * 4 : 0) + (SPLIT ? 64 * BK + 64 * 4 : 0) + (CHAIN ? 32 * BK + 32 * 4 : 0);
     int8_t *tpatch = patch0 + ring * patch_bytes;
 
     const int tid = threadIdx.x, lane = tid & 63;
@@ -97,6 +100,10 @@
     if (POST) {
         if (tid >= 128) ((uint32_t *)slut)[tid] = ((const uint32_t *)p.post_lut2)[tid - 128];
         if (tid < NPO) ((int *)(pwl + NPO * NPO))[tid] = ((const int *)(p.post_w + NPO * NPO))[tid];
+    }
+    if (NEXT) {
+        if (tid >= 128) ((uint32_t *)slut)[tid] = ((const uint32_t *)p.next_lut2)[tid - 128];
+        if (tid < BN) ((int *)(nwl + BN * BK))[tid] = ((const int *)(p.next_w + BN * BK))[tid];
     }
     if (SPLIT) {
         if (tid >= 128) {
@@ -133,6 +140,8 @@
             for (int i = wv; i < NPO * NPO / 1024; i += 4) glds16(p.post_w + i * 1024 + lane * 16, pwl + i * 1024);
         if (SPLIT)
             glds16(p.split_w + wv * 1024 + lane * 16, swl + wv * 1024);
+        if (NEXT && wv < BN / 16)
+            glds16(p.next_w + wv * 1024 + lane * 16, nwl + wv * 1024);
         if (CHAIN && wv < 2)
             glds16(p.chain_w + wv * 1024 + lane * 16, cwl + wv * 1024);
     }
@@ -195,6 +204,8 @@
     const __amdgpu_buffer_rsrc_t orsrc1 = __builtin_amdgcn_make_buffer_rsrc(SPLIT ? p.split_out[1] : p.out, 0, (int)out_bytes1, 0x00020000);
     const unsigned out_bytes2 = CHAIN ? (unsigned)(p.frames - 1) * (unsigned)p.chain_out_stride + (unsigned)(p.out_h * p.out_w) * 32u : 0u;
     const __amdgpu_buffer_rsrc_t orsrc2 = __builtin_amdgcn_make_buffer_rsrc(CHAIN ? p.chain_out : p.out, 0, (int)out_bytes2, 0x00020000);
+    const unsigned out_bytesn = NEXT ? (unsigned)(p.frames - 1) * (unsigned)p.next_out_stride + (unsigned)(p.out_h * p.out_w) * (unsigned)BN : 0u;
+    const __amdgpu_buffer_rsrc_t orsrcn = __builtin_amdgcn_make_buffer_rsrc(NEXT ? p.next_out : p.out, 0, (int)out_bytesn, 0x00020000);
     const bool cside1 = CHAIN && p.chain_side == 2;
     const bool has_add = !SPLIT && p.add != nullptr;
     constexpr int RROW = WOC == 4 ? 1024 : 512;
@@ -203,7 +214,7 @@
     const int frow = lane & 15, fchunk = lane >> 4;
     const int chan = (lane >> 4) * (4 * WOC);
     const int NR = has_add || POST ? NRI : 0;
-    const int ntail = POST ? (has_add ? NRI : 0) + WPX * (NPO / 64) : (SPLIT ? (CHAIN ? 3 : 2) * WPX : NST);
+    const int ntail = POST ? (has_add ? NRI : 0) + WPX * (NPO / 64) : (SPLIT ? (CHAIN ? 3 : 2) * WPX : (NEXT ? 2 : 1) * NST);
     const int ppstride = p.post_out_pix_stride ? p.post_out_pix_stride : NPO;
     auto issue_rows = [&](const int8_t *base, size_t fstride, int tx, int ty, unsigned f) {
 #pragma unroll
@@ -429,7 +440,7 @@
                 }
             }
         }
-        uint32_t pku[POST || SPLIT ? WPX : 1][WOC];
+        uint32_t pku[POST || SPLIT || NEXT ? WPX : 1][WOC];
         if (POST && has_add) {
 #pragma unroll
             for (int u = 0; u < WPX; u++) {
@@ -465,11 +476,48 @@
                 for (int q = 0; q < WOC; q++) pku[SPLIT ? u : 0][q] = pk[q];
                 continue;
             }
+            if (NEXT) {
+#pragma unroll
+                for (int q = 0; q < WOC; q++) pku[NEXT ? u : 0][q] = pk[q];
+            }
             const int voff = voffs[u];
             if (WOC == 4)
                 __builtin_amdgcn_raw_buffer_store_b128((v4i){(int)pk[0], (int)pk[1], (int)pk[2], (int)pk[3]}, orsrc, voff, 0, 0);
             else if (WOC == 2)
                 __builtin_amdgcn_raw_buffer_store_b64((v2i){(int)pk[0], (int)pk[WOC > 1 ? 1 : 0]}, orsrc, voff, 0, 0);
+        }
+        if (NEXT) {
+            constexpr int NM = BN / 16;
+            v4i nw4[NM], nb4[NM];
+#pragma unroll
+            for (int r = 0; r < NM; r++) {
+                nw4[r] = *(const v4i *)(nwl + lds_off(r * 16 + frow, fchunk));
+                nb4[r] = *(const v4i *)(nbl + r * 16 + fchunk * 4);
+            }
+            v4i nc[WPX][NM];
+#pragma unroll
+            for (int u = 0; u < WPX; u++) {
+                const v4i b0 = {(int)pku[NEXT ? u : 0][0], (int)pku[NEXT ? u : 0][WOC > 1 ? 1 : 0], WOC == 4 ? (int)pku[NEXT ? u : 0][WOC > 2 ? 2 : 0] : 0,
+                                WOC == 4 ? (int)pku[NEXT ? u : 0][WOC > 3 ? 3 : 0] : 0};
+#pragma unroll
+                for (int r = 0; r < NM; r++) nc[u][r] = __builtin_amdgcn_mfma_i32_16x16x64_i8(nw4[r], b0, nb4[r], 0, 0, 0);
+            }
+            const int fon = (int)(f * (unsigned)p.next_out_stride) - (int)(f * (unsigned)p.out_stride);
+#pragma unroll
+            for (int u = 0; u < WPX; u++) {
+                int an[NM * 4];
+#pragma unroll
+                for (int r = 0; r < NM; r++)
+#pragma unroll
+                    for (int e = 0; e < 4; e++) an[r * 4 + e] = nc[u][r][e];
+                uint32_t pkn[NM];
+                requant_pack_pre<NM * 4>(an, p.next_cs, pkn);
+                const int voffn = voffs[u] >= 0 ? voffs[u] + fon : -1;
+                if (WOC == 4)
+                    __builtin_amdgcn_raw_buffer_store_b128((v4i){(int)pkn[0], (int)pkn[1], (int)pkn[NM > 2 ? 2 : 0], (int)pkn[NM > 3 ? 3 : 0]}, orsrcn, voffn, 0, 0);
+                else
+                    __builtin_amdgcn_raw_buffer_store_b64((v2i){(int)pkn[0], (int)pkn[1]}, orsrcn, voffn, 0, 0);
+            }
         }
         if (SPLIT) {
             v4i sw4[4], sb4[4];
@@ -637,10 +685,17 @@
             p->chain_out == p->split_out[1] || (long)(p->frames - 1) * (long)p->chain_out_stride + (long)p->out_h * p->out_w * 32 > 0x7fffffffL)
             return false;
     }
+    const bool next = p->next_w != nullptr;
+    if (next) {
+        if (pre || post || split || s != 1 || p->out_c != g->bn || p->oc_pad != g->bn || p->out_pix_stride || p->out_ch_off || !p->lut2 || !p->next_lut2 ||
+            !p->next_out || p->next_out == p->out || (long)(p->frames - 1) * (long)p->next_out_stride + (long)p->out_h * p->out_w * g->bn > 0x7fffffffL)
+            return false;
+    }
     const size_t pb = (size_t)g->nblk * 1024;
     const size_t radd = p->add || post ? (size_t)4 * (th / 4) * (g->bn == 64 ? 1024 : 512) : 0;
     const size_t fixed = LUTB + (pre ? 512 + (size_t)C * BK + pb : 0) + (post ? 512 + (size_t)4 * g->bn * g->bn + (size_t)8 * g->bn : 0) +
                          (split ? 1024 + (size_t)64 * BK + 64 * 4 : 0) + (chain ? 512 + (size_t)32 * BK + 32 * 4 : 0) +
+                         (next ? 512 + (size_t)g->bn * BK + (size_t)g->bn * 4 : 0) +
                          (((size_t)g->nks * 16 + 255) & ~(size_t)255) + (size_t)g->nks * g->bn * BK + radd;
     const size_t budget = patch_lds_budget(g->bn);
     if (fixed + pb > budget) return false;
@@ -660,9 +715,9 @@
 static inline long split_out_bytes(const mhip_conv_i8_t *p, int side) {
     return (long)(p->frames - 1) * (long)p->split_out_stride[side] + (long)p->out_h * p->out_w * 32;
 }
-template <int TH, int BN, bool HAS_LUT, bool PRE = false, bool POST = false, bool SPLIT = false, bool CHAIN = false>
+template <int TH, int BN, bool HAS_LUT, bool PRE = false, bool POST = false, bool SPLIT = false, bool CHAIN = false, bool NEXT = false>
 static int launch_patch_t(const mhip_conv_i8_t *p, int k64, const patch_geom_t &g) {
-    auto kern = conv_i8_patch<TH, BN, HAS_LUT, PRE, POST, SPLIT, CHAIN>;
+    auto kern = conv_i8_patch<TH, BN, HAS_LUT, PRE, POST, SPLIT, CHAIN, NEXT>;
     static int cus = 0;
     static size_t slots_lds[8];
     static int slots_n[8], nslots = 0;
@@ -729,6 +784,13 @@
         if (th == 8) return launch_patch_t<8, 64, true, false, false, true, true>(p, k64, g);
         return launch_patch_t<4, 64, true, false, false, true, true>(p, k64, g);
     }
+    if (p->next_w) {
+#define PATCH_NEXT(T, B) launch_patch_t<T, B, true, false, false, false, false, true>(p, k64, g)
+        if (th == 16) return g.bn == 64 ? PATCH_NEXT(16, 64) : PATCH_NEXT(16, 32);
+        if (th == 8) return g.bn == 64 ? PATCH_NEXT(8, 64) : PATCH_NEXT(8, 32);
+        return g.bn == 64 ? PATCH_NEXT(4, 64) : PATCH_NEXT(4, 32);
+#undef PATCH_NEXT
+    }
     if (p->split_w) {
         if (th == 16) return launch_patch_t<16, 64, true, false, false, true>(p, k64, g);
         if (th == 8) return launch_patch_t<8, 64, true, false, false, true>(p, k64, g);
@@ -786,6 +848,39 @@
     return bytes;
 }
 
+int conv_i8_next_tile_rows(const mhip_conv_i8_t *p) {
+    patch_geom_t g;
+    if (patch_geom(p, 16, &g)) return 16;
+    if (patch_geom(p, 8, &g) && g.ring >= 2) return 8;
+    for (int th : {8, 4})
+        if (patch_geom(p, th, &g)) return th;
+    return 0;
+}
+extern "C" int mhip_conv_i8_next_ok(const mhip_conv_i8_t *p) {
+    if (!p || !p->next_w || p->pre_w || p->post_w || p->split_w || p->chain_side || p->nseg > 1 || p->out_nchw) return 0;
+    return conv_i8_next_tile_rows(p) != 0;
+}
+extern "C" int mhip_conv_i8_next_k(int c, int k) { return c == 64 ? k : (k >> 3) * 16 + (k & 7); }
+extern "C" int mhip_conv_i8_next_row(int c, int oc) {
+    const int per = c / 4, g = oc / per, rem = oc - g * per;
+    return (rem >> 2) * 16 + g * 4 + (rem & 3);
+}
+extern "C" size_t mhip_conv_i8_next_pack(int c, const int8_t *packed, const int32_t *bias, int8_t *out) {
+    if (c != 32 && c != 64) return 0;
+    const size_t bytes = (size_t)c * BK + (size_t)c * 4;
+    if (!packed || !out) return bytes;
+    memset(out, 0, bytes);
+    for (int oc = 0; oc < c; oc++) {
+        const int R = mhip_conv_i8_next_row(c, oc), src = mhip_conv_i8_oc_row(oc, c);
+        for (int ch = 0; ch < c; ch++) {
+            const int k = mhip_conv_i8_next_k(c, ch);
+            out[(size_t)R * BK + ((((k >> 4) ^ ((R >> 1) & 2))) << 4) + (k & 15)] = packed[(size_t)src * 64 + ch];
+        }
+        ((int32_t *)(out + (size_t)c * BK))[R] = bias ? bias[src] : 0;
+    }
+    return bytes;
+}
+
 int conv_i8_split_tile_rows(const mhip_conv_i8_t *p) {
     patch_geom_t g;
     for (int th : {16, 8, 4})
diff --git a/thingino-accel_amd/csrc/host/mars_internal.h b/thingino-accel_amd/csrc/host/mars_internal.h
--- a/thingino-accel_amd/csrc/host/mars_internal.h
+++ b/thingino-accel_amd/csrc/host/mars_internal.h
@@ -87,6 +87,8 @@
     size_t split_w_off;
     int split_chain;
     size_t chain_w_off;
+    int next_1x1;
+    size_t next_w_off;
     size_t w2_off;
     int w2_rows;
     int w2_planes;
@@ -112,7 +114,7 @@
 typedef struct {
     int fusion;
     unsigned no_fuse_lut : 1, no_nhwc_internal : 1, no_vconcat_q : 1, no_pair_f32 : 1, no_rec : 1, no_zero_tail : 1, no_vconcat_f32 : 1,
-        no_rowpad : 1, no_post : 1, no_split : 1, no_chain : 1, no_both : 1, no_both_chain : 1;
+        no_rowpad : 1, no_post : 1, no_split : 1, no_chain : 1, no_both : 1, no_both_chain : 1, no_next : 1;
     size_t rec_limit;
     size_t vconcat_limit;
     size_t bottleneck_limit;
@@ -131,6 +133,7 @@
     int no_chain;
     int no_both;
     int no_both_chain;
+    int no_next;
     int rec_frames;
     int rec_skipped;
     size_t rec_max_frames;
@@ -224,13 +227,14 @@
     FORM_POST,
     FORM_SPLIT,
     FORM_SPLIT_CHAIN,
+    FORM_NEXT,
     FORM_PAIR_F32,
     FORM_BAD,
     FORM_COUNT
 };
 static inline int form_span(int form) {
     static const int span[FORM_COUNT] = {[FORM_PLAIN] = 1, [FORM_PAIR] = 2, [FORM_BOTH] = 2, [FORM_BOTH_CHAIN] = 3, [FORM_POST] = 2, [FORM_SPLIT] = 3,
-                                         [FORM_SPLIT_CHAIN] = 4, [FORM_PAIR_F32] = 2, [FORM_BAD] = 1};
+                                         [FORM_SPLIT_CHAIN] = 4, [FORM_NEXT] = 2, [FORM_PAIR_F32] = 2, [FORM_BAD] = 1};
     return form >= 0 && form < FORM_COUNT ? span[form] : 0;
 }
 static inline int op_form(const mars_model_ext_t *m, int i, int g[4]) {
@@ -238,6 +242,7 @@
     int form = FORM_PLAIN;
     if (o->split_next) form = o->split_chain ? FORM_SPLIT_CHAIN : FORM_SPLIT;
     else if (o->post_next) form = FORM_POST;
+    else if (o->next_1x1) form = FORM_NEXT;
     else if (o->pair_next) form = o->kind == OP_CONV_F32 ? FORM_PAIR_F32 : !o->pair_both ? FORM_PAIR : o->both_chain ? FORM_BOTH_CHAIN : FORM_BOTH;
     int span = form_span(form);
     if (i + span > m->n_ops) { form = FORM_BAD; span = m->n_ops - i; }
@@ -307,6 +312,7 @@
 MARS_INTERNAL void fuse_post(mars_model_ext_t *m);
 MARS_INTERNAL void fuse_split(mars_model_ext_t *m);
 MARS_INTERNAL void fuse_split_chain(mars_model_ext_t *m);
+MARS_INTERNAL void fuse_next(mars_model_ext_t *m);
 MARS_INTERNAL void pad_output_rows(mars_model_ext_t *m);
 MARS_INTERNAL void virtual_concat_q(mars_model_ext_t *m);
 MARS_INTERNAL void f32_policy(mars_model_ext_t *m);
diff --git a/thingino-accel_amd/csrc/host/mars_model.c b/thingino-accel_amd/csrc/host/mars_model.c
--- a/thingino-accel_amd/csrc/host/mars_model.c
+++ b/thingino-accel_amd/csrc/host/mars_model.c
@@ -31,6 +31,7 @@
     sw->no_chain = getenv("MARS_HIP_NO_CHAIN") != NULL;
     sw->no_both = getenv("MARS_HIP_NO_BOTH") != NULL;
     sw->no_both_chain = getenv("MARS_HIP_NO_BOTH_CHAIN") != NULL;
+    sw->no_next = getenv("MARS_HIP_NO_NEXT") != NULL;
     sw->rec_limit = (e = getenv("MARS_HIP_REC_LIMIT")) ? (size_t)strtoull(e, NULL, 0) : (size_t)0xfffffff0u;
     sw->vconcat_limit = (e = getenv("MARS_HIP_VCONCAT_LIMIT")) ? (size_t)strtoull(e, NULL, 0) : (size_t)0x7fffffffu;
     sw->bottleneck_limit = (e = getenv("MARS_HIP_BOTTLENECK_LIMIT")) ? (size_t)strtoull(e, NULL, 0) : 0;
@@ -162,6 +163,7 @@
         fuse_post(m);
         fuse_split(m);
         fuse_split_chain(m);
+        fuse_next(m);
         pad_output_rows(m);
         virtual_concat_q(m);
         fuse_both_chain(m);
@@ -208,6 +210,7 @@
     {FLAG(no_vconcat), ASK_VCONCAT, 0, 0},
     {FLAG(no_bottleneck), ASK_PRE, 0, 0},
     {FLAG(no_post), ASK_GROUP, FORM_POST, FORM_POST},
+    {FLAG(no_next), ASK_GROUP, FORM_NEXT, FORM_NEXT},
     {FLAG(no_chain), ASK_GROUP, FORM_SPLIT_CHAIN, FORM_SPLIT_CHAIN},
     {FLAG(no_split), ASK_GROUP, FORM_SPLIT, FORM_SPLIT_CHAIN},
     {FLAG(no_both_chain), ASK_GROUP, FORM_BOTH_CHAIN, FORM_BOTH_CHAIN},
@@ -223,8 +226,8 @@
     const size_t vlim = m->sw.vconcat_limit, blim = m->sw.bottleneck_limit;
     const int rec_replan = (size_t)n > m->rec_max_frames || (m->rec_skipped && n < m->rec_frames);
     m->rec_frames = n;
-    if (m->no_vconcat || m->no_bottleneck || m->no_post || m->no_split || m->no_chain || m->no_both || m->no_both_chain || rec_replan) {
-        m->no_vconcat = m->no_bottleneck = m->no_post = m->no_split = m->no_chain = m->no_both = m->no_both_chain = 0;
+    if (m->no_vconcat || m->no_bottleneck || m->no_post || m->no_split || m->no_chain || m->no_both || m->no_both_chain || m->no_next || rec_replan) {
+        m->no_vconcat = m->no_bottleneck = m->no_post = m->no_split = m->no_chain = m->no_both = m->no_both_chain = m->no_next = 0;
         const mars_error_t e = replan(m);
         if (e != MARS_OK) return e;
     }
@@ -411,6 +414,8 @@
     ADD(" split_chain %d", o->split_chain);
     if (o->split_chain) ADD(" %zd", (ssize_t)o->chain_w_off);
     ADD(" pair_both %d both_chain %d both_elide %d", o->pair_both, o->both_chain, o->both_elide);
+    ADD(" next_1x1 %d", o->next_1x1);
+    if (o->next_1x1) ADD(" %zd", (ssize_t)o->next_w_off);
     ADD(" pre %d", o->pre);
     if (o->pre) ADD(" %zd %zd %zd %a", (ssize_t)o->pre_w_off, (ssize_t)o->pre_b_off, (ssize_t)o->pre_lut2_off, (double)o->pre_cs);
     ADD(" macs %a bytes %a prof_kind %d", o->macs, o->bytes, o->prof_kind);
@@ -435,7 +440,7 @@
 #define FLAG(cond, ...) if (cond) k += snprintf(line + k, sizeof line - (size_t)k, __VA_ARGS__)
         FLAG(o->kind == OP_CONV_I8 || o->kind == OP_CONV_F32 || o->kind == OP_CONV_F32_VHEAD, " k%dx%d s%d c%d->%d", o->kh, o->kw, o->sw, o->in_c, o->out_c);
         FLAG(o->nchw, " relayout"); FLAG(o->out_nchw, " planar_store"); FLAG(o->lut_off != NO_OFF, " lut"); FLAG(o->add_t, " add=%d", o->add_t - 1);
-        FLAG(o->nseg, " seg=%d", o->nseg); FLAG(o->pair_next && !(o->pair_both && o->nseg), " pair_next");  FLAG(o->pair_both, " pair_both"); FLAG(o->both_chain, " both_chain=%d", o->both_chain); FLAG(o->both_elide, " both_elide"); FLAG(o->post_next, " post_next"); FLAG(o->split_next, " split_next"); FLAG(o->pre, " pre"); FLAG(o->silu_f32, " silu");
+        FLAG(o->nseg, " seg=%d", o->nseg); FLAG(o->pair_next && !(o->pair_both && o->nseg), " pair_next");  FLAG(o->pair_both, " pair_both"); FLAG(o->both_chain, " both_chain=%d", o->both_chain); FLAG(o->both_elide, " both_elide"); FLAG(o->post_next, " post_next"); FLAG(o->next_1x1, " next_1x1"); FLAG(o->split_next, " split_next"); FLAG(o->pre, " pre"); FLAG(o->silu_f32, " silu");
         FLAG(o->k_limit, " k_limit=%d", o->k_limit); FLAG(o->in_rec, " in_rec=%d", o->in_rec); FLAG(o->out_rec, " out_rec");
         FLAG(o->vc_shift, " view=-%d", o->vc_shift); FLAG(o->vc_n, " vcat=%dx%d", o->vc_n, o->vc_run);
         FLAG(o->rows_only, " rows_only=%d", o->rows_only); FLAG(o->out_byte_off, " out_off=%zu", o->out_byte_off); FLAG(o->chain_n, " chain=%d", o->chain_n);
@@ -461,10 +466,10 @@
     if (full) {
         const plan_switches_t *w = &m->sw;
         snprintf(line, sizeof line, "+plan n_ops %d arena_size %zu scratch_per_frame %zu blob_mirror_bytes %zu rec_max_frames %zu rec_skipped %d f32_mode %d | fusion %d"
-                 " no_fuse_lut %d no_nhwc_internal %d no_vconcat_q %d no_pair_f32 %d no_rec %d no_zero_tail %d no_vconcat_f32 %d no_rowpad %d no_post %d no_split %d no_chain %d no_both %d no_both_chain %d rec_limit %zu"
+                 " no_fuse_lut %d no_nhwc_internal %d no_vconcat_q %d no_pair_f32 %d no_rec %d no_zero_tail %d no_vconcat_f32 %d no_rowpad %d no_post %d no_split %d no_chain %d no_both %d no_both_chain %d no_next %d rec_limit %zu"
                  " vconcat_limit %zu bottleneck_limit %zu\n", m->n_ops, m->arena_size, m->scratch_per_frame, m->blob_mirror_bytes, m->rec_max_frames, m->rec_skipped,
                  m->plan_f32_mode, w->fusion, w->no_fuse_lut, w->no_nhwc_internal, w->no_vconcat_q, w->no_pair_f32, w->no_rec, w->no_zero_tail, w->no_vconcat_f32,
-                 w->no_rowpad, w->no_post, w->no_split, w->no_chain, w->no_both, w->no_both_chain, w->rec_limit, w->vconcat_limit, w->bottleneck_limit);
+                 w->no_rowpad, w->no_post, w->no_split, w->no_chain, w->no_both, w->no_both_chain, w->no_next, w->rec_limit, w->vconcat_limit, w->bottleneck_limit);
         EMIT();
     }
 #undef EMIT
diff --git a/thingino-accel_amd/csrc/host/mars_plan.c b/thingino-accel_amd/csrc/host/mars_plan.c
--- a/thingino-accel_amd/csrc/host/mars_plan.c
+++ b/thingino-accel_amd/csrc/host/mars_plan.c
@@ -671,8 +671,8 @@
 }
 void conv_i8_group_records(const mars_model_ext_t *m, int form, const mars_op_t *g[4], int side, int frames, int live, mhip_conv_i8_t *p) {
     const rec_ctx_t c = {m, frames, live};
-    const int patch = form == FORM_POST || form == FORM_SPLIT || form == FORM_SPLIT_CHAIN;
-    conv_i8_record(&c, g[0], patch, &p[0]);
+    const int patch = form == FORM_POST || form == FORM_SPLIT || form == FORM_SPLIT_CHAIN || form == FORM_NEXT;
+    conv_i8_record(&c, g[0], patch && form != FORM_NEXT, &p[0]);
     if (!patch) {
         for (int k = 1; k < form_span(form); k++) conv_i8_record(&c, g[k], 0, &p[k]);
         return;
@@ -688,6 +688,14 @@
         p->post_out_pix_stride = cv3->out_pix_stride; p->post_out_ch_off = cv3->out_ch_off;
         return;
     }
+    if (form == FORM_NEXT) {
+        const mars_op_t *d = g[1];
+        p->next_w = (const int8_t *)rec_param(&c, g[0]->next_w_off, 1);
+        p->next_lut2 = rec_param(&c, d->lut2_off, 0);
+        p->next_cs = d->cs;
+        p->next_out = (int8_t *)rec_addr(&c, d->t_out); p->next_out_stride = rec_stride(&c, d->t_out);
+        return;
+    }
     p->split_w = (const int8_t *)rec_param(&c, g[0]->split_w_off, 1);
     for (int k = 0; k < 2; k++) {
         p->split_lut2[k] = rec_param(&c, g[1 + k]->lut2_off, 0);
@@ -711,6 +719,7 @@
     conv_i8_group_records(m, form, g, side, frames, 0, p);
     switch (form) {
         case FORM_POST: return mhip_conv_i8_post_ok(&p[0]);
+        case FORM_NEXT: return mhip_conv_i8_next_ok(&p[0]);
         case FORM_SPLIT: case FORM_SPLIT_CHAIN: return mhip_conv_i8_split_ok(&p[0]);
         case FORM_BOTH: return mhip_conv_i8_both_ok(&p[0], &p[1]);
         case FORM_BOTH_CHAIN: return mhip_conv_i8_both_chain_ok(&p[0], &p[1], &p[2], side);
@@ -1236,7 +1245,7 @@
 }
 
 static int find_chained_1x1(const mars_model_ext_t *m, int i, int form, int c, const int *writers, int *side_out) {
-    const int n = form_span(form) - 1, O0 = m->ops[i + n - 2].t_out, O1 = m->ops[i + n - 1].t_out;
+    const int n = form_span(form) - 1, O0 = m->ops[n > 1 ? i + n - 2 : i].t_out, O1 = m->ops[i + n - 1].t_out;
     const mars_op_t *a = &m->ops[i], *g[4] = {a, a + 1, a + 2, NULL};
     for (int j = i + n; j < m->n_ops && j <= i + 48; j++) {
         const mars_op_t *d = &m->ops[j];
@@ -1274,6 +1283,36 @@
                                 (int8_t *)(m->arena_host + off));
         a->split_chain = side;
         a->chain_w_off = off;
+    }
+    free(readers);
+}
+
+void fuse_next(mars_model_ext_t *m) {
+    if (m->sw.no_next || m->no_next) return;
+    int *readers, *writers;
+    if (!use_counts(m, &readers, &writers)) return;
+    for (int i = 0; i + 1 < m->n_ops; i += op_span(m, i)) {
+        mars_op_t *a = &m->ops[i];
+        const int c = a->out_c, T = a->t_out;
+        if (a->kind != OP_CONV_I8 || a->pre || !op_plain(m, i)) continue;
+        if ((c != 32 && c != 64) || a->oc_pad != c || a->kh * a->kw < 2 || a->sh != 1 || a->sw != 1 || !a->safe || a->nchw || a->out_nchw || a->nseg ||
+            a->out_pix_stride || a->out_ch_off || a->store_c || a->chain_n || a->in_byte_off || a->out_byte_off || a->lut_off == NO_OFF ||
+            a->lut2_off == NO_OFF)
+            continue;
+        if (T < 0 || writers[T] != 1 || m->mt[T].io_in || m->mt[T].is_weight || m->mt[T].pix_stride) continue;
+        int side;
+        const int j = find_chained_1x1(m, i, FORM_NEXT, c, writers, &side);
+        if (j < 0) continue;
+        const size_t bytes = mhip_conv_i8_next_pack(c, NULL, NULL, NULL);
+        const size_t off = arena_reserve(m, bytes);
+        if (off == NO_OFF) break;
+        move_up(m, i + 1, j);
+        a = &m->ops[i];
+        const mars_op_t *d = &m->ops[i + 1];
+        mhip_conv_i8_next_pack(c, (const int8_t *)(m->arena_host + d->w_off), d->b_off != NO_OFF ? (const int32_t *)(m->arena_host + d->b_off) : NULL,
+                               (int8_t *)(m->arena_host + off));
+        a->next_1x1 = 1;
+        a->next_w_off = off;
     }
     free(readers);
 }
@@ -1787,6 +1826,10 @@
                                     M[3]->t_in[0] != M[o->split_chain]->t_out || M[3]->t_out < 0 || M[3]->t_out == M[1]->t_out || M[3]->t_out == M[2]->t_out ||
                                     M[3]->t_out == o->t_out || m->mt[M[3]->t_out].pix_stride || o->chain_w_off == NO_OFF))
             why = "split_chain without its 1x1 behind the pair";
+        else if (o->next_1x1 && (o->kind != OP_CONV_I8 || !M[1] || !free_1x1_ok(M[1], o, o->out_c, o->out_c) || !op_plain(m, g[1]) || M[1]->t_in[0] != o->t_out ||
+                                 M[1]->t_out < 0 || M[1]->t_out == o->t_out || op_reads(o, M[1]->t_out) || m->mt[M[1]->t_out].pix_stride ||
+                                 o->post_next || o->split_next || o->pair_next || o->pre || o->next_w_off == NO_OFF))
+            why = "next_1x1 without its 1x1 behind a stored result";
         else if (o->both_chain && (!o->pair_both || !M[2] || !free_1x1_ok(M[2], o, 64, 64) || !op_plain(m, g[2]) || (o->both_chain != 1 && o->both_chain != 2) ||
                                    M[2]->t_in[0] != M[o->both_chain - 1]->t_out || M[2]->t_out < 0 || M[2]->t_out == o->t_out || M[2]->t_out == M[1]->t_out))
             why = "both_chain without its 1x1 behind the pair";
diff --git a/thingino-accel_amd/csrc/host/mars_run.c b/thingino-accel_amd/csrc/host/mars_run.c
--- a/thingino-accel_amd/csrc/host/mars_run.c
+++ b/thingino-accel_amd/csrc/host/mars_run.c
@@ -281,7 +281,7 @@
         }
         int rc;
         switch (form) {
-            case FORM_POST: case FORM_SPLIT: case FORM_SPLIT_CHAIN: {
+            case FORM_POST: case FORM_SPLIT: case FORM_SPLIT_CHAIN: case FORM_NEXT: {
                 mhip_conv_i8_t p;
                 conv_i8_group_records(m, form, mem, op->split_chain, m->run_frames, 1, &p);
                 rc = mhip_conv_i8(&p);
diff --git a/thingino-accel_amd/csrc/mhip.h b/thingino-accel_amd/csrc/mhip.h
--- a/thingino-accel_amd/csrc/mhip.h
+++ b/thingino-accel_amd/csrc/mhip.h
@@ -88,7 +88,15 @@
     const uint8_t *chain_lut2;
     float chain_cs;
     int8_t *chain_out;      size_t chain_out_stride;
+    const int8_t *next_w;
+    const uint8_t *next_lut2;
+    float next_cs;
+    int8_t *next_out;       size_t next_out_stride;
 } mhip_conv_i8_t;
+int mhip_conv_i8_next_ok(const mhip_conv_i8_t *p);
+size_t mhip_conv_i8_next_pack(int c, const int8_t *packed, const int32_t *bias, int8_t *out);
+int mhip_conv_i8_next_k(int c, int k);
+int mhip_conv_i8_next_row(int c, int oc);
 int mhip_conv_i8_split_ok(const mhip_conv_i8_t *p);
 size_t mhip_conv_i8_split_pack(const int8_t *packed0, const int32_t *bias0, const int8_t *packed1, const int32_t *bias1, int8_t *out);
 int mhip_conv_i8_split_row(int side, int oc);
```

Result: no change. 61050 (median of 2 runs) (+0.2%).
